# gist-ailab/QuBER

Measured on AMD Instinct MI355X. Metric: refined masks/sec on 640x480 RGB-D (N=20 inst), higher is better.
Workload: dtype f32; 1 GPU; batch=16 640x480 RGB-D, 20 initial instances/frame, ResNet-50 RGB-D refiner (boundary-error -> fg/centre/offset), encode+network+grouping+mask extraction; parallelism=dp1, hipgraph=False, foreground_filter=False

## Files before the change

include/quber_hip.h:

```cpp
#ifndef QUBER_HIP_H
#define QUBER_HIP_H

#include <stddef.h>
#include <stdint.h>

#ifdef __cplusplus
extern "C" {
#endif

typedef struct quber_ctx quber_ctx;

typedef struct quber_config {
    int32_t height, width;
    int32_t max_batch;
    int32_t max_instances;
    int32_t resnet_depth;
    int32_t res5_dilation;
    int32_t backbone_fusion_layers;
    int32_t head_fusion_layers;
    int32_t error_classes;
    int32_t gaussian_sigma;
    int32_t nms_kernel;
    int32_t top_k;
    int32_t stuff_area;
    int32_t min_instance_area;
    int32_t label_divisor;
    int32_t with_network;
    float center_threshold;
    float boundary_ratio;
    float pixel_mean[6];
    float pixel_std[6];
    int32_t eee_mask_on;
    int32_t eee_boundary_on;
    int32_t hierarchical;
    int32_t fusion_feat;
    int32_t fusion_pred;
    int32_t n_levels;
    int32_t level_heads[5][5];
    int32_t fusion_add;
    int32_t streams;
    int32_t compute_dtype;
    int32_t encode_legacy_f32;
    int32_t convs_dim;
    int32_t head_channels;
} quber_config;

#define QUBER_LOGIT_BASE 4

void quber_default_config(quber_config* cfg);
const char* quber_last_error(void);
const char* quber_version(void);

int quber_create(const quber_config* cfg, quber_ctx** out);
void quber_destroy(quber_ctx* ctx);

int quber_set_weight(quber_ctx* ctx, const char* name, const float* host, int64_t numel);
int quber_finalize_weights(quber_ctx* ctx);
int quber_num_weights(quber_ctx* ctx);
int quber_weight_spec(quber_ctx* ctx, int index, const char** name, int64_t* numel);

int quber_encode_initial_masks(quber_ctx* ctx, const uint8_t* dev_masks, int32_t batch, int32_t n_masks,
                               float* dev_out, void* stream);

int quber_encode_label_map(quber_ctx* ctx, const int32_t* dev_labels, int32_t batch, int32_t n_instances, float* dev_out,
                           void* stream);

int64_t quber_workspace_bytes(quber_ctx* ctx);

int quber_explicit_error_maps(quber_ctx* ctx, const uint8_t* dev_init, int32_t n_init, const uint8_t* dev_gt,
                              int32_t n_gt, int32_t batch, uint8_t* dev_out, void* stream);

int quber_forward(quber_ctx* ctx, const uint8_t* dev_bgr, const uint8_t* dev_depth, const float* dev_offsets,
                  int32_t batch, float* dev_logits, void* stream);

int quber_forward_profiled(quber_ctx* ctx, const uint8_t* dev_bgr, const uint8_t* dev_depth,
                           const float* dev_offsets, int32_t batch, float* dev_logits, void* stream,
                           double* kind_ms, int32_t* kind_launches);

int quber_profile_begin(quber_ctx* ctx);
int quber_profile_end(quber_ctx* ctx, void* stream);
int quber_profile_num_stages(quber_ctx* ctx);
int quber_profile_stage(quber_ctx* ctx, int index, const char** name, double* ms, double* bytes, double* flops,
                        int32_t* launches);

int quber_postprocess(quber_ctx* ctx, const float* dev_logits, int32_t n_planes, int32_t batch,
                      float* dev_panoptic, int32_t* dev_count, float* dev_labels, float* dev_scores,
                      float* dev_boxes, int32_t* dev_centers, int32_t* dev_ncenters, void* stream);

int quber_extract_masks(quber_ctx* ctx, const float* dev_panoptic, const float* dev_labels, int32_t batch,
                        int32_t max_inst, uint8_t* dev_masks, void* stream);

int quber_tta_flip_inputs(quber_ctx* ctx, uint8_t* dev_bgr, uint8_t* dev_depth, uint8_t* dev_masks, int32_t batch,
                          int32_t n_masks, void* stream);
int quber_tta_merge(quber_ctx* ctx, const float* dev_logits2, int32_t n_planes, int32_t batch, float* dev_out,
                    void* stream);

int quber_error_decode(quber_ctx* ctx, const float* dev_logits, int32_t n_planes, int32_t first_plane, int32_t classes,
                       int32_t batch, uint8_t* dev_classes, uint32_t* dev_hist, void* stream);
int quber_error_mask_hist(quber_ctx* ctx, const uint8_t* dev_classes, const uint8_t* dev_masks, int32_t batch, int32_t n_masks,
                          int32_t classes, uint32_t* dev_out, void* stream);
int quber_error_score(quber_ctx* ctx, const uint8_t* dev_classes, const uint8_t* dev_explicit, int32_t kind, int32_t error_type,
                      int32_t classes, int32_t batch, uint64_t* dev_table, void* stream);
int quber_error_overlay(quber_ctx* ctx, const uint8_t* dev_bgr, const uint8_t* dev_classes, int32_t batch, uint32_t color0,
                        uint32_t color1, uint32_t color2, uint32_t color3, uint8_t* dev_out, void* stream);

int quber_relabel_panoptic(quber_ctx* ctx, const float* dev_panoptic, const float* dev_labels, const int32_t* dev_count,
                           int32_t batch, int32_t mirror, int32_t* dev_ids, void* stream);
int quber_overlap_masks(quber_ctx* ctx, const uint8_t* dev_masks, const int32_t* dev_ids, int32_t batch, int32_t n_masks,
                        int32_t n_ids, uint32_t* dev_table, uint32_t* dev_area, void* stream);
int quber_overlap_ids(quber_ctx* ctx, const int32_t* dev_a, const int32_t* dev_b, int32_t batch, int32_t n_a, int32_t n_b,
                      uint32_t* dev_table, void* stream);

int quber_cleanup_ids(quber_ctx* ctx, int32_t* dev_ids, int32_t batch, int32_t n_ids, int32_t connectivity, int32_t keep_largest,
                      int32_t min_island_area, int32_t max_hole_area, uint32_t* dev_report, void* stream);
int quber_cleanup_postprocess(quber_ctx* ctx, const float* dev_logits, int32_t n_planes, int32_t batch, float* dev_panoptic,
                              const float* dev_labels, const int32_t* dev_count, float* dev_scores, float* dev_boxes,
                              int32_t connectivity, int32_t keep_largest, int32_t min_island_area, int32_t max_hole_area,
                              uint32_t* dev_report, void* stream);

int quber_perturb_masks(quber_ctx* ctx, const uint8_t* dev_masks, int32_t batch, int32_t n_masks, const int32_t* dev_programs,
                        int32_t n_ops, int32_t ops_per_round, const double* dev_iou_targets, uint8_t* dev_out, uint32_t* dev_report,
                        int32_t placement, void* stream);

int quber_mask_nms(quber_ctx* ctx, const uint8_t* dev_masks, const float* dev_scores, int32_t batch, int32_t n_masks, float thresh,
                   int32_t on_top, uint8_t* dev_out_masks, int32_t* dev_ids, int32_t* dev_source, float* dev_out_scores,
                   int32_t* dev_report, void* stream);

int quber_scene_perturb(quber_ctx* ctx, const uint8_t* dev_gt, const uint8_t* dev_props, const int32_t* dev_n_gt, const int32_t* dev_n_prop,
                        int32_t batch, int32_t n_gt_rows, int32_t n_prop_rows, int32_t max_masks, double min_mask_ratio,
                        const uint8_t* dev_fp_act, const uint8_t* dev_gs_act, const uint8_t* dev_merge_act, const uint8_t* dev_split_act,
                        const int32_t* dev_split_try, const uint8_t* dev_delete_act, uint8_t* dev_out_masks, int32_t* dev_info,
                        int32_t* dev_report, void* stream);

int quber_coco_match(quber_ctx* ctx, const uint8_t* dev_dt, const float* dev_scores, const double* dev_dt_boxes, int32_t n_dt,
                     const uint8_t* dev_gt, const uint8_t* dev_gt_flags, const double* dev_gt_area, const double* dev_gt_boxes, int32_t n_gt,
                     int32_t batch, int32_t iou_type, const double* dev_iou_thrs, int32_t n_thrs, const double* dev_area_rng, int32_t n_rng,
                     int32_t* dev_counts, int32_t* dev_order, float* dev_out_scores, double* dev_dt_area, double* dev_gt_area_used,
                     double* dev_iou, uint8_t* dev_dtm, uint8_t* dev_dtig, uint8_t* dev_gi, int32_t* dev_gorder, void* stream);

int quber_meanshift_seeds(quber_ctx* ctx, const float* dev_emb, int32_t batch, int32_t channels, const int32_t* dev_first, int32_t num_seeds,
                          int32_t* dev_indices, void* stream);
int quber_meanshift_climb(quber_ctx* ctx, const float* dev_emb, int32_t batch, int32_t channels, const int32_t* dev_indices, int32_t num_seeds,
                          float kappa, int32_t iters, float* dev_seeds, void* stream);
int quber_meanshift_link(quber_ctx* ctx, const float* dev_seeds, int32_t batch, int32_t num_seeds, float epsilon, int32_t* dev_seed_labels,
                         void* stream);
int quber_meanshift_assign(quber_ctx* ctx, const float* dev_emb, int32_t batch, int32_t channels, const float* dev_seeds,
                           const int32_t* dev_seed_labels, int32_t num_seeds, const float* dev_depth_z, float depth_threshold, int32_t n_masks,
                           int32_t* dev_ids, uint8_t* dev_masks, int32_t* dev_report, void* stream);
int quber_meanshift_cluster(quber_ctx* ctx, const float* dev_emb, int32_t batch, int32_t channels, const int32_t* dev_first, int32_t num_seeds,
                            float kappa, int32_t iters, float epsilon, const float* dev_depth_z, float depth_threshold, int32_t n_masks,
                            int32_t* dev_indices, float* dev_seeds, int32_t* dev_seed_labels, int32_t* dev_ids, uint8_t* dev_masks,
                            int32_t* dev_report, void* stream);

int quber_gms_seeds(quber_ctx* ctx, const float* dev_votes, const uint8_t* dev_fg, int32_t batch, int32_t subsample, const int32_t* dev_first,
                    const uint32_t* dev_draws, int32_t num_seeds, int32_t* dev_indices, int32_t* dev_info, void* stream);
int quber_gms_climb(quber_ctx* ctx, const float* dev_votes, const uint8_t* dev_fg, int32_t batch, int32_t subsample, const int32_t* dev_indices,
                    const int32_t* dev_info, int32_t num_seeds, float sigma, int32_t iters, float* dev_seeds, void* stream);
int quber_gms_link(quber_ctx* ctx, const float* dev_seeds, int32_t batch, int32_t num_seeds, const int32_t* dev_info, float epsilon,
                   int32_t* dev_seed_labels, void* stream);
int quber_gms_assign(quber_ctx* ctx, const float* dev_votes, const uint8_t* dev_fg, int32_t batch, const float* dev_seeds,
                     const int32_t* dev_seed_labels, const int32_t* dev_info, int32_t num_seeds, int32_t min_pixels, int32_t n_masks,
                     int32_t* dev_ids, uint8_t* dev_masks, float* dev_centers, int32_t* dev_report, void* stream);
int quber_gms_imp(quber_ctx* ctx, int32_t* dev_ids, int32_t batch, int32_t n_ids, int32_t ksize, int32_t largest, int32_t n_masks,
                  uint8_t* dev_masks, float* dev_centers, int32_t* dev_report, void* stream);
int quber_gms_cluster(quber_ctx* ctx, const float* dev_votes, const uint8_t* dev_fg, int32_t batch, const int32_t* dev_first,
                      const uint32_t* dev_draws, int32_t num_seeds, float sigma, int32_t iters, float epsilon, int32_t subsample,
                      int32_t min_pixels, int32_t imp_ksize, int32_t imp_largest, int32_t n_masks, int32_t* dev_indices, float* dev_seeds,
                      int32_t* dev_seed_labels, int32_t* dev_info, int32_t* dev_raw_ids, int32_t* dev_ids, uint8_t* dev_masks,
                      float* dev_centers, int32_t* dev_report, void* stream);

int quber_zoom_rois(quber_ctx* ctx, const int32_t* dev_ids, int32_t batch, int32_t n_ids, float padding, int32_t* dev_rois, void* stream);
int quber_zoom_crop(quber_ctx* ctx, const uint8_t* dev_bgr, const uint8_t* dev_depth, const int32_t* dev_ids, const int32_t* dev_slots,
                    const int32_t* dev_rois, int32_t batch, int32_t n_ids, int32_t n_slots, int32_t crop, uint8_t* dev_bgr_crop,
                    uint8_t* dev_depth_crop, uint8_t* dev_mask_crop, void* stream);
int quber_zoom_paste(quber_ctx* ctx, const int32_t* dev_crop_ids, const float* dev_crop_scores, const uint32_t* dev_table,
                     const uint32_t* dev_area, const uint8_t* dev_depth_crop, const int32_t* dev_slots, const int32_t* dev_rois,
                     int32_t batch, int32_t n_ids, int32_t n_slots, int32_t crop, int32_t n_crop_ids, float min_overlap, int32_t max_inst,
                     int32_t* dev_out_ids, uint8_t* dev_out_masks, int32_t* dev_source, float* dev_out_scores, float* dev_boxes,
                     int32_t* dev_report, void* stream);

#define QUBER_LOSS_WORDS 40
typedef struct quber_loss_spec {
    double top_k;
    double foreground_weight;
    double center_weight;
    double offset_weight;
    int32_t error_type;
    int32_t eee_mask_plane;
    int32_t eee_boundary_plane;
    int32_t eee_mask_loss;
    int32_t eee_boundary_loss;
    int32_t reserved;
} quber_loss_spec;
int quber_loss_targets(quber_ctx* ctx, const int32_t* dev_gt, int32_t batch, int32_t n_gt, int32_t sigma, int32_t small_area,
                       float small_weight, const float* dev_gauss, float* dev_targets, double* dev_points, int32_t* dev_area, void* stream);
int quber_losses(quber_ctx* ctx, const float* dev_logits, int32_t n_planes, const float* dev_targets, const uint8_t* dev_explicit,
                 const quber_loss_spec* spec, int32_t batch, double* dev_out, void* stream);

int64_t quber_contingency_workspace_bytes(int32_t cap);
int quber_label_contingency(const int32_t* dev_pred, const int32_t* dev_gt, int64_t n_pixels, int32_t cap,
                            void* dev_workspace, void* stream);

int64_t quber_boundary_workspace_bytes(int32_t h, int32_t w, int32_t n_masks);
int quber_boundary_overlap(const int32_t* dev_pred, const int32_t* dev_gt, int32_t h, int32_t w, const int32_t* dev_labels,
                           int32_t n_pred, int32_t n_gt, int32_t bound_pix, void* dev_workspace, uint32_t* dev_out,
                           void* stream);

int64_t quber_eval_batch_workspace_bytes(int32_t batch, int32_t h, int32_t w, int32_t cap, int32_t with_boundary);
int quber_eval_batch(const int32_t* dev_pred, const int32_t* dev_gt, int32_t batch, int32_t h, int32_t w, int32_t cap, int32_t bound_pix,
                     int32_t with_boundary, int32_t placement, void* dev_workspace, void* dev_out, void* stream);
int quber_munkres_batch(const double* dev_score, const int32_t* dev_rows, const int32_t* dev_cols, int32_t batch, int32_t cap,
                        int32_t placement, void* dev_workspace, int32_t* dev_assign, int32_t* dev_status, void* stream);

int quber_foreground_filter(const float* dev_fg_logits, int32_t n_classes, int32_t fg_class, const uint8_t* dev_masks,
                            int32_t batch, int32_t n_masks, int64_t hw, uint8_t* dev_fg_mask, uint64_t* dev_counts,
                            void* stream);

int quber_foreground_overlap(const uint8_t* dev_fg, int32_t fg_h, int32_t fg_w, const uint8_t* dev_masks, int32_t batch, int32_t n_masks,
                             int32_t h, int32_t w, uint64_t* dev_counts, void* stream);

int quber_normalize_depth(const void* dev_depth, int32_t is_float32, int64_t n_pixels, double min_val, double max_val,
                          uint8_t* dev_out3, uint8_t* dev_zero, void* stream);

int quber_resize_u8(const uint8_t* dev_src, int32_t src_h, int32_t src_w, int32_t channels, uint8_t* dev_dst,
                    int32_t dst_h, int32_t dst_w, int32_t linear, void* stream);

int quber_inpaint_telea_u8(const uint8_t* host_img, const uint8_t* host_mask, int32_t h, int32_t w, int32_t radius,
                           uint8_t* host_out);
int quber_inpaint_depth_u8(const uint8_t* host_depth3, int32_t h, int32_t w, int32_t kernel, uint8_t* host_out3);
int64_t quber_inpaint_depth_workspace_bytes(int32_t batch, int32_t h, int32_t w);
int quber_inpaint_depth_device(const uint8_t* dev_depth3, int32_t batch, int32_t h, int32_t w, int32_t kernel, void* dev_workspace,
                               int64_t workspace_bytes, uint8_t* dev_out3, void* stream);

int quber_debug_tensor(quber_ctx* ctx, const char* name, float** dev_ptr, int32_t* dims4, int32_t* channel_stride);
int32_t quber_debug_tensor_elem_size(quber_ctx* ctx, const char* name);
double quber_forward_flops(quber_ctx* ctx);
double quber_forward_flops_executed(quber_ctx* ctx);
double quber_forward_flops_padding(quber_ctx* ctx);
int quber_set_option(quber_ctx* ctx, int32_t key, int32_t value);
int quber_get_option(quber_ctx* ctx, int32_t key, int32_t* value);
void quber_set_tuning(int32_t key, int32_t value);
int32_t quber_debug_persistent_segments(int32_t tiles, int32_t blocks, int32_t k_slices, int32_t min_share, int32_t block,
                                        int32_t* out4, int32_t cap);
int32_t quber_debug_persistent_fixup(int32_t tiles, int32_t blocks, int32_t k_slices, int32_t min_share, int32_t xcd, int32_t j,
                                     int32_t* tile, int32_t* slots, int32_t cap);
int64_t quber_debug_ws_bytes(int32_t which, int32_t b, int32_t n, int32_t m, int32_t h, int32_t w, int32_t flag);
int quber_num_ops(quber_ctx* ctx);
int quber_op_info(quber_ctx* ctx, int index, const char** name, int32_t* kind, double* flops, int32_t* launches);
int quber_op_conv2d(const float* dev_x, int32_t batch, int32_t h, int32_t w, int32_t cin, const float* dev_w_oihw,
                    int32_t cout, int32_t ksize, int32_t stride, int32_t pad, int32_t dil, const float* dev_scale,
                    const float* dev_shift, const float* dev_residual, int32_t relu, float* dev_packed_scratch,
                    float* dev_y, void* stream);
int quber_op_conv1x1_f16(const void* dev_x, int32_t batch, int32_t h, int32_t w, int32_t cin, const void* dev_w_oi,
                         int32_t cout, const float* dev_scale, const float* dev_shift, const void* dev_residual,
                         int32_t relu, void* dev_y, void* stream);
int quber_op_conv2d_f16(const void* dev_x, int32_t batch, int32_t h, int32_t w, int32_t cin, const void* dev_w_packed,
                        int32_t cout, int32_t ksize, int32_t stride, int32_t pad, int32_t dil, int32_t kmode,
                        const float* dev_scale, const float* dev_shift, const void* dev_residual, int32_t relu,
                        double* dev_gn_sums, int32_t gn_groups, void* dev_y, void* stream);
int quber_op_conv1x1_dual(const float* dev_y, const float* dev_x, int32_t batch, int32_t oh, int32_t ow, int32_t mid,
                          int32_t h2, int32_t w2, int32_t cin, int32_t stride, const float* dev_w, const float* dev_shift,
                          const float* dev_ones, int32_t cout, int32_t relu, float* dev_out, void* stream);
int quber_op_conv3x3_winograd(const float* dev_x, int32_t batch, int32_t h, int32_t w, int32_t cin,
                              const float* dev_w_oihw, int32_t cout, int32_t dil, int32_t m, const float* dev_scale,
                              const float* dev_shift,
                              int32_t relu, float* dev_u_scratch, float* dev_ws, int64_t ws_floats, float* dev_y,
                              void* stream);
int quber_op_conv2d_view(const float* dev_x, int32_t x_cs, int64_t x_gs, const float* dev_w_oihw, const float* dev_scale, const float* dev_shift,
                         const float* dev_residual, int32_t res_cs, int64_t res_gs, float* dev_y, int32_t y_cs, int64_t y_gs, int32_t groups_of_launch,
                         int32_t batch, int32_t h, int32_t w, int32_t cin, int32_t cout, int32_t ksize, int32_t stride, int32_t pad, int32_t dil,
                         int32_t relu, double* dev_gn_sums, int32_t gn_groups, float* dev_packed_scratch, void* stream);
int quber_debug_conv_route(int32_t x_off, int32_t x_cs, int64_t x_gs, int32_t affine, int32_t res_off, int32_t res_cs, int64_t res_gs, int32_t y_off,
                           int32_t y_cs, int64_t y_gs, int32_t groups_of_launch, int32_t batch, int32_t h, int32_t w, int32_t cin, int32_t cout,
                           int32_t ksize, int32_t stride, int32_t pad, int32_t dil, int32_t gn_groups, int32_t workspace, int32_t cus, int32_t* out12);
int quber_op_conv3x3_winograd_view(const float* dev_x, int32_t x_cs, int64_t x_gs, const float* dev_w_oihw, const float* dev_scale,
                                   const float* dev_shift, float* dev_y, int32_t y_cs, int64_t y_gs, int32_t groups_of_launch, int32_t batch, int32_t h,
                                   int32_t w, int32_t cin, int32_t cout, int32_t dil, int32_t m, int32_t relu, double* dev_gn_sums, int32_t gn_groups,
                                   const double* dev_n_stats, const float* dev_n_gamma, const float* dev_n_beta, int32_t n_param_gs, int32_t n_groups,
                                   int32_t n_relu, float n_eps, float* dev_u_scratch, float* dev_ws, int64_t ws_floats, void* stream);
int quber_debug_winograd_route(int32_t x_cs, int64_t x_gs, int32_t y_cs, int64_t y_gs, int32_t in_place, int32_t groups_of_launch, int32_t batch,
                               int32_t h, int32_t w, int32_t cin, int32_t cout, int32_t dil, int32_t m, int32_t gn_groups, int32_t norm_groups,
                               int64_t ws_floats, int32_t* out12);
int quber_op_conv1x1_dual_view(const float* dev_y, int64_t y_gs, const float* dev_x, int64_t x_gs, const float* dev_w, int64_t w_gs,
                               const float* dev_shift, const float* dev_ones, int32_t ss_gs, float* dev_out, int64_t out_gs, int32_t groups_of_launch,
                               int32_t batch, int32_t oh, int32_t ow, int32_t mid, int32_t h2, int32_t w2, int32_t cin, int32_t stride, int32_t cout,
                               int32_t relu, void* stream);
int quber_debug_dual_route(int64_t y_gs, int64_t x_gs, int64_t w_gs, int32_t ss_gs, int64_t out_gs, int32_t groups_of_launch, int32_t batch, int32_t oh,
                           int32_t ow, int32_t mid, int32_t h2, int32_t w2, int32_t cin, int32_t stride, int32_t cout, int32_t workspace, int32_t cus,
                           int32_t* out12);
int quber_op_groupnorm(const float* dev_x, int32_t batch, int32_t h, int32_t w, int32_t c, int32_t groups,
                       const float* dev_gamma, const float* dev_beta, float eps, int32_t relu,
                       double* dev_stats_scratch, float* dev_y, void* stream);
int quber_op_bilinear(const float* dev_x, int32_t batch, int32_t h, int32_t w, int32_t c, int32_t oh, int32_t ow,
                      float* dev_y, void* stream);
int quber_op_maxpool3x3s2(const float* dev_x, int32_t batch, int32_t h, int32_t w, int32_t c, float* dev_y,
                          void* stream);
int32_t quber_debug_gn_pixels_per_block(int32_t hw, int32_t c, int32_t batch, int32_t groups_of_launch, int32_t stats_pass);
int quber_op_gn_stats(const void* dev_x, int32_t x_cs, int64_t x_gs, int32_t es, int32_t batch, int32_t h, int32_t w, int32_t c,
                      int32_t groups_of_launch, int32_t groups, double* dev_stats, int32_t zero, void* stream);
int quber_op_gn_apply(const void* dev_x, int32_t x_cs, int64_t x_gs, int32_t x_es, void* dev_y, int32_t y_cs, int64_t y_gs, int32_t y_es,
                      int32_t batch, int32_t h, int32_t w, int32_t c, int32_t groups_of_launch, int32_t groups, const double* dev_stats,
                      const float* dev_gamma, const float* dev_beta, int32_t param_gs, float eps, int32_t relu, void* stream);
int quber_op_maxpool_view(const void* dev_x, int32_t x_cs, int64_t x_gs, int32_t x_es, void* dev_y, int32_t y_cs, int64_t y_gs, int32_t y_es,
                          int32_t batch, int32_t h, int32_t w, int32_t c, int32_t groups_of_launch, void* stream);
int quber_op_bilinear_view(const void* dev_x, int32_t x_cs, int32_t x_es, void* dev_y, int32_t y_cs, int32_t y_es, int32_t batch, int32_t h,
                           int32_t w, int32_t c, int32_t oh, int32_t ow, void* stream);
int quber_op_avgpool(const void* dev_x, int32_t x_cs, int32_t x_es, void* dev_y, int32_t y_cs, int32_t y_es, int32_t batch, int32_t h, int32_t w,
                     int32_t c, void* stream);
int quber_op_add_channels(const void* dev_a, int32_t a_cs, int32_t a_es, const void* dev_b, int32_t b_cs, int32_t b_es, void* dev_y, int32_t y_cs,
                          int32_t y_es, int32_t batch, int32_t h, int32_t w, int32_t c, void* stream);
int quber_op_copy_channels(const void* dev_x, int32_t x_cs, int32_t x_es, void* dev_y, int32_t y_cs, int32_t y_es, int32_t batch, int32_t h,
                           int32_t w, int32_t c, void* stream);
int quber_op_predictors(int32_t n, const void* const* dev_feat, const float* const* dev_w, const float* const* dev_bias, void* const* dev_act_dst,
                        const int32_t* cout, const int32_t* q_ch0, const int32_t* act, int32_t c, int32_t feat_cs, int32_t es, int32_t batch,
                        int32_t h, int32_t w, float* dev_q, int32_t q_nch, int32_t act_cs, void* stream);
int quber_op_upsample_logits(const float* dev_q, float* dev_out, int32_t batch, int32_t nch, int32_t h, int32_t w, int32_t scale, int32_t oh,
                             int32_t ow, uint32_t mul_mask, void* stream);
int quber_op_preprocess(const uint8_t* dev_bgr, const uint8_t* dev_depth, const float* dev_offsets, void* dev_x, int32_t x_c, int32_t es,
                        int32_t batch, int32_t batch_cap, int32_t h, int32_t w, const float* mean6, const float* std6, int32_t streams,
                        void* stream);
int quber_dsn_forward(quber_ctx* ctx, const float* dev_xyz, int32_t batch, int32_t flags, float* dev_fg_logits, float* dev_offsets, float* dev_votes,
                      uint8_t* dev_fg_classes, uint8_t* dev_fg, void* stream);
int quber_dsn_forward_profiled(quber_ctx* ctx, const float* dev_xyz, int32_t batch, int32_t flags, float* dev_fg_logits, float* dev_offsets,
                               float* dev_votes, uint8_t* dev_fg_classes, uint8_t* dev_fg, void* stream, double* op_ms);

int32_t quber_op_esp_tiles(int32_t h, int32_t w);
int64_t quber_op_esp_packed_floats(int32_t n1);
int quber_op_dsn_pack(const float* dev_xyz, int32_t batch, int32_t h, int32_t w, int32_t flags, float* dev_x8, float* dev_clean, void* stream);
int quber_op_esp_pack(const float* dev_w1, const float* dev_w2, const float* dev_w4, const float* dev_w8, const float* dev_w16, int32_t n, int32_t n1,
                      float* dev_packed, void* stream);
int quber_op_esp_branches(const float* dev_t, int32_t t_cs, const float* dev_x, int32_t x_cs, float* dev_out, int32_t out_cs, int32_t batch, int32_t h,
                          int32_t w, int32_t c, int32_t groups, const float* dev_packed, double* dev_partials, int32_t tiles, void* stream);
int quber_op_esp_merge(const float* dev_d1, int32_t d1_cs, const float* dev_d2, const float* dev_d4, const float* dev_d8, const float* dev_d16,
                       int32_t d_cs, const float* dev_x, int32_t x_cs, float* dev_out, int32_t out_cs, int32_t batch, int32_t h, int32_t w, int32_t c,
                       int32_t groups, double* dev_partials, int32_t tiles, void* stream);
int quber_op_esp_stats(const double* dev_partials, int32_t batch, int32_t tiles, int32_t groups, double* dev_stats, void* stream);
int quber_op_dsn_head(const float* dev_f, int32_t f_cs, int32_t batch, int32_t h, int32_t w, int32_t c, const float* dev_clean, const float* dev_wfg,
                      const float* dev_wcd, float* dev_logits, float* dev_offsets, float* dev_votes, uint8_t* dev_classes, uint8_t* dev_fg, void* stream);

int quber_rrn_forward(quber_ctx* ctx, const float* dev_rgb_crop, const uint8_t* dev_mask_crop, int32_t n, float logit_threshold, float* dev_logits,
                      uint8_t* dev_refined, void* stream);
int quber_rrn_forward_profiled(quber_ctx* ctx, const float* dev_rgb_crop, const uint8_t* dev_mask_crop, int32_t n, float logit_threshold, float* dev_logits,
                               uint8_t* dev_refined, void* stream, double* op_ms);
int quber_rrn_crop(quber_ctx* ctx, const uint8_t* dev_bytes, const int32_t* dev_ids, const int32_t* dev_slots, const int32_t* dev_rois, const float* dev_table,
                   int32_t batch, int32_t n_ids, int32_t n_slots, int32_t crop, float* dev_rgb_crop, uint8_t* dev_mask_crop, void* stream);
int quber_rrn_paste(quber_ctx* ctx, const uint8_t* dev_refined, const int32_t* dev_slots, const int32_t* dev_rois, const float* dev_z, int32_t batch,
                    int32_t n_ids, int32_t n_slots, int32_t crop, int32_t n_masks, int32_t* dev_out_ids, uint8_t* dev_out_masks, int32_t* dev_source,
                    float* dev_keys, int32_t* dev_report, void* stream);
int quber_op_rrn_pack(const float* dev_rgb, const uint8_t* dev_mask, int32_t batch, int32_t h, int32_t w, float* dev_x8, void* stream);
int quber_op_rrn_head(const float* dev_f, int32_t f_cs, int32_t batch, int32_t h, int32_t w, int32_t c, const float* dev_wfg, float thr, float* dev_logits,
                      uint8_t* dev_refined, void* stream);
int quber_op_rrn_head3(const float* dev_f, int32_t f_cs, int32_t batch, int32_t h, int32_t w, int32_t c, const float* dev_w9, float bias, float thr,
                       float* dev_logits, uint8_t* dev_refined, void* stream);

int32_t quber_op_cgnet_tiles(int32_t h, int32_t w, int32_t joint);
int quber_op_cgnet_joint(const float* dev_x, int32_t x_cs, float* dev_joi, int32_t joi_cs, int32_t batch, int32_t h, int32_t w, int32_t c, int32_t dil,
                         const float* dev_w1, const float* dev_scale1, const float* dev_shift1, const float* dev_slope1, const float* dev_wloc,
                         const float* dev_wsur, const float* dev_scale2, const float* dev_shift2, const float* dev_slope2, double* dev_partials,
                         int32_t tiles, void* stream);
int quber_op_cgnet_sums(const float* dev_x, int32_t x_cs, int32_t batch, int32_t h, int32_t w, int32_t c, double* dev_partials, int32_t tiles,
                        void* stream);
int quber_op_cgnet_apply(const float* dev_joi, int32_t joi_cs, const float* dev_x, int32_t x_cs, float* dev_out, int32_t out_cs, int32_t batch,
                         int32_t h, int32_t w, int32_t c, int32_t hidden, const double* dev_partials, int32_t tiles, const float* dev_fc0,
                         const float* dev_b0, const float* dev_fc2, const float* dev_b2, float* dev_mean, float* dev_y, void* stream);

int quber_op_lmff_preprocess(const uint8_t* dev_bgr, const uint8_t* dev_depth, int64_t pixels, float* dev_x, void* stream);
int quber_op_lmff_dwconv(const float* dev_x, int32_t x_cs, float* dev_y, int32_t y_cs, int32_t batch, int32_t h, int32_t w, int32_t c, int32_t dil,
                         const float* dev_w9, const float* dev_scale, const float* dev_shift, const float* dev_slope, void* stream);
int quber_op_lmff_pool(const float* dev_x, int32_t x_cs, float* dev_y, int32_t y_cs, int32_t batch, int32_t h, int32_t w, int32_t c, int32_t oh,
                       int32_t ow, int32_t mode, void* stream);
int quber_op_lmff_affine(const float* dev_a, int32_t a_cs, const float* dev_b, int32_t b_cs, float* dev_y, int32_t y_cs, int32_t batch, int32_t h,
                         int32_t w, int32_t c, const float* dev_scale, const float* dev_shift, const float* dev_slope, void* stream);
int quber_op_lmff_pmca(const float* dev_x, int32_t x_cs, int32_t batch, int32_t h, int32_t w, int32_t c, const float* dev_w2x2, const float* dev_fc0,
                       const float* dev_alpha, const float* dev_fc2, float* dev_wts, double* dev_sums, void* stream);
int quber_op_lmff_scale(const float* dev_x, int32_t x_cs, const float* dev_wts, float* dev_y, int32_t y_cs, int32_t batch, int32_t h, int32_t w,
                        int32_t c, void* stream);
int quber_op_lmff_gate(const float* dev_o, int32_t o_cs, const float* dev_att, int32_t att_cs, float* dev_q, int32_t batch, int32_t h, int32_t w,
                       int32_t c, void* stream);
int quber_op_group_pixels(const float* dev_logits, int32_t n_planes, int32_t batch, int32_t h, int32_t w, int32_t cap,
                          const int32_t* dev_centers, const int32_t* dev_ncenters, uint8_t* dev_ids, uint32_t* dev_area,
                          void* stream);

#ifdef __cplusplus
}
#endif
#endif
```

quber_amd/_lib.py:

```python
import ctypes as C
import os

_HERE = os.path.dirname(os.path.abspath(__file__))
LIB_PATH = os.environ.get("QUBER_LIB") or os.path.join(_HERE, "libquber_hip.so")


class QuberConfig(C.Structure):
    _fields_ = [
        ("height", C.c_int32), ("width", C.c_int32), ("max_batch", C.c_int32), ("max_instances", C.c_int32),
        ("resnet_depth", C.c_int32), ("res5_dilation", C.c_int32), ("backbone_fusion_layers", C.c_int32),
        ("head_fusion_layers", C.c_int32), ("error_classes", C.c_int32), ("gaussian_sigma", C.c_int32),
        ("nms_kernel", C.c_int32), ("top_k", C.c_int32), ("stuff_area", C.c_int32),
        ("min_instance_area", C.c_int32), ("label_divisor", C.c_int32), ("with_network", C.c_int32),
        ("center_threshold", C.c_float), ("boundary_ratio", C.c_float),
        ("pixel_mean", C.c_float * 6), ("pixel_std", C.c_float * 6),
        ("eee_mask_on", C.c_int32), ("eee_boundary_on", C.c_int32), ("hierarchical", C.c_int32),
        ("fusion_feat", C.c_int32), ("fusion_pred", C.c_int32), ("n_levels", C.c_int32),
        ("level_heads", (C.c_int32 * 5) * 5), ("fusion_add", C.c_int32), ("streams", C.c_int32),
        ("compute_dtype", C.c_int32), ("encode_legacy_f32", C.c_int32),
        ("convs_dim", C.c_int32), ("head_channels", C.c_int32),
    ]


class QuberError(RuntimeError):
    pass


_P = C.c_void_p
_I = C.c_int32
SIGNATURES = {
    "quber_default_config": (None, [C.POINTER(QuberConfig)]),
    "quber_last_error": (C.c_char_p, []),
    "quber_version": (C.c_char_p, []),
    "quber_create": (C.c_int, [C.POINTER(QuberConfig), C.POINTER(_P)]),
    "quber_destroy": (None, [_P]),
    "quber_set_weight": (C.c_int, [_P, C.c_char_p, _P, C.c_int64]),
    "quber_finalize_weights": (C.c_int, [_P]),
    "quber_num_weights": (C.c_int, [_P]),
    "quber_weight_spec": (C.c_int, [_P, C.c_int, C.POINTER(C.c_char_p), C.POINTER(C.c_int64)]),
    "quber_encode_initial_masks": (C.c_int, [_P, _P, _I, _I, _P, _P]),
    "quber_encode_label_map": (C.c_int, [_P, _P, _I, _I, _P, _P]),
    "quber_workspace_bytes": (C.c_int64, [_P]),
    "quber_explicit_error_maps": (C.c_int, [_P, _P, _I, _P, _I, _I, _P, _P]),
    "quber_forward": (C.c_int, [_P, _P, _P, _P, _I, _P, _P]),
    "quber_forward_profiled": (C.c_int, [_P, _P, _P, _P, _I, _P, _P, C.POINTER(C.c_double * 3), C.POINTER(_I * 3)]),
    "quber_profile_begin": (C.c_int, [_P]),
    "quber_profile_end": (C.c_int, [_P, _P]),
    "quber_profile_num_stages": (C.c_int, [_P]),
    "quber_profile_stage": (C.c_int, [_P, C.c_int, C.POINTER(C.c_char_p), C.POINTER(C.c_double), C.POINTER(C.c_double),
                                      C.POINTER(C.c_double), C.POINTER(_I)]),
    "quber_postprocess": (C.c_int, [_P, _P, _I, _I, _P, _P, _P, _P, _P, _P, _P, _P]),
    "quber_extract_masks": (C.c_int, [_P, _P, _P, _I, _I, _P, _P]),
    "quber_tta_flip_inputs": (C.c_int, [_P, _P, _P, _P, _I, _I, _P]),
    "quber_tta_merge": (C.c_int, [_P, _P, _I, _I, _P, _P]),
    "quber_error_decode": (C.c_int, [_P, _P, _I, _I, _I, _I, _P, _P, _P]),
    "quber_error_mask_hist": (C.c_int, [_P, _P, _P, _I, _I, _I, _P, _P]),
    "quber_error_score": (C.c_int, [_P, _P, _P, _I, _I, _I, _I, _P, _P]),
    "quber_error_overlay": (C.c_int, [_P, _P, _P, _I, C.c_uint32, C.c_uint32, C.c_uint32, C.c_uint32, _P, _P]),
    "quber_relabel_panoptic": (C.c_int, [_P, _P, _P, _P, _I, _I, _P, _P]),
    "quber_overlap_masks": (C.c_int, [_P, _P, _P, _I, _I, _I, _P, _P, _P]),
    "quber_overlap_ids": (C.c_int, [_P, _P, _P, _I, _I, _I, _P, _P]),
    "quber_cleanup_ids": (C.c_int, [_P, _P, _I, _I, _I, _I, _I, _I, _P, _P]),
    "quber_cleanup_postprocess": (C.c_int, [_P, _P, _I, _I, _P, _P, _P, _P, _P, _I, _I, _I, _I, _P, _P]),
    "quber_perturb_masks": (C.c_int, [_P, _P, _I, _I, _P, _I, _I, _P, _P, _P, _I, _P]),
    "quber_mask_nms": (C.c_int, [_P, _P, _P, _I, _I, C.c_float, _I, _P, _P, _P, _P, _P, _P]),
    "quber_scene_perturb": (C.c_int, [_P, _P, _P, _P, _P, _I, _I, _I, _I, C.c_double] + [_P] * 10),
    "quber_coco_match": (C.c_int, [_P, _P, _P, _P, _I, _P, _P, _P, _P, _I, _I, _I, _P, _I, _P, _I] + [_P] * 11),
    "quber_meanshift_seeds": (C.c_int, [_P, _P, _I, _I, _P, _I, _P, _P]),
    "quber_meanshift_climb": (C.c_int, [_P, _P, _I, _I, _P, _I, C.c_float, _I, _P, _P]),
    "quber_meanshift_link": (C.c_int, [_P, _P, _I, _I, C.c_float, _P, _P]),
    "quber_meanshift_assign": (C.c_int, [_P, _P, _I, _I, _P, _P, _I, _P, C.c_float, _I, _P, _P, _P, _P]),
    "quber_meanshift_cluster": (C.c_int, [_P, _P, _I, _I, _P, _I, C.c_float, _I, C.c_float, _P, C.c_float, _I, _P, _P, _P, _P, _P, _P, _P]),
    "quber_gms_seeds": (C.c_int, [_P, _P, _P, _I, _I, _P, _P, _I, _P, _P, _P]),
    "quber_gms_climb": (C.c_int, [_P, _P, _P, _I, _I, _P, _P, _I, C.c_float, _I, _P, _P]),
    "quber_gms_link": (C.c_int, [_P, _P, _I, _I, _P, C.c_float, _P, _P]),
    "quber_gms_assign": (C.c_int, [_P, _P, _P, _I, _P, _P, _P, _I, _I, _I, _P, _P, _P, _P, _P]),
    "quber_gms_imp": (C.c_int, [_P, _P, _I, _I, _I, _I, _I, _P, _P, _P, _P]),
    "quber_gms_cluster": (C.c_int, [_P, _P, _P, _I, _P, _P, _I, C.c_float, _I, C.c_float, _I, _I, _I, _I, _I, _P, _P, _P, _P, _P, _P, _P, _P, _P, _P]),
    "quber_zoom_rois": (C.c_int, [_P, _P, _I, _I, C.c_float, _P, _P]),
    "quber_zoom_crop": (C.c_int, [_P, _P, _P, _P, _P, _P, _I, _I, _I, _I, _P, _P, _P, _P]),
    "quber_zoom_paste": (C.c_int, [_P, _P, _P, _P, _P, _P, _P, _P, _I, _I, _I, _I, _I, C.c_float, _I, _P, _P, _P, _P, _P, _P, _P]),
    "quber_loss_targets": (C.c_int, [_P, _P, _I, _I, _I, _I, C.c_float, _P, _P, _P, _P, _P]),
    "quber_losses": (C.c_int, [_P, _P, _I, _P, _P, _P, _I, _P, _P]),
    "quber_contingency_workspace_bytes": (C.c_int64, [_I]),
    "quber_label_contingency": (C.c_int, [_P, _P, C.c_int64, _I, _P, _P]),
    "quber_boundary_workspace_bytes": (C.c_int64, [_I, _I, _I]),
    "quber_boundary_overlap": (C.c_int, [_P, _P, _I, _I, _P, _I, _I, _I, _P, _P, _P]),
    "quber_eval_batch_workspace_bytes": (C.c_int64, [_I, _I, _I, _I, _I]),
    "quber_eval_batch": (C.c_int, [_P, _P, _I, _I, _I, _I, _I, _I, _I, _P, _P, _P]),
    "quber_munkres_batch": (C.c_int, [_P, _P, _P, _I, _I, _I, _P, _P, _P, _P]),
    "quber_foreground_filter": (C.c_int, [_P, _I, _I, _P, _I, _I, C.c_int64, _P, _P, _P]),
    "quber_normalize_depth": (C.c_int, [_P, _I, C.c_int64, C.c_double, C.c_double, _P, _P, _P]),
    "quber_inpaint_telea_u8": (C.c_int, [_P, _P, _I, _I, _I, _P]),
    "quber_inpaint_depth_u8": (C.c_int, [_P, _I, _I, _I, _P]),
    "quber_inpaint_depth_workspace_bytes": (C.c_int64, [_I, _I, _I]),
    "quber_inpaint_depth_device": (C.c_int, [_P, _I, _I, _I, _I, _P, C.c_int64, _P, _P]),
    "quber_resize_u8": (C.c_int, [_P, _I, _I, _I, _P, _I, _I, _I, _P]),
    "quber_debug_tensor": (C.c_int, [_P, C.c_char_p, C.POINTER(_P), C.POINTER(_I * 4), C.POINTER(_I)]),
    "quber_debug_tensor_elem_size": (C.c_int32, [_P, C.c_char_p]),
    "quber_forward_flops": (C.c_double, [_P]),
    "quber_forward_flops_executed": (C.c_double, [_P]),
    "quber_forward_flops_padding": (C.c_double, [_P]),
    "quber_set_tuning": (None, [_I, _I]),
    "quber_set_option": (C.c_int, [_P, _I, _I]),
    "quber_get_option": (C.c_int, [_P, _I, C.POINTER(_I)]),
    "quber_num_ops": (C.c_int, [_P]),
    "quber_op_info": (C.c_int, [_P, C.c_int, C.POINTER(C.c_char_p), C.POINTER(_I), C.POINTER(C.c_double), C.POINTER(_I)]),
    "quber_debug_persistent_segments": (C.c_int32, [_I, _I, _I, _I, _I, _P, _I]),
    "quber_debug_persistent_fixup": (C.c_int32, [_I, _I, _I, _I, _I, _I, _P, _P, _I]),
    "quber_debug_ws_bytes": (C.c_int64, [_I, _I, _I, _I, _I, _I, _I]),
    "quber_op_conv1x1_f16": (C.c_int, [_P, _I, _I, _I, _I, _P, _I, _P, _P, _P, _I, _P, _P]),
    "quber_op_conv2d_f16": (C.c_int, [_P, _I, _I, _I, _I, _P, _I, _I, _I, _I, _I, _I, _P, _P, _P, _I, _P, _I, _P, _P]),
    "quber_op_conv1x1_dual": (C.c_int, [_P, _P, _I, _I, _I, _I, _I, _I, _I, _I, _P, _P, _P, _I, _I, _P, _P]),
    "quber_op_conv2d": (C.c_int, [_P, _I, _I, _I, _I, _P, _I, _I, _I, _I, _I, _P, _P, _P, _I, _P, _P, _P]),
    "quber_op_conv3x3_winograd": (C.c_int, [_P, _I, _I, _I, _I, _P, _I, _I, _I, _P, _P, _I, _P, _P, C.c_int64, _P, _P]),
    "quber_op_conv2d_view": (C.c_int, [_P, _I, C.c_int64, _P, _P, _P, _P, _I, C.c_int64, _P, _I, C.c_int64] + [_I] * 11 + [_P, _I, _P, _P]),
    "quber_debug_conv_route": (C.c_int, [_I, _I, C.c_int64, _I, _I, _I, C.c_int64, _I, _I, C.c_int64] + [_I] * 13 + [_P]),
    "quber_op_conv3x3_winograd_view": (C.c_int, [_P, _I, C.c_int64, _P, _P, _P, _P, _I, C.c_int64] + [_I] * 9 + [_P, _I, _P, _P, _P, _I, _I, _I, C.c_float,
                                                 _P, _P, C.c_int64, _P]),
    "quber_debug_winograd_route": (C.c_int, [_I, C.c_int64, _I, C.c_int64] + [_I] * 11 + [C.c_int64, _P]),
    "quber_op_conv1x1_dual_view": (C.c_int, [_P, C.c_int64, _P, C.c_int64, _P, C.c_int64, _P, _P, _I, _P, C.c_int64] + [_I] * 11 + [_P]),
    "quber_debug_dual_route": (C.c_int, [C.c_int64, C.c_int64, C.c_int64, _I, C.c_int64] + [_I] * 12 + [_P]),
    "quber_op_groupnorm": (C.c_int, [_P, _I, _I, _I, _I, _I, _P, _P, C.c_float, _I, _P, _P, _P]),
    "quber_op_bilinear": (C.c_int, [_P, _I, _I, _I, _I, _I, _I, _P, _P]),
    "quber_op_maxpool3x3s2": (C.c_int, [_P, _I, _I, _I, _I, _P, _P]),
    "quber_debug_gn_pixels_per_block": (C.c_int32, [_I, _I, _I, _I, _I]),
    "quber_op_gn_stats": (C.c_int, [_P, _I, C.c_int64, _I, _I, _I, _I, _I, _I, _I, _P, _I, _P]),
    "quber_op_gn_apply": (C.c_int, [_P, _I, C.c_int64, _I, _P, _I, C.c_int64, _I, _I, _I, _I, _I, _I, _I, _P, _P, _P, _I, C.c_float, _I, _P]),
    "quber_op_maxpool_view": (C.c_int, [_P, _I, C.c_int64, _I, _P, _I, C.c_int64, _I, _I, _I, _I, _I, _I, _P]),
    "quber_op_bilinear_view": (C.c_int, [_P, _I, _I, _P, _I, _I, _I, _I, _I, _I, _I, _I, _P]),
    "quber_op_avgpool": (C.c_int, [_P, _I, _I, _P, _I, _I, _I, _I, _I, _I, _P]),
    "quber_op_add_channels": (C.c_int, [_P, _I, _I, _P, _I, _I, _P, _I, _I, _I, _I, _I, _I, _P]),
    "quber_op_copy_channels": (C.c_int, [_P, _I, _I, _P, _I, _I, _I, _I, _I, _I, _P]),
    "quber_op_predictors": (C.c_int, [_I, _P, _P, _P, _P, _P, _P, _P, _I, _I, _I, _I, _I, _I, _P, _I, _I, _P]),
    "quber_op_upsample_logits": (C.c_int, [_P, _P, _I, _I, _I, _I, _I, _I, _I, C.c_uint32, _P]),
    "quber_op_preprocess": (C.c_int, [_P, _P, _P, _P, _I, _I, _I, _I, _I, _I, _P, _P, _I, _P]),
    "quber_op_group_pixels": (C.c_int, [_P, _I, _I, _I, _I, _I, _P, _P, _P, _P, _P]),
    "quber_foreground_overlap": (C.c_int, [_P, _I, _I, _P, _I, _I, _I, _I, _P, _P]),
    "quber_dsn_forward": (C.c_int, [_P, _P, _I, _I, _P, _P, _P, _P, _P, _P]),
    "quber_dsn_forward_profiled": (C.c_int, [_P, _P, _I, _I, _P, _P, _P, _P, _P, _P, _P]),
    "quber_op_esp_tiles": (C.c_int32, [_I, _I]),
    "quber_op_esp_packed_floats": (C.c_int64, [_I]),
    "quber_op_dsn_pack": (C.c_int, [_P, _I, _I, _I, _I, _P, _P, _P]),
    "quber_op_esp_pack": (C.c_int, [_P, _P, _P, _P, _P, _I, _I, _P, _P]),
    "quber_op_esp_branches": (C.c_int, [_P, _I, _P, _I, _P, _I, _I, _I, _I, _I, _I, _P, _P, _I, _P]),
    "quber_op_esp_merge": (C.c_int, [_P, _I, _P, _P, _P, _P, _I, _P, _I, _P, _I, _I, _I, _I, _I, _I, _P, _I, _P]),
    "quber_op_esp_stats": (C.c_int, [_P, _I, _I, _I, _P, _P]),
    "quber_op_dsn_head": (C.c_int, [_P, _I, _I, _I, _I, _I, _P, _P, _P, _P, _P, _P, _P, _P, _P]),
    "quber_rrn_forward": (C.c_int, [_P, _P, _P, _I, C.c_float, _P, _P, _P]),
    "quber_rrn_forward_profiled": (C.c_int, [_P, _P, _P, _I, C.c_float, _P, _P, _P, _P]),
    "quber_rrn_crop": (C.c_int, [_P, _P, _P, _P, _P, _P, _I, _I, _I, _I, _P, _P, _P]),
    "quber_rrn_paste": (C.c_int, [_P, _P, _P, _P, _P, _I, _I, _I, _I, _I, _P, _P, _P, _P, _P, _P]),
    "quber_op_rrn_pack": (C.c_int, [_P, _P, _I, _I, _I, _P, _P]),
    "quber_op_rrn_head": (C.c_int, [_P, _I, _I, _I, _I, _I, _P, C.c_float, _P, _P, _P]),
    "quber_op_rrn_head3": (C.c_int, [_P, _I, _I, _I, _I, _I, _P, C.c_float, C.c_float, _P, _P, _P]),
    "quber_op_cgnet_tiles": (C.c_int32, [_I, _I, _I]),
    "quber_op_cgnet_joint": (C.c_int, [_P, _I, _P, _I, _I, _I, _I, _I, _I] + [_P] * 10 + [_I, _P]),
    "quber_op_cgnet_sums": (C.c_int, [_P, _I, _I, _I, _I, _I, _P, _I, _P]),
    "quber_op_cgnet_apply": (C.c_int, [_P, _I, _P, _I, _P, _I, _I, _I, _I, _I, _I, _P, _I, _P, _P, _P, _P, _P, _P, _P]),
    "quber_op_lmff_preprocess": (C.c_int, [_P, _P, C.c_int64, _P, _P]),
    "quber_op_lmff_dwconv": (C.c_int, [_P, _I, _P, _I, _I, _I, _I, _I, _I, _P, _P, _P, _P, _P]),
    "quber_op_lmff_pool": (C.c_int, [_P, _I, _P, _I, _I, _I, _I, _I, _I, _I, _I, _P]),
    "quber_op_lmff_affine": (C.c_int, [_P, _I, _P, _I, _P, _I, _I, _I, _I, _I, _P, _P, _P, _P]),
    "quber_op_lmff_pmca": (C.c_int, [_P, _I, _I, _I, _I, _I, _P, _P, _P, _P, _P, _P, _P]),
    "quber_op_lmff_scale": (C.c_int, [_P, _I, _P, _P, _I, _I, _I, _I, _I, _P]),
    "quber_op_lmff_gate": (C.c_int, [_P, _I, _P, _I, _P, _I, _I, _I, _I, _P]),
}

_lib = None


def load():
    global _lib
    if _lib is not None:
        return _lib
    if not os.path.exists(LIB_PATH):
        raise QuberError(
            f"{LIB_PATH} not found: build it with `make -C quber_amd/csrc` (or __graft_entry__.build()); "
            "quber_amd has no CPU fallback")
    import torch
    lib = C.CDLL(LIB_PATH)
    for name, (res, args) in SIGNATURES.items():
        fn = getattr(lib, name)
        fn.restype = res
        fn.argtypes = args
    mode = os.environ.get("QUBER_WINOGRAD", "auto").lower()
    if mode not in ("auto", "f6", "f4", "f2", "off"):
        raise QuberError(f"QUBER_WINOGRAD={mode!r}: expected auto, f6, f4, f2 or off")
    lib.quber_set_tuning(6, 1 if mode == "off" else 0)
    lib.quber_set_tuning(9, {"f2": 2, "f4": 4, "f6": 6}.get(mode, 0))
    if "QUBER_PERSIST" in os.environ:
        lib.quber_set_tuning(13, int(os.environ["QUBER_PERSIST"]))
    _lib = lib
    return lib


def check(rc):
    if rc != 0:
        raise QuberError(load().quber_last_error().decode())
```

quber_amd/csrc/api.hip:

```cpp
#include "plan.h"

#include <optional>

using namespace quber;

namespace quber { int wf_read_stamps(unsigned long long* dst, int n), h8_read_stamps(unsigned long long* dst, int n), x8_read_stamps(unsigned long long* dst, int n); }

int quber::check_cfg(const quber_config& c) {
    if (c.height <= 0 || c.width <= 0) return fail("height and width must be positive");
    if (c.with_network && (c.height < 16 || c.width < 16)) return fail("frames smaller than 16 x 16 are not supported");
    if (c.with_network == 2) {
        if (c.height % 8 || c.width % 8) return fail("LMFFNet needs height and width to be multiples of 8");
        return c.max_batch >= 1 ? 0 : fail("max_batch must be >= 1");
    }
    if (c.with_network == 3) {
        if (c.height % 8 || c.width % 8) return fail("CGNet needs height and width to be multiples of 8");
        return c.max_batch >= 1 ? 0 : fail("max_batch must be >= 1");
    }
    if (c.with_network == 4) {
        if (c.height < 16 || c.width < 16 || c.height % 16 || c.width % 16) return fail("the Depth Seeding Network needs height and width to be multiples of 16");
        return c.max_batch >= 1 ? 0 : fail("max_batch must be >= 1");
    }
    if (c.with_network == 5) {
        if (c.height != c.width || c.height < 16 || c.height % 16) return fail("the Region Refinement Network needs square crops whose side is a multiple of 16");
        return c.max_batch >= 1 ? 0 : fail("max_batch must be >= 1");
    }
    if (c.max_batch < 1) return fail("max_batch must be >= 1");
    if (c.max_instances < 1) return fail("max_instances must be >= 1");
    if (c.resnet_depth != 50 && c.resnet_depth != 101 && c.resnet_depth != 152) return fail("resnet_depth must be 50, 101 or 152");
    if (c.res5_dilation != 1 && c.res5_dilation != 2 && c.res5_dilation != 4) return fail("res5_dilation must be 1, 2 or 4");
    if (c.res5_dilation == 1) return fail("res5_dilation 1 (output stride 32) is not supported by this build");
    if (c.error_classes < 2 || c.error_classes > 4) return fail("error_classes must be 2..4");
    if (c.streams != 1 && c.streams != 2) return fail("streams must be 1 or 2");
    if (c.with_network == 1 && c.convs_dim != 128 && c.convs_dim != 256) return fail("convs_dim must be 128 or 256");
    if (c.with_network == 1 && c.head_channels != 32 && c.head_channels != 64) return fail("head_channels must be 32 or 64");
    if (c.compute_dtype < 0 || c.compute_dtype > 3)
        return fail("compute_dtype must be 0 (fp32 MFMA), 1 (bf16 operands), 2 (fp16 operands) or 3 (fp32 operands as 3 bf16 terms)");
    if (c.with_network && c.hierarchical) {
        if (c.n_levels < 1 || c.n_levels > 5) return fail("n_levels must be 1..5");
        int seen[5] = {0, 0, 0, 0, 0};
        for (int i = 0; i < c.n_levels; ++i) {
            if (c.level_heads[i][0] < 0) return fail("empty hierarchy level");
            for (int j = 0; j < 5 && c.level_heads[i][j] >= 0; ++j) {
                const int k = c.level_heads[i][j];
                if (k > 4) return fail("hierarchy head id out of range");
                seen[k]++;
            }
        }
        const int want[5] = {1, 1, 1, c.eee_mask_on ? 1 : 0, c.eee_boundary_on ? 1 : 0};
        for (int k = 0; k < 5; ++k)
            if (seen[k] != want[k]) return fail("the hierarchy must list every enabled head exactly once");
    }
    if (c.top_k < 1 || c.top_k > 254) return fail("top_k must be in 1..254");
    if (c.gaussian_sigma < 1 || c.gaussian_sigma > 40) return fail("gaussian_sigma out of range");
    return 0;
}

static int ws_reserve(quber_ctx* c, LazyWs& w, size_t need) {
    if (need <= w.bytes) return 0;
    if (w.p) {
        QB_CHECK(hipFree(w.p));
        c->alloc_bytes -= w.bytes;
        w = LazyWs();
    }
    QB_CHECK(hipMalloc(&w.p, need));
    w.bytes = need;
    c->alloc_bytes += need;
    return 0;
}

extern "C" {

const char* quber_version(void) { return "quber-hip 0.1 (gfx950, fp32 MFMA)"; }

void quber_default_config(quber_config* c) {
    memset(c, 0, sizeof(*c));
    c->height = 480; c->width = 640; c->max_batch = 1; c->max_instances = 64;
    c->resnet_depth = 50; c->res5_dilation = 2; c->backbone_fusion_layers = 2; c->head_fusion_layers = 3;
    c->error_classes = 4; c->gaussian_sigma = 10; c->nms_kernel = 7; c->top_k = 200; c->stuff_area = 2048;
    c->min_instance_area = 512; c->label_divisor = 1000; c->with_network = 1;
    c->eee_mask_on = 0; c->eee_boundary_on = 1; c->hierarchical = 1; c->fusion_feat = 1; c->fusion_pred = 1;
    c->n_levels = 2;
    c->streams = 2;
    c->fusion_add = 0;
    c->convs_dim = 128; c->head_channels = 32;
    for (int i = 0; i < 5; ++i)
        for (int j = 0; j < 5; ++j) c->level_heads[i][j] = -1;
    c->level_heads[0][0] = 4;
    c->level_heads[1][0] = 0; c->level_heads[1][1] = 1; c->level_heads[1][2] = 2;
    c->center_threshold = 0.3f; c->boundary_ratio = 0.01f;
    const float mean[6] = {103.53f, 116.28f, 123.675f, 127.5f, 127.5f, 127.5f};
    for (int i = 0; i < 6; ++i) { c->pixel_mean[i] = mean[i]; c->pixel_std[i] = 1.f; }
}

int quber_create(const quber_config* cfg, quber_ctx** out) {
    if (!cfg || !out) return fail("null argument");
    if (check_cfg(*cfg)) return -1;
    int ndev = 0;
    if (hipGetDeviceCount(&ndev) != hipSuccess || ndev == 0) return fail("no HIP device available");
    int device = 0;
    if (hipGetDevice(&device) != hipSuccess) return fail("hipGetDevice failed");
    quber_ctx* c = new quber_ctx();
    c->cfg = *cfg;
    c->tune = quber::g_tune;
    c->device = device;
    const int B = cfg->max_batch, H = cfg->height, W = cfg->width;
    const int sg = cfg->gaussian_sigma, side = 6 * sg + 3, c0 = 3 * sg + 1;
    std::vector<float> g((size_t)side * side);
    for (int y = 0; y < side; ++y)
        for (int x = 0; x < side; ++x)
            g[(size_t)y * side + x] = (float)exp(-((double)((x - c0) * (x - c0)) + (double)((y - c0) * (y - c0))) / (2.0 * sg * sg));
    Builder b(c, false);
    c->gauss = b.upload(g);
    c->enc_ws = b.dalloc_bytes(encode_ws_bytes(B, cfg->max_instances, H, W));
    c->enc_bad = (int*)b.dalloc_bytes(16);
    c->err_ws = (uint8_t*)b.dalloc_bytes(errmaps_ws_bytes(B, cfg->max_instances > 0 ? cfg->max_instances : 1, H, W));
    c->post_ws = b.dalloc_bytes(postprocess_ws_bytes(B, H, W, cfg->top_k));
    c->cleanup_ws = b.dalloc_bytes(cleanup_ws_bytes(B, H, W, cfg->top_k));
    if (!b.err.empty()) {
        std::string e = b.err;
        quber_destroy(c);
        return fail(e);
    }
    if (cfg->with_network) {
        Builder dry(c, true);
        if (cfg->with_network == 2) build_lmff(dry);
        else if (cfg->with_network == 3) build_cgnet(dry);
        else if (cfg->with_network == 4) build_dsn(dry);
        else if (cfg->with_network == 5) build_rrn(dry);
        else dry.build();
    }
    *out = c;
    return 0;
}

void quber_destroy(quber_ctx* c) {
    if (!c) return;
    if (c->prof && quber::g_prof == c->prof.get()) quber::g_prof = nullptr;
    for (hipEvent_t e : c->prof_events) (void)hipEventDestroy(e);
    for (int l = 1; l < LANES; ++l) {
        if (c->lane_fork[l]) (void)hipEventDestroy(c->lane_fork[l]);
        if (c->lane_join[l]) (void)hipEventDestroy(c->lane_join[l]);
        if (c->lane_stream[l]) (void)hipStreamDestroy(c->lane_stream[l]);
    }
    for (void* p : c->allocs) (void)hipFree(p);
    for (LazyWs& w : c->lazy)
        if (w.p) (void)hipFree(w.p);
    delete c;
}

int quber_num_weights(quber_ctx* c) { return c ? (int)c->specs.size() : 0; }
int quber_weight_spec(quber_ctx* c, int i, const char** name, int64_t* numel) {
    if (!c || i < 0 || i >= (int)c->specs.size()) return fail("weight index out of range");
    *name = c->specs[i].first.c_str();
    *numel = c->specs[i].second;
    return 0;
}

int quber_set_weight(quber_ctx* c, const char* name, const float* host, int64_t numel) {
    if (!c || !name || !host || numel <= 0) return fail("bad argument to quber_set_weight");
    if (c->finalized) return fail("weights already finalized");
    c->hostw[name].assign(host, host + numel);
    return 0;
}

int quber_finalize_weights(quber_ctx* c) {
    if (!c) return fail("null context");
    if (!c->cfg.with_network) return fail("context was created with with_network = 0");
    if (c->finalized) return fail("weights already finalized");
    quber::TuneScope tscope(&c->tune);
    Builder b(c, false);
    c->flops = c->wino_flops = c->wino_saved = c->wino_pad = 0.0;
    if (c->cfg.with_network >= 2 && c->cfg.with_network <= 5) {
        c->splitk_floats = (size_t)4 << 20;
        c->splitk_ws = (float*)b.dalloc_bytes(sizeof(float) * c->splitk_floats);
        if (c->cfg.with_network == 2) build_lmff(b);
        else if (c->cfg.with_network == 3) build_cgnet(b);
        else if (c->cfg.with_network == 4) build_dsn(b);
        else build_rrn(b);
    } else {
        b.build();
    }
    if (c->wino_floats) c->wino_ws = (float*)b.dalloc_bytes(sizeof(float) * c->wino_floats);
    if (c->lanes_built) {
        c->lane_splitk_floats = c->splitk_floats;
        for (int l = 1; l < LANES; ++l) {
            QB_CHECK(hipStreamCreateWithFlags(&c->lane_stream[l], hipStreamNonBlocking));
            QB_CHECK(hipEventCreateWithFlags(&c->lane_fork[l], hipEventDisableTiming));
            QB_CHECK(hipEventCreateWithFlags(&c->lane_join[l], hipEventDisableTiming));
            c->lane_splitk_ws[l] = (float*)b.dalloc_bytes(sizeof(float) * c->lane_splitk_floats);
            if (c->lane_wino_floats[l]) c->lane_wino_ws[l] = (float*)b.dalloc_bytes(sizeof(float) * c->lane_wino_floats[l]);
        }
    }
    if (!b.err.empty()) {
        c->ops.clear();
        return fail(b.err);
    }
    QB_CHECK(hipDeviceSynchronize());
    c->hostw.clear();
    c->finalized = true;
    return 0;
}

double quber_forward_flops(quber_ctx* c) { return c ? c->flops : 0.0; }
double quber_forward_flops_executed(quber_ctx* c) {
    if (!c) return 0.0;
    return c->flops - c->wino_saved;
}
double quber_forward_flops_padding(quber_ctx* c) { return c ? c->wino_pad : 0.0; }
void quber_set_tuning(int32_t key, int32_t value) {
    if (op_set_tuning(key, value)) return;
    (void)quber::tuning_set(quber::g_tune, key, value);
}

int quber_set_option(quber_ctx* c, int32_t key, int32_t value) {
    if (!c) return fail("null context");
    if (quber::tuning_plan_time(key) && c->finalized) return fail("option " + std::to_string(key) + " shapes the plan: set it before quber_finalize_weights");
    if (!quber::tuning_set(c->tune, key, value)) return fail("unknown option key " + std::to_string(key));
    return 0;
}

int quber_get_option(quber_ctx* c, int32_t key, int32_t* value) {
    if (!c || !value) return fail("null argument");
    int* f = quber::tuning_field(c->tune, key);
    if (!f) return fail("unknown option key " + std::to_string(key));
    *value = *f;
    return 0;
}

#ifdef WF_STAMPS
int quber_wf_read_stamps(unsigned long long* dst, int n) { return quber::wf_read_stamps(dst, n); }
#endif
#ifdef H8_STAMPS
int quber_h8_read_stamps(unsigned long long* dst, int n) { return quber::h8_read_stamps(dst, n); }
#endif
#ifdef X8_STAMPS
int quber_x8_read_stamps(unsigned long long* dst, int n) { return quber::x8_read_stamps(dst, n); }
#endif
#ifdef PK_STAMPS
int quber_pk_read_stamps(unsigned long long* dst, int n) { return quber::pk_read_stamps(dst, n); }
int quber_pk_read_span(unsigned long long* dst, int n) { return quber::pk_read_span(dst, n); }
#endif

int32_t quber_debug_persistent_segments(int32_t tiles, int32_t blocks, int32_t k_slices, int32_t min_share, int32_t block, int32_t* out4, int32_t cap) {
    return quber::conv_persistent_segments(tiles, blocks, k_slices, min_share, block, out4, cap);
}
int32_t quber_debug_persistent_fixup(int32_t tiles, int32_t blocks, int32_t k_slices, int32_t min_share, int32_t xcd, int32_t j, int32_t* tile, int32_t* slots, int32_t cap) {
    return quber::conv_persistent_fixup(tiles, blocks, k_slices, min_share, xcd, j, tile, slots, cap);
}

int64_t quber_debug_ws_bytes(int32_t which, int32_t b, int32_t n, int32_t m, int32_t h, int32_t w, int32_t flag) {
    switch (which) {
    case 0: return (int64_t)mask_nms_ws_bytes(b, n, h, w);
    case 1: return (int64_t)coco_match_ws_bytes(b, n, h, w, flag);
    case 2: return (int64_t)scene_ws_bytes(b, n, m, h, w);
    case 3: return (int64_t)meanshift_ws_bytes(b, h, w);
    case 4: return (int64_t)gms_ws_bytes(b, h, w);
    case 5: return (int64_t)zoom_ws_bytes(b, h, w);
    case 6: return (int64_t)losses_ws_bytes(b, h, w);
    case 7: return (int64_t)cleanup_ws_bytes(b, h, w, n);
    case 8: return (int64_t)postprocess_ws_bytes(b, h, w, n);
    default: return -1;
    }
}

int quber_profile_begin(quber_ctx* c) {
    if (!c) return fail("null context");
    if (!c->prof) c->prof.reset(new quber::Profiler());
    c->prof->recs.clear(); c->prof->sums.clear(); c->prof->used = 0;
    quber::g_prof = c->prof.get();
    return 0;
}

int quber_profile_end(quber_ctx* c, void* stream) {
    if (!c || !c->prof || quber::g_prof != c->prof.get()) return fail("quber_profile_end without quber_profile_begin");
    quber::g_prof = nullptr;
    QB_CHECK(hipStreamSynchronize((hipStream_t)stream));
    quber::Profiler& p = *c->prof;
    p.sums.assign(p.tags.size(), quber::StageSum());
    for (size_t i = 0; i < p.tags.size(); ++i) p.sums[i].name = p.tags[i];
    for (const quber::ProfRec& r : p.recs) {
        float ms = 0.f;
        QB_CHECK(hipEventElapsedTime(&ms, r.e0, r.e1));
        quber::StageSum& s = p.sums[r.tag];
        s.ms += ms; s.bytes += r.bytes; s.flops += r.flops; s.launches += 1;
    }
    return 0;
}

int quber_profile_num_stages(quber_ctx* c) { return (c && c->prof) ? (int)c->prof->sums.size() : 0; }

int quber_profile_stage(quber_ctx* c, int i, const char** name, double* ms, double* bytes, double* flops, int32_t* launches) {
    if (!c || !c->prof || i < 0 || i >= (int)c->prof->sums.size()) return fail("stage index out of range");
    const quber::StageSum& s = c->prof->sums[i];
    *name = s.name.c_str(); *ms = s.ms; *bytes = s.bytes; *flops = s.flops; *launches = s.launches;
    return 0;
}

int quber_num_ops(quber_ctx* c) { return c ? (int)c->ops.size() : 0; }
int quber_op_info(quber_ctx* c, int i, const char** name, int32_t* kind, double* flops, int32_t* launches) {
    if (!c || i < 0 || i >= (int)c->ops.size()) return fail("op index out of range");
    const Op& o = c->ops[i];
    *name = o.name.c_str(); *kind = o.kind; *flops = o.flops; *launches = o.launches;
    return 0;
}

int quber_encode_initial_masks(quber_ctx* c, const uint8_t* masks, int32_t batch, int32_t n, float* out, void* stream) {
    if (check_batch(c, batch)) return -1;
    if (n > c->cfg.max_instances) return fail("more initial masks than max_instances");
    if (!masks && n > 0) return fail("null masks");
    return launch_encode(masks, batch, n, c->cfg.height, c->cfg.width, c->gauss, c->cfg.gaussian_sigma, c->cfg.encode_legacy_f32, c->enc_ws, out, (hipStream_t)stream);
}

int quber_encode_label_map(quber_ctx* c, const int32_t* labels, int32_t batch, int32_t n, float* out, void* stream) {
    if (check_batch(c, batch)) return -1;
    if (n > c->cfg.max_instances) return fail("more instances than max_instances");
    if (!labels && n > 0) return fail("null label map");
    return launch_encode_labels(labels, batch, n, c->cfg.height, c->cfg.width, c->gauss, c->cfg.gaussian_sigma, c->cfg.encode_legacy_f32, c->enc_ws, out, c->enc_bad, (hipStream_t)stream);
}

int64_t quber_workspace_bytes(quber_ctx* c) { return c ? (int64_t)c->alloc_bytes : 0; }

int quber_explicit_error_maps(quber_ctx* c, const uint8_t* init, int32_t n_init, const uint8_t* gt, int32_t n_gt, int32_t batch, uint8_t* out, void* stream) {
    if (check_batch(c, batch)) return -1;
    const int H = c->cfg.height, W = c->cfg.width;
    int d = (int)rint((double)c->cfg.boundary_ratio * sqrt((double)H * H + (double)W * W));
    if (d < 1) d = 1;
    return launch_errmaps(init, n_init, gt, n_gt, batch, c->cfg.max_instances > 0 ? c->cfg.max_instances : 1, H, W, d, c->err_ws, out, (hipStream_t)stream);
}

static int forward_begin(quber_ctx* c, const char* who, std::optional<quber::TuneScope>& scope, const uint8_t* bgr, const uint8_t* depth,
                         const float* offs, int batch, float* logits, bool lmff_own, bool rest_ok, const char* null_msg, hipStream_t st) {
    if (check_batch(c, batch)) return -1;
    if (!c->finalized) return fail(std::string(who) + " before quber_finalize_weights");
    scope.emplace(&c->tune);
    if (c->cfg.with_network == 4) return fail(std::string(who) + ": a Depth Seeding Network context runs through quber_dsn_forward");
    if (c->cfg.with_network == 5) return fail(std::string(who) + ": a Region Refinement Network context runs through quber_rrn_forward");
    if (lmff_own && c->cfg.with_network >= 2) return 1;
    if (!bgr || (!depth && c->cfg.streams == 2) || !offs || !logits || !rest_ok) return fail(null_msg);
    c->cur_out = logits;
    c->cur_bgr = bgr; c->cur_depth = depth; c->cur_off = offs;
    return c->stem_fused ? 0 : launch_preprocess(bgr, depth, offs, c->X, batch, c->cfg.max_batch, c->cfg.height, c->cfg.width,
                                                 c->cfg.pixel_mean, c->cfg.pixel_std, c->cfg.streams, st);
}

int quber_forward(quber_ctx* c, const uint8_t* bgr, const uint8_t* depth, const float* offs, int32_t batch, float* logits, void* stream) {
    hipStream_t st = (hipStream_t)stream;
    std::optional<quber::TuneScope> tscope;
    int rc = forward_begin(c, "quber_forward", tscope, bgr, depth, offs, batch, logits, true, true, "null tensor", st);
    if (rc == 1) {
        if (!bgr || !depth || !logits) return fail("null tensor");
        c->cur_out = logits;
        const long pixels = (long)batch * c->cfg.height * c->cfg.width;
        int r2 = c->cfg.with_network == 3 ? launch_cg_preprocess(bgr, depth, pixels, c->X.p, st) : launch_lmff_preprocess(bgr, depth, pixels, c->X.p, st);
        for (size_t i = 0; !r2 && i < c->ops.size(); ++i)
            if (!c->ops[i].ctl) r2 = c->ops[i].run(batch, st);
        return r2;
    }
    if (rc) return rc;
    c->lanes_on = c->lanes_built && tune().lanes && batch <= (c->cfg.compute_dtype == 0 || c->cfg.compute_dtype == 3 ? LANE_BATCH_F32 : LANE_BATCH) && c->lane_stream[1] != nullptr &&
                  quber::g_prof == nullptr;
    auto lane_used = [&](int l) { return c->lanes_on && l > 0; };
    for (auto& op : c->ops) {
        if (op.ctl == 1) {
            if (lane_used(op.lane)) {
                QB_CHECK(hipEventRecord(c->lane_fork[op.lane], st));
                QB_CHECK(hipStreamWaitEvent(c->lane_stream[op.lane], c->lane_fork[op.lane], 0));
            }
            continue;
        }
        if (op.ctl == 2) {
            if (lane_used(op.lane)) {
                QB_CHECK(hipEventRecord(c->lane_join[op.lane], c->lane_stream[op.lane]));
                QB_CHECK(hipStreamWaitEvent(st, c->lane_join[op.lane], 0));
            }
            continue;
        }
        c->lane_now = lane_used(op.lane) ? op.lane : 0;
        rc = op.run(batch, c->lane_now ? c->lane_stream[op.lane] : st);
        if (rc) return rc;
    }
    c->lane_now = 0;
    c->lanes_on = false;
    return 0;
}

static int run_ops(quber_ctx* c, int batch, hipStream_t st, double* op_ms) {
    const size_t n = c->ops.size();
    if (op_ms && c->prof_events.size() < 2 * n) {
        const size_t old = c->prof_events.size();
        c->prof_events.resize(2 * n);
        for (size_t i = old; i < 2 * n; ++i) QB_CHECK(hipEventCreate(&c->prof_events[i]));
    }
    for (size_t i = 0; i < n; ++i) {
        if (op_ms) QB_CHECK(hipEventRecord(c->prof_events[2 * i], st));
        if (!c->ops[i].ctl) {
            const int rc = c->ops[i].run(batch, st);
            if (rc) return rc;
        }
        if (op_ms) QB_CHECK(hipEventRecord(c->prof_events[2 * i + 1], st));
    }
    if (!op_ms) return 0;
    QB_CHECK(hipStreamSynchronize(st));
    for (size_t i = 0; i < n; ++i) {
        float ms = 0.f;
        QB_CHECK(hipEventElapsedTime(&ms, c->prof_events[2 * i], c->prof_events[2 * i + 1]));
        op_ms[i] = ms;
    }
    return 0;
}

static int dsn_run(quber_ctx* c, const char* who, const float* xyz, int batch, int flags, float* fg_logits, float* offsets, float* votes, uint8_t* fg_classes, uint8_t* fg,
                   hipStream_t st, double* op_ms) {
    if (check_batch(c, batch)) return -1;
    if (c->cfg.with_network != 4) return fail(std::string(who) + ": the context was not created with with_network = 4");
    if (!c->finalized) return fail(std::string(who) + " before quber_finalize_weights");
    if (!xyz) return fail(std::string(who) + ": null xyz");
    if (flags & ~1) return fail(std::string(who) + ": unknown flag bits");
    quber::TuneScope tscope(&c->tune);
    c->dsn_xyz = xyz; c->dsn_flags = flags;
    c->dsn_logits = fg_logits; c->dsn_offsets = offsets; c->dsn_votes = votes; c->dsn_classes = fg_classes; c->dsn_fg = fg;
    return run_ops(c, batch, st, op_ms);
}

int quber_dsn_forward(quber_ctx* c, const float* xyz, int32_t batch, int32_t flags, float* fg_logits, float* offsets, float* votes, uint8_t* fg_classes, uint8_t* fg,
                      void* stream) {
    return dsn_run(c, "quber_dsn_forward", xyz, batch, flags, fg_logits, offsets, votes, fg_classes, fg, (hipStream_t)stream, nullptr);
}

int quber_dsn_forward_profiled(quber_ctx* c, const float* xyz, int32_t batch, int32_t flags, float* fg_logits, float* offsets, float* votes, uint8_t* fg_classes,
                               uint8_t* fg, void* stream, double* op_ms) {
    if (!op_ms) return fail("quber_dsn_forward_profiled: null op_ms");
    return dsn_run(c, "quber_dsn_forward_profiled", xyz, batch, flags, fg_logits, offsets, votes, fg_classes, fg, (hipStream_t)stream, op_ms);
}

static int rrn_run(quber_ctx* c, const char* who, const float* rgb_crop, const uint8_t* mask_crop, int n, float thr, float* logits, uint8_t* refined, hipStream_t st,
                   double* op_ms) {
    if (check_batch(c, n)) return -1;
    if (c->cfg.with_network != 5) return fail(std::string(who) + ": the context was not created with with_network = 5");
    if (!c->finalized) return fail(std::string(who) + " before quber_finalize_weights");
    if (!rgb_crop || !mask_crop) return fail(std::string(who) + ": null crops");
    if (!logits && !refined) return fail(std::string(who) + ": neither logits nor refined masks requested");
    if (!(thr == thr)) return fail(std::string(who) + ": logit_threshold is not a number");
    quber::TuneScope tscope(&c->tune);
    c->rrn_rgb = rgb_crop; c->rrn_mask = mask_crop; c->rrn_thr = thr; c->rrn_logits = logits; c->rrn_refined = refined;
    return run_ops(c, n, st, op_ms);
}

int quber_rrn_forward(quber_ctx* c, const float* rgb_crop, const uint8_t* mask_crop, int32_t n, float logit_threshold, float* logits, uint8_t* refined, void* stream) {
    return rrn_run(c, "quber_rrn_forward", rgb_crop, mask_crop, n, logit_threshold, logits, refined, (hipStream_t)stream, nullptr);
}

int quber_rrn_forward_profiled(quber_ctx* c, const float* rgb_crop, const uint8_t* mask_crop, int32_t n, float logit_threshold, float* logits, uint8_t* refined,
                               void* stream, double* op_ms) {
    if (!op_ms) return fail("quber_rrn_forward_profiled: null op_ms");
    return rrn_run(c, "quber_rrn_forward_profiled", rgb_crop, mask_crop, n, logit_threshold, logits, refined, (hipStream_t)stream, op_ms);
}

int quber_forward_profiled(quber_ctx* c, const uint8_t* bgr, const uint8_t* depth, const float* offs, int32_t batch,
                           float* logits, void* stream, double* kind_ms, int32_t* kind_launches) {
    hipStream_t st = (hipStream_t)stream;
    std::optional<quber::TuneScope> tscope;
    int rc = forward_begin(c, "quber_forward_profiled", tscope, bgr, depth, offs, batch, logits, false, kind_ms && kind_launches, "null argument", st);
    if (rc) return rc;
    const size_t n = c->ops.size();
    if (c->prof_events.size() < 2 * n) {
        const size_t old = c->prof_events.size();
        c->prof_events.resize(2 * n);
        for (size_t i = old; i < 2 * n; ++i) QB_CHECK(hipEventCreate(&c->prof_events[i]));
    }
    c->lanes_on = false;
    for (size_t i = 0; i < n; ++i) {
        QB_CHECK(hipEventRecord(c->prof_events[2 * i], st));
        if (!c->ops[i].ctl) {
            rc = c->ops[i].run(batch, st);
            if (rc) return rc;
        }
        QB_CHECK(hipEventRecord(c->prof_events[2 * i + 1], st));
    }
    QB_CHECK(hipStreamSynchronize(st));
    for (int k = 0; k < OP_KINDS; ++k) { kind_ms[k] = 0.0; kind_launches[k] = 0; }
    for (size_t i = 0; i < n; ++i) {
        float ms = 0.f;
        QB_CHECK(hipEventElapsedTime(&ms, c->prof_events[2 * i], c->prof_events[2 * i + 1]));
        kind_ms[c->ops[i].kind] += ms;
        kind_launches[c->ops[i].kind] += 1;
    }
    return 0;
}

int quber_postprocess(quber_ctx* c, const float* logits, int32_t n_planes, int32_t batch, float* pan, int32_t* count,
                      float* labels, float* scores, float* boxes, int32_t* centers, int32_t* ncenters, void* stream) {
    if (check_batch(c, batch)) return -1;
    PostCfg pc;
    pc.threshold = c->cfg.center_threshold; pc.nms_kernel = c->cfg.nms_kernel; pc.top_k = c->cfg.top_k;
    pc.stuff_area = c->cfg.stuff_area; pc.min_area = c->cfg.min_instance_area; pc.label_divisor = c->cfg.label_divisor;
    pc.cap = c->cfg.top_k;
    return launch_postprocess(logits, n_planes, batch, c->cfg.height, c->cfg.width, pc, c->post_ws, pan, count, labels,
                              scores, boxes, centers, ncenters, (hipStream_t)stream);
}

int quber_extract_masks(quber_ctx* c, const float* pan, const float* labels, int32_t batch, int32_t max_inst,
                        uint8_t* masks, void* stream) {
    if (check_batch(c, batch)) return -1;
    return launch_extract_masks(pan, labels, batch, c->cfg.height, c->cfg.width, c->cfg.top_k, max_inst, masks,
                                (hipStream_t)stream);
}

int quber_tta_flip_inputs(quber_ctx* c, uint8_t* bgr, uint8_t* depth, uint8_t* masks, int32_t batch, int32_t n, void* stream) {
    if (check_tta_batch(c, batch)) return -1;
    if (n < 0 || n > c->cfg.max_instances) return fail("initial masks outside 0..max_instances");
    if (!bgr || (!masks && n > 0)) return fail("null tensor");
    const int H = c->cfg.height, W = c->cfg.width;
    const long hw = (long)H * W;
    hipStream_t st = (hipStream_t)stream;
    if (launch_tta_flip_u8(bgr, bgr + batch * hw * 3, batch, H, W, 3, st)) return -1;
    if (depth && launch_tta_flip_u8(depth, depth + batch * hw * 3, batch, H, W, 3, st)) return -1;
    if (n > 0 && launch_tta_flip_u8(masks, masks + (long)batch * n * hw, (long)batch * n, H, W, 1, st)) return -1;
    return 0;
}

int quber_tta_merge(quber_ctx* c, const float* logits2, int32_t n_planes, int32_t batch, float* out, void* stream) {
    if (check_tta_batch(c, batch)) return -1;
    if (n_planes < 4) return fail("test-time augmentation: fewer than 4 logit planes");
    if (!logits2 || !out) return fail("null tensor");
    return launch_tta_merge(logits2, n_planes, batch, c->cfg.height, c->cfg.width, out, (hipStream_t)stream);
}

int quber_error_decode(quber_ctx* c, const float* logits, int32_t n_planes, int32_t first_plane, int32_t classes, int32_t batch,
                       uint8_t* classes_out, uint32_t* hist, void* stream) {
    if (check_batch(c, batch)) return -1;
    if (!logits || !classes_out) return fail("null tensor");
    return launch_error_decode(logits, n_planes, first_plane, classes, batch, c->cfg.height, c->cfg.width, classes_out, hist,
                               (hipStream_t)stream);
}

int quber_error_mask_hist(quber_ctx* c, const uint8_t* classes_map, const uint8_t* masks, int32_t batch, int32_t n, int32_t classes,
                          uint32_t* out, void* stream) {
    if (check_batch(c, batch)) return -1;
    if (n < 0 || n > c->cfg.max_instances) return fail("initial masks outside 0..max_instances");
    if (n == 0) return 0;
    if (!classes_map || !masks || !out) return fail("null tensor");
    return launch_error_mask_hist(classes_map, masks, batch, n, classes, c->cfg.height, c->cfg.width, out, (hipStream_t)stream);
}

int quber_error_score(quber_ctx* c, const uint8_t* classes_map, const uint8_t* explicit_maps, int32_t kind, int32_t error_type,
                      int32_t classes, int32_t batch, uint64_t* table, void* stream) {
    if (check_batch(c, batch)) return -1;
    if (!classes_map || !explicit_maps || !table) return fail("null tensor");
    return launch_error_score(classes_map, explicit_maps, kind, error_type, classes, batch, c->cfg.height, c->cfg.width,
                              (unsigned long long*)table, (hipStream_t)stream);
}

// ... 513 lines not shown
```

quber_amd/csrc/common.h:

```cpp
#pragma once
#include <hip/hip_runtime.h>
#include <stdint.h>
#include <string>

struct quber_loss_spec;

namespace quber {

struct View {
    float* p = nullptr;
    int B = 0, H = 0, W = 0, C = 0;
    int cs = 0;
    long gs = 0;
    int es = 4;
    float* at(long elems) const { return p ? reinterpret_cast<float*>(reinterpret_cast<char*>(p) + elems * es) : nullptr; }
};

struct ConvP {
    const float* in;
    const float* w;
    const float* scale;
    const float* shift;
    const float* res;
    const float* prelu;
    float* out;
    int B, H, W, Cin, in_cs;
    int OH, OW, Cout, out_cs;
    int res_cs;
    int K, Kpad;
    int kh, kw, stride, pad, dil;
    int relu;
    int M;
    int mtiles, ntiles;
    int vec_out;
    float* ws;
    size_t ws_floats;
    int ksplit;
    int kchunk;
    int nfull, tail_shift;
    int ws_rows, ws_row0;
    double* gn_sum;
    int gn_groups, gn_cpg;
    int ohw;
    int kmode;
    int skip_rows;
    long in_gs, out_gs, res_gs, w_gs;
    int ss_gs;
    const char* tag;
    int pk_T, pk_tpg, pk_min, pk_in_bytes, pk_debug;
    const float* in2;
    int in2_cs, H2, W2, stride2, K1, pk_in2_bytes;
    long in2_gs;
    int es;
    int acc_chunk;
    int lean_in_bytes;
    unsigned dv_m[5], dv_s[5];
    const void* w3;
    long w3_plane;
    int dil_g[4];
    int h8_ss_bytes;
    const double* n_stats; const float* n_gamma; const float* n_beta; float* n_coef;
    int n_groups, n_param_gs, n_relu, n_coef_bytes; float n_eps;
    int bf16;
    int zones, zx1, zx2;
};

int device_cus();
void set_error(const std::string& msg);
int fail(const std::string& msg);

inline size_t ws_align(size_t v) { return (v + 255) / 256 * 256; }
struct WsWalk {
    char* base;
    size_t off = 0;
    template <class T> T* take(size_t count, bool pad = true) {
        T* p = base ? reinterpret_cast<T*>(base + off) : nullptr;
        off += pad ? ws_align(count * sizeof(T)) : count * sizeof(T);
        return p;
    }
};

struct ProfScope {
    int rec;
    hipStream_t st;
    ProfScope(const char* tag, double bytes, double flops, hipStream_t s);
    ~ProfScope();
    ProfScope(const ProfScope&) = delete;
    ProfScope& operator=(const ProfScope&) = delete;
};

struct WinoNorm {
    const double* stats;
    const float* gamma;
    const float* beta;
    int groups, cpg, param_gs, relu;
    double n;
    float eps;
};

struct WinoP {
    View in, out;
    const float* u;
    const void* u3;
    long u3_plane;
    const float* uf;
    int algo;
    const float* scale;
    const float* shift;
    int ss_gs, relu;
    int dil;
    int m;
    int pack;
    int dtype;
    double* gn_sum;
    int gn_groups;
    WinoNorm norm;
    float* ws;
    size_t ws_floats;
    float* splitk_ws;
    size_t splitk_floats;
};

enum { ROUTE_TILE = 1, ROUTE_SPLITK = 2, ROUTE_PERSISTENT = 3, ROUTE_WINO = 4, ROUTE_WINO_FUSED = 5, ROUTE_X8 = 6, ROUTE_SEPARATE = 7 };
struct ConvRoute {
    int kernel;
    int sums;
    int BM, BN;
    int S;
    int tail_shift;
    int tiles, blocks, nk, min_share;
    int packed, shared_v;
    int cus;
};

int launch_conv(const ConvP& p, int G, hipStream_t st, ConvRoute* dry = nullptr);
int launch_conv_winograd(const WinoP& q, int B, int G, hipStream_t st, ConvRoute* dry = nullptr);
int launch_winograd_weights(const float* w_oihw, int Cout, int Cin, int m, float* u, hipStream_t st);
void winograd_weights_host(const float* w_oihw, int Cout, int Cin, int m, float* u);
bool winograd_eligible(int k, int stride, int pad, int dil, int Cin, int Cout);
bool winograd_m6_channels_ok(int Cin, int Cout);
size_t winograd_ws_floats(int B, int H, int W, int Cin, int Cout, int G, int dil, int m);
double winograd_mac_ratio(int H, int W, int dil, int m);
double winograd_mac_ratio_run(int H, int W, int dil, int m, bool pack);
bool winograd_fused_ok(const WinoP& q, int B, int G);
int launch_conv_winograd_fused(const WinoP& q, int B, int G, hipStream_t st, ConvRoute* dry = nullptr);
void winograd_fused_pack_host(const float* u, int Cout, int Cin, float* uf);
int launch_winograd_fused_pack(const float* u, int Cout, int Cin, float* uf, hipStream_t st);
size_t winograd_fused_ws_floats(int B, int Cin, int G);
int winograd_fused_prepare();

struct Tuning {
    int winograd = 0;
    int wino_min_cin = 32;
    int wino_max_ratio = 67;
    int wino_variant = 0;
    int wino_min_cout = 32;
    int wino_pairs = 0;
    int wino_chunk_mb = 0;
    int wino_pack = 1;
    int wino_fused = 1;
    int wino_fused_max_cin = 160;
    int acc_chunk = 2;
    int tile_128x64 = 1;
    int force_tile = 0;
    int force_split = 0;
    int tail_split = 1;
    int persist = 1;
    int persist_min_nk = 32;
    int persist_min_tiles = 256;
    int persist_debug = 0;
    int stem_fused = 1;
    int lean_loader = 1;
    int fuse_shortcut = 1;
    int lanes = 1;
    int h8 = 1;
    int x8 = 1;
    int x8_min_nk = 8;
    int x8_min_rounds = 2;
    int zone_cols = 1;
    int small_n_64 = 1;
    int aspp_lanes = 1;
    int h8_narrow = 1;
    int h8_norm = 1;
    int cgnet_fused = 1;
    int dsn_fused = 0;
    int rrn_head = 1;
    int h8_min_tiles = 224;
};
extern Tuning g_tune;
extern thread_local const Tuning* t_tune;
inline const Tuning& tune() { return t_tune ? *t_tune : g_tune; }
struct TuneScope {
    const Tuning* prev;
    explicit TuneScope(const Tuning* t) : prev(t_tune) { t_tune = t; }
    ~TuneScope() { t_tune = prev; }
    TuneScope(const TuneScope&) = delete;
    TuneScope& operator=(const TuneScope&) = delete;
};
bool tuning_set(Tuning& t, int key, int value);
template <int BM, int BN, int WM, int WN> int launch_conv_persistent(ConvP p, int G, int bpc, hipStream_t st);
struct PkGrid {
    int tiles, blocks, nk, min_share;
    void report(ConvRoute* r) const { r->tiles = tiles; r->blocks = blocks; r->nk = nk; r->min_share = min_share; }
};
PkGrid conv_persistent_grid(const ConvP& p, int G, int bpc);
size_t conv_persistent_ws_floats(int BM, int BN, int bpc);
bool conv_persistent_ok(const ConvP& p);
int conv_persistent_segments(int T, int P, int nk, int min_slices, int bid, int* out4, int cap);
int conv_persistent_fixup(int T, int P, int nk, int min_slices, int xcd, int j, int* tile, int* slots, int cap);
int launch_conv_dual(ConvP p, int G, hipStream_t st, ConvRoute* dry = nullptr);
bool conv_h8_patch_takes(const ConvP& p, int G, bool norm);
int launch_conv_x8(ConvP p, int G, hipStream_t st, ConvRoute* dry = nullptr);
int launch_split_bf16x3(const float* w, long n, void* planes, hipStream_t st);
int launch_conv_h8(ConvP p, int G, hipStream_t st);
#ifdef PK_STAMPS
int pk_read_stamps(unsigned long long* dst, int n);
int pk_read_span(unsigned long long* dst, int n);
#endif
int launch_preprocess(const uint8_t* rgb, const uint8_t* depth, const float* offs, const View& x, int B, int Bcap,
                      int H, int W, const float* mean6, const float* std6, int streams, hipStream_t st);
int launch_maxpool3x3s2(const View& in, const View& out, int B, int G, hipStream_t st);
int launch_stem_conv1(const uint8_t* bgr, const uint8_t* depth, const float* offs, int B, int H, int W, int streams, const float* mean6,
                      const float* std6, const float* w, const float* scale, const float* shift, float* out, long out_gs, int es, hipStream_t st,
                      const void* wf16 = nullptr);
int launch_zero(void* p, size_t bytes, hipStream_t st);
int launch_gn_stats(const View& in, int B, int G, int groups, double* stats, hipStream_t st, bool zero = true);
int gn_pixels_per_block(int HW, int C, int B, int G, bool stats = false);
int launch_gn_apply(const View& in, const View& out, int B, int G, int groups, const double* stats,
                    const float* gamma, const float* beta, int param_gs, float eps, int relu, hipStream_t st);
int launch_bilinear(const View& in, const View& out, int B, hipStream_t st);
int launch_avgpool(const View& in, const View& out, int B, hipStream_t st);
struct PredHeads { int n; const void* in[5]; const float* w[5]; const float* bias[5]; void* sm[5]; int cout[5], q_ch0[5], act[5] ; };
int launch_predictors(const PredHeads& hs, int C, int in_cs, int es, int H, int W, float* q, int q_nch, int sm_cs, int B, hipStream_t st);
int launch_copy_channels(const View& in, const View& out, int B, hipStream_t st);
int launch_add_channels(const View& a, const View& b, const View& out, int B, hipStream_t st);
int launch_upsample_logits(const float* q, float* out, int B, int nch, int h, int w, int scale, int OH, int OW,
                           unsigned mul_mask, hipStream_t st);

int launch_normalize_depth(const void* depth, int is_float, long n, double lo, double hi, uint8_t* out3, uint8_t* zero,
                           hipStream_t st);

int inpaint_telea_u8_host(const uint8_t* img, const uint8_t* mask, int H, int W, int radius, uint8_t* out);
int inpaint_depth_u8_host(const uint8_t* depth3, int H, int W, int kernel, uint8_t* out3);
size_t inpaint_depth_ws_bytes(int B, int H, int W);
int launch_inpaint_depth(const uint8_t* depth3, int B, int H, int W, int kernel, void* ws, size_t ws_bytes, uint8_t* out3, hipStream_t st);
int launch_resize_u8(const uint8_t* src, int sh, int sw, int ch, uint8_t* dst, int dh, int dw, int linear, hipStream_t st);

int launch_lmff_preprocess(const uint8_t* bgr, const uint8_t* depth, long pixels, float* x, hipStream_t st);
int launch_dwconv3x3(const View& in, const View& out, int B, int dil, const float* w9, const float* scale,
                     const float* shift, const float* slope, hipStream_t st);
int launch_pool_s2(const View& in, const View& out, int B, int mode , hipStream_t st);
int launch_affine_prelu(const View& a, const View* b, const View& out, int B, const float* scale, const float* shift,
                        const float* slope, hipStream_t st);
int launch_pmca(const View& x, int B, const float* w2x2, const float* fc0, const float* alpha, const float* fc2, float* wts,
                double* sums , hipStream_t st);
int launch_scale_channels(const View& in, const float* wts, const View& out, int B, hipStream_t st);
int launch_mad_gate(const View& o, const View& att, float* q, int B, int C, hipStream_t st);
int launch_argmax_fg(const float* logits, int B, long HW, int nc, int cls, uint8_t* fg, hipStream_t st);
int launch_mask_overlap(const uint8_t* masks, const uint8_t* fg, int B, int K, long HW, unsigned long long* counts,
                        hipStream_t st);

int cg_joint_tiles(int H, int W);
int cg_sums_tiles(int H, int W);
int launch_cg_preprocess(const uint8_t* bgr, const uint8_t* depth, long pixels, float* x, hipStream_t st);
int launch_cg_joint(const View& x, const View& joi, int B, int dil, const float* w1, const float* s1, const float* h1, const float* a1, const float* wloc,
                    const float* wsur, const float* s2, const float* h2, const float* a2, double* partials, int tiles, hipStream_t st);
int launch_cg_sums(const View& in, int B, double* partials, int tiles, hipStream_t st);
int launch_cg_apply(const View& joi, const View* x, const View& out, int B, int hidden, const double* partials, int tiles, const float* fc0, const float* b0,
                    const float* fc2, const float* b2, float* mean, float* y, hipStream_t st);
int launch_cg_planes(const View& in, int nc, int B, float* q, hipStream_t st);
int launch_fg_overlap(const uint8_t* fg, int fh, int fw, const uint8_t* masks, int B, int K, int H, int W, unsigned long long* counts, hipStream_t st);

int esp_tiles(int H, int W);
int esp_nt(int n1);
size_t esp_packed_floats(int n1);
int launch_dsn_pack(const float* xyz, int B, int H, int W, int flags, float* x8, float* clean, hipStream_t st);
int launch_esp_pack(const float* const w[5], int n, int n1, float* packed, hipStream_t st);
int launch_esp_branches(const View& t, const View* x, const View& out, int B, int n, int n1, int groups, const float* packed, double* partials, int tiles, hipStream_t st);
int launch_esp_merge(const View d[5], const View* x, const View& out, int B, int n, int n1, int groups, double* partials, int tiles, hipStream_t st);
int launch_esp_stats(const double* partials, int B, int tiles, int groups, double* stats, hipStream_t st);
int launch_dsn_head(const View& f, int B, const float* clean, const float* wfg, const float* wcd, float* logits, float* offsets, float* votes, uint8_t* classes,
                    uint8_t* fg, hipStream_t st);

int launch_rrn_crop(const uint8_t* img, const int* ids, const int* slots, const int* rois, const float* table, int B, int n_ids, int T, int S, int H, int W,
                    float* rgb_crop, uint8_t* mask_crop, hipStream_t st);
int launch_rrn_pack(const float* rgb, const uint8_t* mask, int B, int H, int W, float* x8, hipStream_t st);
int launch_rrn_head(const View& f, int B, const float* wfg, float thr, float* logits, uint8_t* refined, hipStream_t st);
int launch_rrn_head3(const View& f, int B, const float* w9, float bias, float thr, float* logits, uint8_t* refined, hipStream_t st);
int launch_rrn_paste(const uint8_t* refined, const int* slots, const int* rois, const float* z, int B, int n_ids, int T, int S, int N, int H, int W,
                     int* out_ids, uint8_t* out_masks, int* source, float* keys, int* report, void* ws, int cap_b, hipStream_t st);
size_t rrn_paste_ws_bytes(int cap_b, int H, int W);

int launch_boundary_overlap(const int* pred, const int* gt, int H, int W, const int* labels, int n_pred, int n_gt, int radius,
                            void* ws, unsigned* out, hipStream_t st);
size_t boundary_ws_bytes(int H, int W, int n_masks);
int launch_contingency(const int* pred, const int* gt, long n, int cap, void* ws, hipStream_t st);
size_t contingency_ws_bytes(int cap);
int launch_eval_batch(const int* pred, const int* gt, int batch, int H, int W, int cap, int radius, int with_boundary, int placement, void* ws,
                      void* out, hipStream_t st);
size_t eval_batch_ws_bytes(int batch, int H, int W, int cap, int with_boundary);
size_t eval_batch_out_bytes(int batch, int cap);
int launch_munkres_batch(const double* score, const int* rows, const int* cols, int batch, int cap, int placement, double* mat, int* assign,
                         long assign_stride, int* status, long status_stride, hipStream_t st);

int launch_encode(const uint8_t* masks, int B, int N, int H, int W, const float* gauss, int sigma, int legacy_f32,
                  void* ws, float* out, hipStream_t st);
int launch_encode_labels(const int* labels, int B, int N, int H, int W, const float* gauss, int sigma, int legacy_f32, void* ws,
                         float* out, int* bad, hipStream_t st);
size_t encode_ws_bytes(int B, int N, int H, int W);

int launch_errmaps(const uint8_t* init, int N, const uint8_t* gt, int Ng, int B, int Nmax, int H, int W, int d,
                   uint8_t* ws, uint8_t* out, hipStream_t st);
size_t errmaps_ws_bytes(int B, int Nmax, int H, int W);

struct InstStat {
    double prob;
    unsigned long long sy, sx;
    unsigned cnt;
    int xmin, ymin, xmax, ymax;
    int pad;
};
int launch_post_finalize(const float* logits, int nch, int B, int H, int W, int cap, const int* count, const InstStat* stats, float* scores,
                         float* boxes, hipStream_t st);
int launch_post_paint_finalize(const float* logits, int nch, int B, int H, int W, int cap, int label_divisor, const int* ids, const float* lut,
                               const int* count, float* pan, InstStat* stats, float* scores, float* boxes, hipStream_t st);
struct PostCfg {
    float threshold;
    int nms_kernel, top_k, stuff_area, min_area, label_divisor, cap;
};
int launch_postprocess(const float* logits, int nch, int B, int H, int W, const PostCfg& c, void* ws,
                       float* pan, int* count, float* labels, float* scores, float* boxes, int* centers,
                       int* ncenters, hipStream_t st);
size_t postprocess_ws_bytes(int B, int H, int W, int cap);
int launch_extract_masks(const float* pan, const float* labels, int B, int H, int W, int cap, int max_inst,
                         uint8_t* out, hipStream_t st);
int launch_tta_flip_u8(const uint8_t* src, uint8_t* dst, long planes, int H, int W, int C, hipStream_t st);
int launch_tta_merge(const float* logits2, int planes, int B, int H, int W, float* out, hipStream_t st);
int launch_error_decode(const float* logits, int n_planes, int first_plane, int classes, int B, int H, int W, uint8_t* cls,
                        unsigned* hist, hipStream_t st);
int launch_error_mask_hist(const uint8_t* cls, const uint8_t* masks, int B, int N, int classes, int H, int W, unsigned* out,
                           hipStream_t st);
int launch_error_score(const uint8_t* cls, const uint8_t* expl, int kind, int error_type, int classes, int B, int H, int W,
                       unsigned long long* table, hipStream_t st);
int launch_error_overlay(const uint8_t* bgr, const uint8_t* cls, int B, int H, int W, const unsigned* colors, uint8_t* out,
                         hipStream_t st);
int launch_relabel_panoptic(const float* pan, const float* labels, const int* count, int B, int top_k, int mirror, int H, int W,
                            int* ids, hipStream_t st);
int launch_overlap_masks(const uint8_t* masks, const int* ids, int B, int N, int n_ids, int H, int W, unsigned* table, unsigned* area,
                         hipStream_t st);
int launch_overlap_ids(const int* a, const int* b, int B, int n_a, int n_b, int H, int W, unsigned* table, hipStream_t st);
int launch_cleanup_ids(int* ids, int B, int H, int W, int n_ids, int conn, int keep_largest, int min_island, int max_hole, void* ws,
                       unsigned* report, hipStream_t st);
int launch_cleanup_postprocess(const float* logits, int nch, int B, int H, int W, int cap, int label_divisor, float* pan, const float* labels, const int* count,
                               float* scores, float* boxes, int conn, int keep_largest, int min_island, int max_hole, void* ws,
                               unsigned* report, hipStream_t st);
size_t cleanup_ws_bytes(int B, int H, int W, int cap);
int launch_perturb(const uint8_t* masks, long n_masks, int H, int W, const int* programs, int n_ops, int ops_per_round, const double* targets,
                   uint8_t* out, unsigned* report, int lds, void* ws, hipStream_t st);
bool perturb_fits_lds(int H, int W);
size_t perturb_ws_bytes(long n_masks, int H, int W);
int launch_mask_nms(const uint8_t* masks, const float* scores, int B, int N, int H, int W, float thresh, int small_on_top, uint8_t* out_masks,
                    int* ids, int* source, float* out_scores, int* report, void* ws, hipStream_t st);
size_t mask_nms_ws_bytes(int B, int N, int H, int W);
int mask_nms_max();
struct ScenePerturbArgs {
    const uint8_t* gt; const uint8_t* props; const int* n_gt; const int* n_prop; int N; int P; int M; double min_mask_ratio;
    const uint8_t* fp_act; const uint8_t* gs_act; const uint8_t* merge_act; const uint8_t* split_act; const int* split_try;
    const uint8_t* delete_act; uint8_t* out_masks; int* info; int* report;
};
int launch_scene_perturb(const ScenePerturbArgs& q, int B, int H, int W, void* ws, hipStream_t st);
size_t scene_ws_bytes(int B, int S, int M, int H, int W);
int scene_max();
struct CocoMatchArgs {
    const uint8_t* dt; const float* scores; const double* dt_boxes; int n_dt;
    const uint8_t* gt; const uint8_t* gt_flags; const double* gt_area; const double* gt_boxes; int n_gt;
    int iou_type; const double* iou_thrs; int n_thrs; const double* area_rng; int n_rng;
    int* counts; int* order; float* out_scores; double* dt_area; double* gt_area_used; double* iou;
    uint8_t* dtm; uint8_t* dtig; uint8_t* gi; int* gorder;
};
int launch_coco_match(const CocoMatchArgs& q, int B, int H, int W, void* ws, hipStream_t st);
size_t coco_match_ws_bytes(int B, int n_gt, int H, int W, int bbox);
int coco_match_top();
int launch_meanshift_seeds(const float* X, const int* first, int B, int S, int H, int W, int* idx, void* ws, int cap_b, hipStream_t st);
int launch_meanshift_climb(const float* X, const int* idx, float* Z, int B, int S, int H, int W, float kappa, int iters, void* ws, int cap_b,
                           hipStream_t st);
int launch_meanshift_link(const float* Z, int B, int S, float eps, int* labels, hipStream_t st);
int launch_meanshift_assign(const float* X, const float* Z, const int* seed_labels, const float* depth_z, float thresh, int B, int S, int N, int H,
                            int W, int* ids, uint8_t* planes, int* report, void* ws, int cap_b, hipStream_t st);
size_t meanshift_ws_bytes(int cap_b, int H, int W);
int launch_gms_seeds(const float* votes, const uint8_t* fg, const int* first, const unsigned* draws, int B, int S, int sub, int H, int W, int* idx,
                     int* info, void* ws, int cap_b, hipStream_t st);
int launch_gms_climb(const float* votes, const uint8_t* fg, const int* idx, const int* counts, float* Z, int B, int S, int sub, int H, int W,
                     float sigma, int iters, bool compact, void* ws, int cap_b, hipStream_t st);
int launch_gms_link(const float* Z, const int* counts, int B, int S, float eps, int* labels, hipStream_t st);
int launch_gms_assign(const float* votes, const uint8_t* fg, const float* Z, const int* seed_labels, const int* counts, int B, int S, int N,
                      int min_pixels, int H, int W, int* ids, uint8_t* planes, float* centers, int* report, void* ws, int cap_b, hipStream_t st);
int launch_gms_imp(int* ids, int B, int n_ids, int ksize, int largest, int N, int H, int W, uint8_t* planes, float* centers, int* report, void* ws,
                   int cap_b, void* cleanup_ws, hipStream_t st);
int launch_gms_copy_ids(const int* src, int* dst, size_t n, hipStream_t st);
size_t gms_ws_bytes(int cap_b, int H, int W);
size_t gms_imp_lds_bytes(int H, int W);
int gms_prepare();
int launch_zoom_rois(const int* ids, int B, int n_ids, int H, int W, float padding, int* rois, void* ws, int cap_b, hipStream_t st);
int launch_zoom_crop(const uint8_t* bgr, const uint8_t* depth, const int* ids, const int* slots, const int* rois, int B, int n_ids, int T, int S,
                     int H, int W, uint8_t* bgr_crop, uint8_t* depth_crop, uint8_t* mask_crop, hipStream_t st);
int launch_zoom_paste(const int* crop_ids, const float* crop_scores, const unsigned* table, const unsigned* area, const uint8_t* depth_crop,
                      const int* slots, const int* rois, int B, int n_ids, int T, int S, int C, float min_overlap, int max_inst, int H, int W,
                      int* out_ids, uint8_t* out_masks, int* source, float* out_scores, float* boxes, int* report, void* ws, int cap_b,
                      hipStream_t st);
size_t zoom_ws_bytes(int cap_b, int H, int W);
int launch_loss_targets(const int* labels, int B, int n, int H, int W, int sigma, int small_area, float small_weight, int legacy_f32,
                        const float* gauss, float* targets, double* points, int* area, void* ws, int cap_b, hipStream_t st);
int launch_losses(const float* logits, int P, const float* targets, const uint8_t* expl, const ::quber_loss_spec& sp, int ncls, long k,
                  int B, int H, int W, double* out, void* ws, int cap_b, hipStream_t st);
size_t losses_ws_bytes(int cap_b, int H, int W);
int launch_group_pixels(const float* logits, int nch, int B, int H, int W, int cap, const int* centers, const int* ncenters,
                        uint8_t* idmap, unsigned* area, hipStream_t st);

}

#define QB_CHECK(expr)                                                                         \
    do {                                                                                       \
        hipError_t e__ = (expr);                                                               \
        if (e__ != hipSuccess)                                                                 \
            return quber::fail(std::string(#expr) + ": " + hipGetErrorString(e__));            \
    } while (0)
```

quber_amd/csrc/runtime.hip:

```cpp
#include <atomic>

#include "plan.h"

namespace quber {

Tuning g_tune;
thread_local const Tuning* t_tune = nullptr;

struct TuneKey { int key; int Tuning::*field; bool plan; };
constexpr TuneKey TUNE_KEYS[] = {
    {3, &Tuning::force_split, false},           {4, &Tuning::force_tile, false},
    {5, &Tuning::tail_split, false},            {6, &Tuning::winograd, true},
    {7, &Tuning::wino_min_cin, true},           {8, &Tuning::wino_max_ratio, true},
    {9, &Tuning::wino_variant, true},           {10, &Tuning::wino_min_cout, true},
    {13, &Tuning::persist, false},              {14, &Tuning::persist_min_nk, false},
    {15, &Tuning::persist_min_tiles, false},    {16, &Tuning::persist_debug, false},
    {17, &Tuning::wino_pairs, false},           {18, &Tuning::fuse_shortcut, true},
    {19, &Tuning::tile_128x64, false},          {20, &Tuning::wino_chunk_mb, false},
    {21, &Tuning::acc_chunk, false},            {24, &Tuning::lanes, false},
    {25, &Tuning::wino_fused, true},            {27, &Tuning::wino_fused_max_cin, true},
    {29, &Tuning::stem_fused, true},            {30, &Tuning::lean_loader, false},
    {31, &Tuning::h8, false},                   {32, &Tuning::h8_min_tiles, false},
    {35, &Tuning::x8, false},                   {36, &Tuning::x8_min_rounds, false},
    {37, &Tuning::x8_min_nk, false},            {38, &Tuning::h8_narrow, false},
    {39, &Tuning::h8_norm, true},               {41, &Tuning::aspp_lanes, true},
    {42, &Tuning::small_n_64, false},           {43, &Tuning::zone_cols, false},
    {51, &Tuning::wino_pack, true},              {52, &Tuning::cgnet_fused, true},
    {53, &Tuning::dsn_fused, true},              {54, &Tuning::rrn_head, true},
};
int* tuning_field(Tuning& t, int key) {
    for (const TuneKey& k : TUNE_KEYS)
        if (k.key == key) return &(t.*k.field);
    return nullptr;
}
bool tuning_set(Tuning& t, int key, int value) {
    int* f = tuning_field(t, key);
    if (f) *f = value;
    return f != nullptr;
}
bool tuning_plan_time(int key) {
    for (const TuneKey& k : TUNE_KEYS)
        if (k.key == key) return k.plan;
    return false;
}

int device_cus() {
    static std::atomic<int> cache[64];
    int dev = 0;
    if (hipGetDevice(&dev) != hipSuccess) return -1;
    const bool cached = dev >= 0 && dev < 64;
    if (cached) {
        const int v = cache[dev].load(std::memory_order_relaxed);
        if (v > 0) return v;
    }
    hipDeviceProp_t prop;
    if (hipGetDeviceProperties(&prop, dev) != hipSuccess) return -1;
    const int cus = prop.multiProcessorCount > 0 ? prop.multiProcessorCount : 256;
    if (cached) cache[dev].store(cus, std::memory_order_relaxed);
    return cus;
}

static thread_local std::string g_err;
extern "C" const char* quber_last_error(void) { return g_err.c_str(); }
void set_error(const std::string& m) { g_err = m; }
int fail(const std::string& m) { g_err = m; return -1; }

thread_local Profiler* g_prof = nullptr;

ProfScope::ProfScope(const char* tag, double bytes, double flops, hipStream_t s) : rec(-1), st(s) {
    Profiler* p = g_prof;
    if (!p) return;
    int ti = -1;
    for (size_t i = 0; i < p->tags.size(); ++i)
        if (p->tags[i] == tag) { ti = (int)i; break; }
    if (ti < 0) { ti = (int)p->tags.size(); p->tags.emplace_back(tag); }
    ProfRec r{ti, p->get(), p->get(), bytes, flops};
    if (!r.e0 || !r.e1 || hipEventRecord(r.e0, s) != hipSuccess) return;
    rec = (int)p->recs.size();
    p->recs.push_back(r);
}
ProfScope::~ProfScope() {
    if (rec >= 0 && g_prof) (void)hipEventRecord(g_prof->recs[rec].e1, st);
}

}
```

quber_amd/csrc/wino_fused.hip:

```cpp
#include <algorithm>

#include "common.h"
#include "winograd_xf.h"

namespace quber {


using namespace wxf;

__host__ __device__ inline long fused_src(long i, int Cout, int Cin) {
    const int e = (int)(i & 3), l = (int)((i >> 2) & 63);
    long r = i >> 8;
    const int p = (int)(r % 36);
    r /= 36;
    const int ks = (int)(r % (Cin / 8)), cc = (int)(r / (Cin / 8));
    return ((long)p * Cout + cc * 32 + (l & 31)) * Cin + ks * 8 + 4 * (l >> 5) + e;
}

namespace {

using f32x16 = __attribute__((ext_vector_type(16))) float;
using f32x4 = __attribute__((ext_vector_type(4))) float;
using f32x2 = __attribute__((ext_vector_type(2))) float;

#ifndef WF_SPLIT
#define WF_SPLIT 7
#endif
#ifndef WF_SKIP
#define WF_SKIP 0
#endif
#ifndef WF_OPT
#define WF_OPT 3
#endif
#ifdef WF_STAMPS
constexpr int WF_STAMP_BLOCKS = 512, WF_STAMP_N = 16;
__device__ unsigned long long g_wf_stamps[WF_STAMP_BLOCKS * 4 * WF_STAMP_N];
#define WF_STAMP(i) do { if (lane == 0 && blockIdx.x < WF_STAMP_BLOCKS && blockIdx.z == 0) g_wf_stamps[((int)blockIdx.x * 4 + wave) * WF_STAMP_N + (i)] = (i) == 15 ? __builtin_amdgcn_s_memrealtime() : __builtin_amdgcn_s_memtime(); } while (0)
#else
#define WF_STAMP(i) do {} while (0)
#endif
constexpr int FT = 32;
constexpr int FC = 32;
constexpr int FK = 16;
constexpr int FP = 36;
constexpr int SLICE = FP * FT * 8;
constexpr int STAGE = 2 * SLICE;
constexpr int M_FLOATS = FP * FT * FC;
constexpr int SMEM_BYTES = 2 * STAGE * 4 + 2 * 32 * 2 * 8;
static_assert(M_FLOATS == 2 * STAGE, "the epilogue image overlays the two round images");
constexpr unsigned OOBH = 0x40000000u;
constexpr int RSRC_FLAGS = 0x00020000;

__device__ __forceinline__ __amdgpu_buffer_rsrc_t make_rsrc(const void* ptr, unsigned bytes) {
    const unsigned long a = (unsigned long)ptr;
    const unsigned lo = __builtin_amdgcn_readfirstlane((unsigned)a), hi = __builtin_amdgcn_readfirstlane((unsigned)(a >> 32));
    return __builtin_amdgcn_make_buffer_rsrc(reinterpret_cast<void*>(((unsigned long)hi << 32) | lo), 0,
                                             (int)__builtin_amdgcn_readfirstlane(bytes), RSRC_FLAGS);
}
__device__ __forceinline__ f32x2 buf_load2(__amdgpu_buffer_rsrc_t r, unsigned voff, unsigned soff) {
    return __builtin_bit_cast(f32x2, __builtin_amdgcn_raw_buffer_load_b64(r, voff, soff, 0));
}
__device__ __forceinline__ void buf_store4(f32x4 v, __amdgpu_buffer_rsrc_t r, unsigned voff) {
    using u32x4 = __attribute__((ext_vector_type(4))) unsigned;
    __builtin_amdgcn_raw_buffer_store_b128(__builtin_bit_cast(u32x4, v), r, voff, 0, 0);
}
__device__ __forceinline__ f32x4 buf_load4(__amdgpu_buffer_rsrc_t r, unsigned voff, unsigned soff) {
    return __builtin_bit_cast(f32x4, __builtin_amdgcn_raw_buffer_load_b128(r, voff, soff, 0));
}

__device__ __forceinline__ f32x2 pk_fma(f32x2 a, f32x2 c, f32x2 b) {
    f32x2 d;
    asm("v_pk_fma_f32 %0, %1, %2, %3" : "=v"(d) : "v"(a), "s"(c), "v"(b));
    return d;
}
__device__ __forceinline__ f32x2 pk_fnma(f32x2 a, f32x2 c, f32x2 b) {
    f32x2 d;
    asm("v_pk_fma_f32 %0, %1, %2, %3 neg_lo:[0,1,0] neg_hi:[0,1,0]" : "=v"(d) : "v"(a), "s"(c), "v"(b));
    return d;
}
__device__ __forceinline__ f32x2 pk_fma_v(f32x2 a, f32x2 c, f32x2 b) {
    f32x2 d;
    asm("v_pk_fma_f32 %0, %1, %2, %3" : "=v"(d) : "v"(a), "v"(c), "v"(b));
    return d;
}
__device__ __forceinline__ void bt4(const f32x2* x, f32x2* y) {
    const f32x2 k225 = {2.25f, 2.25f}, k05625 = {0.5625f, 0.5625f}, k075 = {0.75f, 0.75f}, k15 = {1.5f, 1.5f};
    const f32x2 k1265625 = {1.265625f, 1.265625f}, k28125 = {2.8125f, 2.8125f};
    const f32x2 t1 = pk_fnma(x[1], k225, x[3]), e1 = pk_fnma(x[2], k225, x[4]);
    const f32x2 t2 = pk_fnma(x[1], k05625, x[3]), e2 = pk_fnma(x[2], k05625, x[4]);
    y[0] = pk_fma(x[0], k1265625, pk_fnma(x[2], k28125, x[4]));
    y[1] = pk_fma(t1, k075, e1);
    y[2] = pk_fnma(t1, k075, e1);
    y[3] = pk_fma(t2, k15, e2);
    y[4] = pk_fnma(t2, k15, e2);
    y[5] = pk_fma(x[1], k1265625, pk_fnma(x[3], k28125, x[5]));
}

struct PV { f32x2 lo, hi; };
__device__ __forceinline__ f32x2 pk_add(f32x2 a, f32x2 b) {
    f32x2 d;
    asm("v_pk_add_f32 %0, %1, %2" : "=v"(d) : "v"(a), "v"(b));
    return d;
}
__device__ __forceinline__ f32x2 pk_sub(f32x2 a, f32x2 b) {
    f32x2 d;
    asm("v_pk_add_f32 %0, %1, %2 neg_lo:[0,1] neg_hi:[0,1]" : "=v"(d) : "v"(a), "v"(b));
    return d;
}
__device__ __forceinline__ f32x2 pk_mul(f32x2 a, f32x2 c) {
    f32x2 d;
    asm("v_pk_mul_f32 %0, %1, %2" : "=v"(d) : "v"(a), "s"(c));
    return d;
}
__device__ __forceinline__ f32x2 at4_y(int o, f32x2 x0, f32x2 a, f32x2 b, f32x2 c, f32x2 d, f32x2 x5) {
    const f32x2 k075 = {0.75f, 0.75f}, k15 = {1.5f, 1.5f}, k05625 = {0.5625f, 0.5625f}, k225 = {2.25f, 2.25f};
    const f32x2 k0421875 = {0.421875f, 0.421875f}, k3375 = {3.375f, 3.375f};
    if (o == 0) return pk_add(pk_add(x0, a), c);
    if (o == 1) return pk_fma(d, k15, pk_mul(b, k075));
    if (o == 2) return pk_fma(c, k225, pk_mul(a, k05625));
    return pk_fma(b, k0421875, pk_fma(d, k3375, x5));
}
__device__ __forceinline__ void at4(const PV* x, PV* y) {
    const f32x2 al = pk_add(x[1].lo, x[2].lo), bl = pk_sub(x[1].lo, x[2].lo), cl = pk_add(x[3].lo, x[4].lo), dl = pk_sub(x[3].lo, x[4].lo);
    const f32x2 ah = pk_add(x[1].hi, x[2].hi), bh = pk_sub(x[1].hi, x[2].hi), ch = pk_add(x[3].hi, x[4].hi), dh = pk_sub(x[3].hi, x[4].hi);
#pragma unroll
    for (int o = 0; o < 4; ++o) {
        y[o].lo = at4_y(o, x[0].lo, al, bl, cl, dl, x[5].lo);
        y[o].hi = at4_y(o, x[0].hi, ah, bh, ch, dh, x[5].hi);
    }
}
__device__ __forceinline__ PV ldpv(const float* p) {
    const f32x4 t = *reinterpret_cast<const f32x4*>(p);
    return PV{f32x2{t.x, t.y}, f32x2{t.z, t.w}};
}

struct FusedArgs {
    const float* in; long in_gs; int in_cs, H, W, Cin; unsigned in_bytes;
    const float* uf; long uf_gs;
    const float* coef; long coef_gs;
    int relu_in;
    int Ball, boff, B;
    const float* scale; const float* shift; int ss_gs, relu;
    float* out; int out_cs; long out_gs; int Cout; unsigned out_bytes;
    int TH, TW, d; long tiles, per_img; int NC, NB;
    double* gn_sum; int gn_groups, gn_cpg;
};

template <bool NORM>
__global__ __launch_bounds__(256) __attribute__((amdgpu_waves_per_eu(1, 1))) void wino_fused_kernel(const FusedArgs a) {
    extern __shared__ __attribute__((aligned(16))) float smem[];
    double* const gacc = reinterpret_cast<double*>(smem + 2 * STAGE);
    const int t = threadIdx.x, lane = t & 63;
    const int wave = __builtin_amdgcn_readfirstlane(t >> 6);
    const int g = blockIdx.z;
    const int xcd = blockIdx.x & 7, bq_ = a.NB >> 3, br = a.NB & 7;
    const int vb = (xcd < br ? xcd * (bq_ + 1) : br * (bq_ + 1) + (xcd - br) * bq_) + (blockIdx.x >> 3);
    const int tb = vb / a.NC, cc = vb - tb * a.NC;
    if (t < 128) gacc[t] = 0.0;
    WF_STAMP(0);
    WF_STAMP(15);

    const int lt = t >> 3, q = t & 7;
    const long tile = (long)tb * FT + lt;
    const bool tvalid = tile < a.tiles;
    const TileAt ta = locate32(tvalid ? (unsigned)tile : 0u, (unsigned)a.TH, (unsigned)a.TW, (unsigned)a.d);
    const int y0 = a.d * (4 * ta.ty - 1) + ta.py, x0 = a.d * (4 * ta.tx - 1) + ta.px;
    const unsigned pix = (unsigned)a.in_cs * 4u;
    const unsigned base = (unsigned)((ta.b * a.H + y0) * a.W + x0) * pix + (unsigned)q * 8u;
    unsigned rowbase[6], colterm[6];
    bool edge = false;
#pragma unroll
    for (int i = 0; i < 6; ++i) {
        const bool ok = tvalid && (unsigned)(y0 + i * a.d) < (unsigned)a.H;
        rowbase[i] = ok ? base + (unsigned)(i * a.d * a.W) * pix : OOBH;
        edge |= !ok;
    }
#pragma unroll
    for (int j = 0; j < 6; ++j) {
        const bool ok = (unsigned)(x0 + j * a.d) < (unsigned)a.W;
        colterm[j] = ok ? (unsigned)(j * a.d) * pix : OOBH;
        edge |= !ok;
    }
    const bool border = NORM && __any(edge);
    const float relu_lo = a.relu_in ? 0.f : -__builtin_inff();
    const __amdgpu_buffer_rsrc_t rs_in = make_rsrc(a.in + (long)g * a.in_gs, a.in_bytes);
    const int nslice = a.Cin / 8;
    const __amdgpu_buffer_rsrc_t rs_u = make_rsrc(a.uf + (long)g * a.uf_gs + (long)cc * nslice * (FP * 256), (unsigned)nslice * (FP * 1024u));
    const float* coef = NORM ? a.coef + (long)g * a.coef_gs + ((long)(a.boff + ta.b) * a.Cin + 2 * q) * 2 : nullptr;

    f32x2 dd[6][6];
    f32x4 cf = {1.f, 0.f, 1.f, 0.f};
    const int R = a.Cin / FK;
    auto gload_row = [&](int i, int r) __attribute__((always_inline)) {
        const unsigned so = (unsigned)r * (FK * 4u);
#pragma unroll
        for (int j = 0; j < 6; ++j) {
#if (WF_SKIP & 1)
            asm volatile("" : "+v"(dd[i][j]) : "s"(so));
#else
            dd[i][j] = buf_load2(rs_in, rowbase[i] + colterm[j], so);
#endif
        }
    };
    auto gload_coef = [&](int r) __attribute__((always_inline)) {
        if constexpr (NORM) cf = *reinterpret_cast<const f32x4*>(coef + (long)r * (FK * 2));
    };
    auto col_pass = [&](int j) __attribute__((always_inline)) {
        f32x2 col[6], tc[6];
#pragma unroll
        for (int i = 0; i < 6; ++i) {
            f32x2 v = dd[i][j];
            if constexpr (NORM) {
                v = pk_fma_v(v, f32x2{cf.x, cf.z}, f32x2{cf.y, cf.w});
                v.x = fmaxf(v.x, relu_lo); v.y = fmaxf(v.y, relu_lo);
            }
            col[i] = v;
        }
        if constexpr (NORM) {
            if (border) {
                asm volatile("");
#pragma unroll
                for (int i = 0; i < 6; ++i)
                    if (rowbase[i] == OOBH || colterm[j] == OOBH) col[i] = f32x2{0.f, 0.f};
            }
        }
        bt4(col, tc);
#pragma unroll
        for (int i = 0; i < 6; ++i) dd[i][j] = tc[i];
    };
    auto row_pass = [&](int i, float* vs) __attribute__((always_inline)) {
        float* dst = vs + (q >> 2) * SLICE + lt * 8 + 2 * (q & 3);
        f32x2 row[6];
        bt4(dd[i], row);
#pragma unroll
        for (int j = 0; j < 6; ++j) *reinterpret_cast<f32x2*>(dst + (i * 6 + j) * (FT * 8)) = row[j];
    };

    constexpr int SPLIT = WF_SPLIT;
    f32x16 acc[2][9];
    const f32x16 zero = {0.f, 0.f, 0.f, 0.f, 0.f, 0.f, 0.f, 0.f, 0.f, 0.f, 0.f, 0.f, 0.f, 0.f, 0.f, 0.f};
    const int a_off = (wave * 9) * (FT * 8) + (lane & 31) * 8 + (lane >> 5) * 4;
    const unsigned b_voff = (unsigned)lane * 16u;
    const unsigned b_pos = (unsigned)(wave * 9) * 1024u;
    constexpr int BR = 6;
    f32x4 bq[BR];
    auto bload = [&](int slot, int r, int kk) __attribute__((always_inline)) {
        const int sl = 2 * r + kk / 9, pi = kk % 9;
#if (WF_SKIP & 2)
        asm volatile("" : "+v"(bq[slot]) : "s"(sl));
#else
        bq[slot] = buf_load4(rs_u, sl < nslice ? b_voff : 0x80000000u, (unsigned)sl * (FP * 1024u) + b_pos + (unsigned)pi * 1024u);
#endif
    };
    auto round = [&](const float* vs, float* vn, const int r, const int kbase, const bool first) __attribute__((always_inline)) {
        const int r2 = r + 2 < R ? r + 2 : R - 1;
        f32x4 av_next = *reinterpret_cast<const f32x4*>(vs + a_off);
#pragma unroll
        for (int k = 0; k < 18; ++k) {
            const int s = k / 9, pi = k % 9;
            const f32x4 av = av_next;
            if (k + 1 < 18) av_next = *reinterpret_cast<const f32x4*>(vs + ((k + 1) / 9) * SLICE + a_off + ((k + 1) % 9) * (FT * 8));
            const f32x4 bv = bq[(kbase + k) % BR];
#if (WF_SKIP & 16)
            acc[pi < SPLIT ? s : 0][pi][0] += av.x * bv.x + av.y * bv.y + av.z * bv.z + av.w * bv.w;
#else
            f32x16& ac = acc[pi < SPLIT ? s : 0][pi];
#if (WF_OPT & 2)
            ac = __builtin_amdgcn_mfma_f32_32x32x2f32(bv.x, av.x, (first && (s == 0 || pi < SPLIT)) ? zero : ac, 0, 0, 0);
            ac = __builtin_amdgcn_mfma_f32_32x32x2f32(bv.y, av.y, ac, 0, 0, 0);
            ac = __builtin_amdgcn_mfma_f32_32x32x2f32(bv.z, av.z, ac, 0, 0, 0);
            ac = __builtin_amdgcn_mfma_f32_32x32x2f32(bv.w, av.w, ac, 0, 0, 0);
#else
            ac = __builtin_amdgcn_mfma_f32_32x32x2f32(av.x, bv.x, (first && (s == 0 || pi < SPLIT)) ? zero : ac, 0, 0, 0);
            ac = __builtin_amdgcn_mfma_f32_32x32x2f32(av.y, bv.y, ac, 0, 0, 0);
            ac = __builtin_amdgcn_mfma_f32_32x32x2f32(av.z, bv.z, ac, 0, 0, 0);
            ac = __builtin_amdgcn_mfma_f32_32x32x2f32(av.w, bv.w, ac, 0, 0, 0);
#endif
#endif
            bload((kbase + k) % BR, r, k + BR);
#if !(WF_SKIP & 4)
            if (k < 6) { row_pass(k, vn); gload_row(k, r2); }
            if (k == 6) gload_coef(r2);
            if (k >= 12) col_pass(k - 12);
#endif
            __builtin_amdgcn_sched_barrier(0);
        }
    };

    float* const st0 = smem;
    float* const st1 = smem + STAGE;
    {
        f32x2 d1[6][6];
        const unsigned so1 = (unsigned)(R > 1 ? 1 : 0) * (FK * 4u);
#pragma unroll
        for (int i = 0; i < 6; ++i) gload_row(i, 0);
#pragma unroll
        for (int i = 0; i < 6; ++i)
#pragma unroll
            for (int j = 0; j < 6; ++j) d1[i][j] = buf_load2(rs_in, rowbase[i] + colterm[j], so1);
        gload_coef(0);
#pragma unroll
        for (int g0 = 0; g0 < BR; ++g0) bload(g0, 0, g0);
#pragma unroll
        for (int j = 0; j < 6; ++j) col_pass(j);
#pragma unroll
        for (int i = 0; i < 6; ++i) row_pass(i, st0);
#pragma unroll
        for (int i = 0; i < 6; ++i)
#pragma unroll
            for (int j = 0; j < 6; ++j) dd[i][j] = d1[i][j];
    }
    gload_coef(R > 1 ? 1 : 0);
#pragma unroll
    for (int j = 0; j < 6; ++j) col_pass(j);
    __syncthreads();
    static_assert(36 % BR == 0, "the ring index is static over a pair of rounds");
    WF_STAMP(1);
    round(st0, st1, 0, 0, true);
    __syncthreads();
    WF_STAMP(2);
    round(st1, st0, 1, 18, false);
    __syncthreads();
    WF_STAMP(3);
    for (int r = 2; r < ((WF_SKIP & 64) ? 0 : R); r += 2) {
        round(st0, st1, r, 0, false);
        __syncthreads();
        round(st1, st0, r + 1, 18, false);
        __syncthreads();
    }
    WF_STAMP(6);

#if (WF_SKIP & 32)
    if (acc[0][0][0] != 12345.f) return;
#endif
    const int h = lane >> 5, rr = lane & 31;
#if (WF_OPT & 2)
#pragma unroll
    for (int pi = 0; pi < 9; ++pi)
#pragma unroll
        for (int g4 = 0; g4 < 4; ++g4) {
            f32x4 v;
#pragma unroll
            for (int e = 0; e < 4; ++e) v[e] = pi < SPLIT ? acc[0][pi][4 * g4 + e] + acc[1][pi][4 * g4 + e] : acc[0][pi][4 * g4 + e];
            *reinterpret_cast<f32x4*>(smem + ((wave * 9 + pi) * FT + rr) * FC + (((2 * g4 + h) ^ ((rr >> 1) & 7)) << 2)) = v;
        }
#else
#pragma unroll
    for (int pi = 0; pi < 9; ++pi)
#pragma unroll
        for (int e = 0; e < 16; ++e)
            smem[((wave * 9 + pi) * FT + 8 * (e >> 2) + 4 * h + (e & 3)) * FC + rr] = pi < SPLIT ? acc[0][pi][e] + acc[1][pi][e] : acc[0][pi][e];
#endif
    __syncthreads();
    WF_STAMP(7);
    const int c = cc * FC + 4 * q;
#if (WF_OPT & 2)
    const int csw = (q ^ ((lt >> 1) & 7)) << 2;
#else
    const int csw = 4 * q;
#endif
    PV s[4][6];
#pragma unroll
    for (int j = 0; j < 6; ++j) {
        PV col[6], sj[4];
#pragma unroll
        for (int i = 0; i < 6; ++i) col[i] = ldpv(smem + ((i * 6 + j) * FT + lt) * FC + csw);
        at4(col, sj);
#pragma unroll
        for (int i = 0; i < 4; ++i) s[i][j] = sj[i];
    }
    PV sc = {f32x2{1.f, 1.f}, f32x2{1.f, 1.f}}, sh = {f32x2{0.f, 0.f}, f32x2{0.f, 0.f}};
    if (a.scale) {
        sc = ldpv(a.scale + g * a.ss_gs + c);
        sh = ldpv(a.shift + g * a.ss_gs + c);
    }
    const float lo = a.relu ? 0.f : -__builtin_inff();
    const int b0 = (int)(((long)tb * FT) / a.per_img);
    double sa = 0.0, sq = 0.0;
#if (WF_OPT & 4)
    f32x2 psa = {0.f, 0.f}, psq = {0.f, 0.f};
#endif
    const __amdgpu_buffer_rsrc_t rs_out = make_rsrc(a.out + (long)g * a.out_gs, a.out_bytes);
    const unsigned opix = (unsigned)a.out_cs * 4u;
    const int oy0 = a.d * 4 * ta.ty + ta.py, ox0 = a.d * 4 * ta.tx + ta.px;
    const unsigned obase = (unsigned)((ta.b * a.H + oy0) * a.W + ox0) * opix + (unsigned)c * 4u;
    unsigned orow[4], ocol[4];
#pragma unroll
    for (int i = 0; i < 4; ++i) {
        orow[i] = (tvalid && oy0 + i * a.d < a.H) ? obase + (unsigned)(i * a.d * a.W) * opix : OOBH;
        ocol[i] = (ox0 + i * a.d < a.W) ? (unsigned)(i * a.d) * opix : OOBH;
    }
#pragma unroll
    for (int i = 0; i < 4; ++i) {
        PV row[4];
        at4(s[i], row);
#pragma unroll
        for (int j = 0; j < 4; ++j) {
            const f32x2 yl = pk_fma_v(row[j].lo, sc.lo, sh.lo), yh = pk_fma_v(row[j].hi, sc.hi, sh.hi);
            const f32x4 y = {fmaxf(yl.x, lo), fmaxf(yl.y, lo), fmaxf(yh.x, lo), fmaxf(yh.y, lo)};
            const unsigned vo = orow[i] + ocol[j];
            if (a.gn_sum) {
                if (vo < OOBH) {
#if (WF_OPT & 4)
                    const f32x2 y01 = {y.x, y.y}, y23 = {y.z, y.w};
                    psa = pk_add(pk_add(psa, y01), y23);
                    psq = pk_fma_v(y23, y23, pk_fma_v(y01, y01, psq));
#else
#pragma unroll
                    for (int e = 0; e < 4; ++e) { sa += (double)y[e]; sq += (double)y[e] * y[e]; }
#endif
                }
            }
            buf_store4(y, rs_out, vo);
        }
    }
    WF_STAMP(8);
    if (a.gn_sum) {
#if (WF_OPT & 4)
        sa = (double)psa.x + (double)psa.y;
        sq = (double)psq.x + (double)psq.y;
#endif
        if (tvalid && (sa != 0.0 || sq != 0.0)) {
            const int grp = c / a.gn_cpg, o = ta.b == b0 ? 0 : 64;
            atomicAdd(&gacc[o + grp * 2], sa);
            atomicAdd(&gacc[o + grp * 2 + 1], sq);
        }
        __syncthreads();
        if (t < 128) {
            const double v = gacc[t];
            const int b = b0 + (t >> 6);
            if (v != 0.0 && b < a.B) atomicAdd(&a.gn_sum[(((long)g * a.Ball + a.boff + b) * a.gn_groups) * 2 + (t & 63)], v);
        }
    }
    WF_STAMP(9);
#ifdef WF_STAMPS
    if (lane == 0 && blockIdx.x < WF_STAMP_BLOCKS && blockIdx.z == 0) {
        g_wf_stamps[((int)blockIdx.x * 4 + wave) * WF_STAMP_N + 14] = __builtin_amdgcn_s_memrealtime();
        g_wf_stamps[((int)blockIdx.x * 4 + wave) * WF_STAMP_N + 13] = ((unsigned long long)__builtin_amdgcn_s_getreg(63508) << 32) | __builtin_amdgcn_s_getreg(63492);
    }
#endif
}


namespace w64 {
constexpr int FT = 16, FC = 64, FK = 32;
constexpr int SLICE = FP * FT * 16;
constexpr int STAGE = 2 * SLICE;
static_assert(FP * FT * FC == 2 * STAGE, "the epilogue image overlays the two round images");
constexpr int SMEM_BYTES = 2 * STAGE * 4 + 2 * 32 * 2 * 8;
}

__host__ __device__ inline bool fused_wide(int Cout, int Cin) { return Cout % 64 == 0 && ((Cin / 32) % 2 == 0 || (Cin == 32 && (WF_OPT & 1))); }
__host__ __device__ inline long fused64_src(long i, int Cout, int Cin) {
    const int e = (int)(i & 3), l = (int)((i >> 2) & 63), nt = (int)((i >> 8) & 3);
    long r = i >> 10;
    const int p = (int)(r % 36);
    r /= 36;
    const int ks = (int)(r % (Cin / 16)), cc = (int)(r / (Cin / 16));
    return ((long)p * Cout + cc * 64 + nt * 16 + (l & 15)) * Cin + ks * 16 + 4 * (l >> 4) + e;
}

template <bool NORM, bool ONE = false>
__global__ __launch_bounds__(256) __attribute__((amdgpu_waves_per_eu(1, 1))) void wino_fused64_kernel(const FusedArgs a) {
    constexpr int FT = w64::FT, FC = w64::FC, FK = w64::FK, SLICE = w64::SLICE, STAGE = w64::STAGE;
    extern __shared__ __attribute__((aligned(16))) float smem[];
    double* const gacc = reinterpret_cast<double*>(smem + 2 * STAGE);
    const int t = threadIdx.x, lane = t & 63;
    const int wave = __builtin_amdgcn_readfirstlane(t >> 6);
    const int g = blockIdx.z;
    const int xcd = blockIdx.x & 7, bq_ = a.NB >> 3, br = a.NB & 7;
    const int vb = (xcd < br ? xcd * (bq_ + 1) : br * (bq_ + 1) + (xcd - br) * bq_) + (blockIdx.x >> 3);
    const int tb = vb / a.NC, cc = vb - tb * a.NC;
    if (t < 128) gacc[t] = 0.0;
    WF_STAMP(0);
    WF_STAMP(15);

    const int lt = t >> 4, q = t & 15;
    const long tile = (long)tb * FT + lt;
    const bool tvalid = tile < a.tiles;
    const TileAt ta = locate32(tvalid ? (unsigned)tile : 0u, (unsigned)a.TH, (unsigned)a.TW, (unsigned)a.d);
    const int y0 = a.d * (4 * ta.ty - 1) + ta.py, x0 = a.d * (4 * ta.tx - 1) + ta.px;
    const unsigned pix = (unsigned)a.in_cs * 4u;
    const unsigned base = (unsigned)((ta.b * a.H + y0) * a.W + x0) * pix + (unsigned)q * 8u;
    unsigned rowbase[6], colterm[6];
    bool edge = false;
#pragma unroll
    for (int i = 0; i < 6; ++i) {
        const bool ok = tvalid && (unsigned)(y0 + i * a.d) < (unsigned)a.H;
        rowbase[i] = ok ? base + (unsigned)(i * a.d * a.W) * pix : OOBH;
        edge |= !ok;
    }
#pragma unroll
    for (int j = 0; j < 6; ++j) {
        const bool ok = (unsigned)(x0 + j * a.d) < (unsigned)a.W;
        colterm[j] = ok ? (unsigned)(j * a.d) * pix : OOBH;
        edge |= !ok;
    }
    const bool border = NORM && __any(edge);
    const float relu_lo = a.relu_in ? 0.f : -__builtin_inff();
    const __amdgpu_buffer_rsrc_t rs_in = make_rsrc(a.in + (long)g * a.in_gs, a.in_bytes);
    const int nslice = a.Cin / 16;
    const __amdgpu_buffer_rsrc_t rs_u = make_rsrc(a.uf + (long)g * a.uf_gs + (long)cc * nslice * (FP * 1024), (unsigned)nslice * (FP * 4096u));
    const float* coef = NORM ? a.coef + (long)g * a.coef_gs + ((long)(a.boff + ta.b) * a.Cin + 2 * q) * 2 : nullptr;

    f32x2 dd[6][6];
    f32x4 cf = {1.f, 0.f, 1.f, 0.f};
    const int R = a.Cin / FK;
    auto gload_row = [&](int i, int r) __attribute__((always_inline)) {
        const unsigned so = (unsigned)r * (FK * 4u);
#pragma unroll
        for (int j = 0; j < 6; ++j) dd[i][j] = buf_load2(rs_in, rowbase[i] + colterm[j], so);
    };
    auto gload_coef = [&](int r) __attribute__((always_inline)) {
        if constexpr (NORM) cf = *reinterpret_cast<const f32x4*>(coef + (long)r * (FK * 2));
    };
    auto col_pass = [&](int j) __attribute__((always_inline)) {
        f32x2 col[6], tc[6];
#pragma unroll
        for (int i = 0; i < 6; ++i) {
            f32x2 v = dd[i][j];
            if constexpr (NORM) {
                v = pk_fma_v(v, f32x2{cf.x, cf.z}, f32x2{cf.y, cf.w});
                v.x = fmaxf(v.x, relu_lo); v.y = fmaxf(v.y, relu_lo);
            }
            col[i] = v;
        }
        if constexpr (NORM) {
            if (border) {
                asm volatile("");
#pragma unroll
                for (int i = 0; i < 6; ++i)
                    if (rowbase[i] == OOBH || colterm[j] == OOBH) col[i] = f32x2{0.f, 0.f};
            }
        }
        bt4(col, tc);
#pragma unroll
        for (int i = 0; i < 6; ++i) dd[i][j] = tc[i];
    };
    auto row_pass = [&](int i, float* vs) __attribute__((always_inline)) {
        float* dst = vs + (q >> 3) * SLICE + lt * 16 + 2 * (q & 7);
        f32x2 row[6];
        bt4(dd[i], row);
#pragma unroll
        for (int j = 0; j < 6; ++j) *reinterpret_cast<f32x2*>(dst + (i * 6 + j) * (FT * 16)) = row[j];
    };

    constexpr int SPLIT = WF_SPLIT;
    f32x4 acc[2][9][4];
    const f32x4 zero = {0.f, 0.f, 0.f, 0.f};
    const int a_off = (wave * 9) * (FT * 16) + (lane & 15) * 16 + (lane >> 4) * 4;
    const unsigned b_voff = (unsigned)lane * 16u;
    const unsigned b_pos = (unsigned)(wave * 9) * 4096u;
    constexpr int BR = 3;
    f32x4 bq[BR][4];
    auto bload = [&](int slot, int r, int kk) __attribute__((always_inline)) {
        const int sl = 2 * r + kk / 9, pi = kk % 9;
        const unsigned vo = sl < nslice ? b_voff : 0x80000000u;
        const unsigned so = (unsigned)sl * (FP * 4096u) + b_pos + (unsigned)pi * 4096u;
#pragma unroll
        for (int nt = 0; nt < 4; ++nt) bq[slot][nt] = buf_load4(rs_u, vo + nt * 1024u, so);
    };
    auto round = [&](const float* vs, float* vn, const int r, const int kbase, const bool first) __attribute__((always_inline)) {
        const int r2 = r + 2 < R ? r + 2 : R - 1;
        const bool do_rows = !(WF_OPT & 1) || r + 1 < R, do_full = !(WF_OPT & 1) || r + 2 < R;
        f32x4 av_next = *reinterpret_cast<const f32x4*>(vs + a_off);
#pragma unroll
        for (int k = 0; k < 18; ++k) {
            const int s2 = k / 9, pi = k % 9;
            const f32x4 av = av_next;
            if (k + 1 < 18) av_next = *reinterpret_cast<const f32x4*>(vs + ((k + 1) / 9) * SLICE + a_off + ((k + 1) % 9) * (FT * 16));
            f32x4 bv[4];
#pragma unroll
            for (int nt = 0; nt < 4; ++nt) bv[nt] = bq[(kbase + k) % BR][nt];
#pragma unroll
            for (int e = 0; e < 4; ++e)
#pragma unroll
                for (int nt = 0; nt < 4; ++nt) {
                    f32x4& ac = acc[pi < SPLIT ? s2 : 0][pi][nt];
                    const f32x4 c0 = (first && e == 0 && (s2 == 0 || pi < SPLIT)) ? zero : ac;
#if (WF_OPT & 2)
                    ac = __builtin_amdgcn_mfma_f32_16x16x4f32(bv[nt][e], av[e], c0, 0, 0, 0);
#else
                    ac = __builtin_amdgcn_mfma_f32_16x16x4f32(av[e], bv[nt][e], c0, 0, 0, 0);
#endif
                }
            bload((kbase + k) % BR, r, k + BR);
            if (k < 6 && do_rows) row_pass(k, vn);
            if (do_full) {
                if (k < 6) gload_row(k, r2);
                if (k == 6) gload_coef(r2);
                if (k >= 12) col_pass(k - 12);
            }
            __builtin_amdgcn_sched_barrier(0);
        }
    };

    float* const st0 = smem;
    float* const st1 = smem + STAGE;
    const int r1 = R > 1 ? 1 : 0;
    static_assert(36 % BR == 0, "the ring index is static over a pair of rounds");
    if constexpr (ONE) {
#pragma unroll
        for (int i = 0; i < 6; ++i) gload_row(i, 0);
        gload_coef(0);
#pragma unroll
        for (int g0 = 0; g0 < BR; ++g0) bload(g0, 0, g0);
#pragma unroll
        for (int j = 0; j < 6; ++j) col_pass(j);
#pragma unroll
        for (int i = 0; i < 6; ++i) row_pass(i, st0);
        __syncthreads();
        WF_STAMP(1);
        round(st0, st1, 0, 0, true);
        __syncthreads();
    } else {
    {
        f32x2 d1[6][6];
        const unsigned so1 = (unsigned)r1 * (FK * 4u);
#pragma unroll
        for (int i = 0; i < 6; ++i) gload_row(i, 0);
#pragma unroll
        for (int i = 0; i < 6; ++i)
#pragma unroll
            for (int j = 0; j < 6; ++j) d1[i][j] = buf_load2(rs_in, rowbase[i] + colterm[j], so1);
        gload_coef(0);
#pragma unroll
        for (int g0 = 0; g0 < BR; ++g0) bload(g0, 0, g0);
#pragma unroll
        for (int j = 0; j < 6; ++j) col_pass(j);
#pragma unroll
        for (int i = 0; i < 6; ++i) row_pass(i, st0);
#pragma unroll
        for (int i = 0; i < 6; ++i)
#pragma unroll
            for (int j = 0; j < 6; ++j) dd[i][j] = d1[i][j];
    }
    gload_coef(r1);
#pragma unroll
    for (int j = 0; j < 6; ++j) col_pass(j);
    __syncthreads();
    WF_STAMP(1);
    round(st0, st1, 0, 0, true);
    __syncthreads();
    WF_STAMP(2);
    round(st1, st0, 1, 18, false);
    __syncthreads();
    WF_STAMP(3);
    for (int r = 2; r < R; r += 2) {
        round(st0, st1, r, 0, false);
        __syncthreads();
        round(st1, st0, r + 1, 18, false);
        __syncthreads();
    }
    }
    WF_STAMP(6);

    const int hq = lane >> 4, rr = lane & 15;
#if (WF_OPT & 2)
#pragma unroll
    for (int pi = 0; pi < 9; ++pi)
#pragma unroll
        for (int nt = 0; nt < 4; ++nt) {
            const f32x4 v = pi < SPLIT ? acc[0][pi][nt] + acc[1][pi][nt] : acc[0][pi][nt];
            *reinterpret_cast<f32x4*>(smem + ((wave * 9 + pi) * FT + rr) * FC + (((nt * 4 + hq) ^ rr) << 2)) = v;
        }
#else
#pragma unroll
    for (int pi = 0; pi < 9; ++pi)
#pragma unroll
        for (int nt = 0; nt < 4; ++nt)
#pragma unroll
            for (int e = 0; e < 4; ++e)
                smem[((wave * 9 + pi) * FT + 4 * hq + e) * FC + ((nt ^ hq) << 4) + rr] = pi < SPLIT ? acc[0][pi][nt][e] + acc[1][pi][nt][e] : acc[0][pi][nt][e];
#endif
    __syncthreads();
    WF_STAMP(7);
    const int c = cc * FC + 4 * q;
#if (WF_OPT & 2)
    const int csw = ((q ^ lt) & 15) << 2;
#else
    const int csw = (((q >> 2) ^ ((lt >> 2) & 3)) << 4) + (q & 3) * 4;
#endif
    PV s[4][6];
#pragma unroll
    for (int j = 0; j < 6; ++j) {
        PV col[6], sj[4];
#pragma unroll
        for (int i = 0; i < 6; ++i) col[i] = ldpv(smem + ((i * 6 + j) * FT + lt) * FC + csw);
        at4(col, sj);
#pragma unroll
        for (int i = 0; i < 4; ++i) s[i][j] = sj[i];
    }
    PV sc = {f32x2{1.f, 1.f}, f32x2{1.f, 1.f}}, sh = {f32x2{0.f, 0.f}, f32x2{0.f, 0.f}};
    if (a.scale) {
        sc = ldpv(a.scale + g * a.ss_gs + c);
        sh = ldpv(a.shift + g * a.ss_gs + c);
    }
    const float lo = a.relu ? 0.f : -__builtin_inff();
    const int b0 = (int)(((long)tb * FT) / a.per_img);
    double sa = 0.0, sq = 0.0;
#if (WF_OPT & 4)
    f32x2 psa = {0.f, 0.f}, psq = {0.f, 0.f};
#endif
    const __amdgpu_buffer_rsrc_t rs_out = make_rsrc(a.out + (long)g * a.out_gs, a.out_bytes);
    const unsigned opix = (unsigned)a.out_cs * 4u;
    const int oy0 = a.d * 4 * ta.ty + ta.py, ox0 = a.d * 4 * ta.tx + ta.px;
    const unsigned obase = (unsigned)((ta.b * a.H + oy0) * a.W + ox0) * opix + (unsigned)c * 4u;
    unsigned orow[4], ocol[4];
#pragma unroll
    for (int i = 0; i < 4; ++i) {
        orow[i] = (tvalid && oy0 + i * a.d < a.H) ? obase + (unsigned)(i * a.d * a.W) * opix : OOBH;
        ocol[i] = (ox0 + i * a.d < a.W) ? (unsigned)(i * a.d) * opix : OOBH;
    }
#pragma unroll
    for (int i = 0; i < 4; ++i) {
        PV row[4];
        at4(s[i], row);
#pragma unroll
        for (int j = 0; j < 4; ++j) {
            const f32x2 yl = pk_fma_v(row[j].lo, sc.lo, sh.lo), yh = pk_fma_v(row[j].hi, sc.hi, sh.hi);
            const f32x4 y = {fmaxf(yl.x, lo), fmaxf(yl.y, lo), fmaxf(yh.x, lo), fmaxf(yh.y, lo)};
            const unsigned vo = orow[i] + ocol[j];
            if (a.gn_sum) {
                if (vo < OOBH) {
#if (WF_OPT & 4)
                    const f32x2 y01 = {y.x, y.y}, y23 = {y.z, y.w};
                    psa = pk_add(pk_add(psa, y01), y23);
                    psq = pk_fma_v(y23, y23, pk_fma_v(y01, y01, psq));
#else
#pragma unroll
                    for (int e = 0; e < 4; ++e) { sa += (double)y[e]; sq += (double)y[e] * y[e]; }
#endif
                }
            }
            buf_store4(y, rs_out, vo);
        }
    }
    WF_STAMP(8);
    if (a.gn_sum) {
#if (WF_OPT & 4)
        sa = (double)psa.x + (double)psa.y;
        sq = (double)psq.x + (double)psq.y;
#endif
        if (tvalid && (sa != 0.0 || sq != 0.0)) {
            const int grp = c / a.gn_cpg, o = ta.b == b0 ? 0 : 64;
            atomicAdd(&gacc[o + grp * 2], sa);
            atomicAdd(&gacc[o + grp * 2 + 1], sq);
        }
        __syncthreads();
        if (t < 128) {
            const double v = gacc[t];
            const int b = b0 + (t >> 6);
            if (v != 0.0 && b < a.B) atomicAdd(&a.gn_sum[(((long)g * a.Ball + a.boff + b) * a.gn_groups) * 2 + (t & 63)], v);
        }
    }
    WF_STAMP(9);
#ifdef WF_STAMPS
    if (lane == 0 && blockIdx.x < WF_STAMP_BLOCKS && blockIdx.z == 0) {
        g_wf_stamps[((int)blockIdx.x * 4 + wave) * WF_STAMP_N + 14] = __builtin_amdgcn_s_memrealtime();
        g_wf_stamps[((int)blockIdx.x * 4 + wave) * WF_STAMP_N + 13] = ((unsigned long long)__builtin_amdgcn_s_getreg(63508) << 32) | __builtin_amdgcn_s_getreg(63492);
    }
#endif
}

__global__ void wino_norm_coef_kernel(const WinoNorm np, int G, int Ball, int Cin, float* __restrict__ coef) {
    const long n = (long)G * Ball * Cin;
    for (long i = blockIdx.x * (long)blockDim.x + threadIdx.x; i < n; i += (long)gridDim.x * blockDim.x) {
        const int c = (int)(i % Cin);
        const long gb = i / Cin;
        const int g = (int)(gb / Ball);
        const double* sb = np.stats + (gb * np.groups + c / np.cpg) * 2;
        const double mean = sb[0] / np.n;
        double var = sb[1] / np.n - mean * mean;
        if (var < 0.0) var = 0.0;
        const float rstd = (float)(1.0 / sqrt(var + (double)np.eps));
        const float sc = rstd * np.gamma[g * np.param_gs + c];
        coef[i * 2] = sc;
        coef[i * 2 + 1] = np.beta[g * np.param_gs + c] - (float)mean * sc;
    }
}

__global__ void wino_pack_fused_kernel(const float* __restrict__ u, int Cout, int Cin, float* __restrict__ uf) {
    const long n = (long)FP * Cout * Cin;
    for (long i = blockIdx.x * (long)blockDim.x + threadIdx.x; i < n; i += (long)gridDim.x * blockDim.x)
        uf[i] = u[fused_wide(Cout, Cin) ? fused64_src(i, Cout, Cin) : fused_src(i, Cout, Cin)];
}

}

void winograd_fused_pack_host(const float* u, int Cout, int Cin, float* uf) {
    const long n = (long)FP * Cout * Cin;
    for (long i = 0; i < n; ++i) uf[i] = u[fused_wide(Cout, Cin) ? fused64_src(i, Cout, Cin) : fused_src(i, Cout, Cin)];
}

int launch_winograd_fused_pack(const float* u, int Cout, int Cin, float* uf, hipStream_t st) {
    hipLaunchKernelGGL(wino_pack_fused_kernel, dim3(512), dim3(256), 0, st, u, Cout, Cin, uf);
    QB_CHECK(hipGetLastError());
    return 0;
}

bool winograd_fused_ok(const WinoP& q, int Ball, int G) {
    const View& in = q.in;
    const View& out = q.out;
    if (!tune().wino_fused || q.m != 4 || (q.dtype != 0 && q.dtype != 3) || !q.uf || in.es != 4 || out.es != 4) return false;
    if (q.dtype == 3 && G > 1 && in.gs == 0 && out.C >= 64) return false;
    if (in.C % 32 || out.C % FC) return false;
    if (in.p == out.p) return false;
    if (in.C > tune().wino_fused_max_cin) return false;
    const double in_bytes = 4.0 * (((double)Ball * in.H * in.W - 1) * in.cs + in.C);
    const double out_bytes = 4.0 * (((double)Ball * in.H * in.W - 1) * out.cs + out.C);
    if (in_bytes > (double)0x3F000000u || out_bytes > (double)0x3F000000u) return false;
    if ((long)q.dil * in.W * in.cs * 4 * 6 > (1L << 26)) return false;
    return true;
}

size_t winograd_fused_ws_floats(int B, int Cin, int G) { return (size_t)2 * G * B * Cin; }

int winograd_fused_prepare() {
    QB_CHECK(hipFuncSetAttribute((const void*)wino_fused_kernel<true>, hipFuncAttributeMaxDynamicSharedMemorySize, SMEM_BYTES));
    QB_CHECK(hipFuncSetAttribute((const void*)wino_fused_kernel<false>, hipFuncAttributeMaxDynamicSharedMemorySize, SMEM_BYTES));
    QB_CHECK(hipFuncSetAttribute((const void*)wino_fused64_kernel<true>, hipFuncAttributeMaxDynamicSharedMemorySize, w64::SMEM_BYTES));
    QB_CHECK(hipFuncSetAttribute((const void*)wino_fused64_kernel<false>, hipFuncAttributeMaxDynamicSharedMemorySize, w64::SMEM_BYTES));
    QB_CHECK(hipFuncSetAttribute((const void*)wino_fused64_kernel<true, true>, hipFuncAttributeMaxDynamicSharedMemorySize, w64::SMEM_BYTES));
    QB_CHECK(hipFuncSetAttribute((const void*)wino_fused64_kernel<false, true>, hipFuncAttributeMaxDynamicSharedMemorySize, w64::SMEM_BYTES));
    return 0;
}

#ifdef WF_STAMPS
int wf_read_stamps(unsigned long long* dst, int n) {
    if (n > WF_STAMP_BLOCKS * 4 * WF_STAMP_N) n = WF_STAMP_BLOCKS * 4 * WF_STAMP_N;
    QB_CHECK(hipMemcpyFromSymbol(dst, HIP_SYMBOL(g_wf_stamps), sizeof(unsigned long long) * n));
    return 0;
}
#endif

static bool fused_gn_here(const WinoP& q, int Cout, long tiles_per_image, int ft) {
    return q.gn_sum && q.gn_groups > 0 && q.gn_groups <= 32 && (Cout / q.gn_groups) % 4 == 0 && tiles_per_image >= ft;
}

int launch_conv_winograd_fused(const WinoP& q, int Ball, int G, hipStream_t st, ConvRoute* dry) {
    const View& in = q.in;
    const View& out = q.out;
    const int H = in.H, W = in.W, d = q.dil;
    FusedArgs a{};
    a.in = in.p; a.in_gs = in.gs; a.in_cs = in.cs; a.H = H; a.W = W; a.Cin = in.C;
    a.in_bytes = (unsigned)(4 * (((long)Ball * H * W - 1) * in.cs + in.C));
    a.uf = q.uf; a.uf_gs = (long)FP * out.C * in.C;
    a.Ball = Ball; a.boff = 0; a.B = Ball;
    a.scale = q.scale; a.shift = q.shift; a.ss_gs = q.ss_gs; a.relu = q.relu;
    a.out = out.p; a.out_cs = out.cs; a.out_gs = out.gs; a.Cout = out.C;
    a.out_bytes = (unsigned)(4 * (((long)Ball * H * W - 1) * out.cs + out.C));
    a.TH = tiles_1d(H, d, 4); a.TW = tiles_1d(W, d, 4); a.d = d;
    a.per_img = wino_tiles(H, W, d, 4);
    a.tiles = (long)Ball * a.per_img;
    const bool wide = fused_wide(out.C, in.C);
    const int ft = wide ? w64::FT : FT;
    a.NC = out.C / (wide ? w64::FC : FC);
    const long tblocks = (a.tiles + ft - 1) / ft;
    if (tblocks * a.NC >= (1L << 31) || a.tiles + 64 >= (1L << 31)) return fail("winograd (fused): too many blocks");
    a.NB = (int)(tblocks * a.NC);
    const bool gn_here = fused_gn_here(q, out.C, a.per_img, ft);
    if (dry) {
        dry->kernel = ROUTE_WINO_FUSED; dry->sums = !q.gn_sum ? 0 : gn_here ? ROUTE_WINO_FUSED : ROUTE_SEPARATE;
        dry->BM = ft; dry->BN = wide ? w64::FC : FC; dry->S = 1; dry->tail_shift = 0; dry->tiles = (int)a.per_img; dry->blocks = a.NB;
        return 0;
    }
    a.gn_sum = gn_here ? q.gn_sum : nullptr; a.gn_groups = q.gn_groups; a.gn_cpg = q.gn_groups ? out.C / q.gn_groups : 1;
    const bool norm = q.norm.stats != nullptr;
    if (norm) {
        WinoNorm np = q.norm;
        if (np.groups <= 0 || in.C % np.groups) return fail("winograd (fused): GroupNorm groups do not divide the channels");
        np.cpg = in.C / np.groups;
        np.n = (double)H * W * np.cpg;
        if (winograd_fused_ws_floats(Ball, in.C, G) > q.ws_floats) return fail("winograd (fused): workspace too small");
        const long n = (long)G * Ball * in.C;
        hipLaunchKernelGGL(wino_norm_coef_kernel, dim3((unsigned)((n + 255) / 256)), dim3(256), 0, st, np, G, Ball, in.C, q.ws);
        QB_CHECK(hipGetLastError());
        a.coef = q.ws; a.coef_gs = (long)Ball * in.C * 2; a.relu_in = np.relu;
    }
    {
        ProfScope prof(q.dtype == 3 ? "conv_gemm_f32pipe" : "wino_fused", 4.0 * G * ((double)Ball * H * W * (in.C + out.C) + (double)FP * in.C * out.C),
                       2.0 * G * FP * (double)a.tiles * in.C * out.C, st);
        const void* fn32 = norm ? (const void*)wino_fused_kernel<true> : (const void*)wino_fused_kernel<false>;
        const void* fn64 = in.C == 32 ? (norm ? (const void*)wino_fused64_kernel<true, true> : (const void*)wino_fused64_kernel<false, true>)
                                      : (norm ? (const void*)wino_fused64_kernel<true> : (const void*)wino_fused64_kernel<false>);
        const void* fn = wide ? fn64 : fn32;
        const int smem_bytes = wide ? w64::SMEM_BYTES : SMEM_BYTES;
        void* args[] = {(void*)&a};
        QB_CHECK(hipLaunchKernel(fn, dim3(a.NB, 1, G), dim3(256), args, smem_bytes, st));
    }
    QB_CHECK(hipGetLastError());
    if (q.gn_sum && !gn_here) return launch_gn_stats(out, Ball, G, q.gn_groups, q.gn_sum, st, false);
    return 0;
}

}
```

Baseline: 10180 refined masks/s.

## Make fused Winograd kernel persistent with next-tile prefetch during epilogue

Converts the fused Winograd conv kernels into a persistent, XCD-aware walk: the launch is capped at one block per CU (for non-norm, narrow or Cin=32 cases), and each block iterates over several virtual tile blocks. During the output epilogue of one item, the block locates and issues global loads for the next item, so input and filter loading overlaps with output transform and store. The change adds loop-carried state, per-iteration GN accumulator resets and extra register pressure. It also exposes a debug walk function and tuning keys.

```diff
diff --git a/include/quber_hip.h b/include/quber_hip.h
--- a/include/quber_hip.h
+++ b/include/quber_hip.h
@@ -244,6 +244,7 @@
                                         int32_t* out4, int32_t cap);
 int32_t quber_debug_persistent_fixup(int32_t tiles, int32_t blocks, int32_t k_slices, int32_t min_share, int32_t xcd, int32_t j,
                                      int32_t* tile, int32_t* slots, int32_t cap);
+int32_t quber_debug_wino_fused_walk(int32_t NB, int32_t blocks, int32_t block, int32_t* items, int32_t cap);
 int64_t quber_debug_ws_bytes(int32_t which, int32_t b, int32_t n, int32_t m, int32_t h, int32_t w, int32_t flag);
 int quber_num_ops(quber_ctx* ctx);
 int quber_op_info(quber_ctx* ctx, int index, const char** name, int32_t* kind, double* flops, int32_t* launches);
diff --git a/quber_amd/_lib.py b/quber_amd/_lib.py
--- a/quber_amd/_lib.py
+++ b/quber_amd/_lib.py
@@ -108,6 +108,7 @@
     "quber_op_info": (C.c_int, [_P, C.c_int, C.POINTER(C.c_char_p), C.POINTER(_I), C.POINTER(C.c_double), C.POINTER(_I)]),
     "quber_debug_persistent_segments": (C.c_int32, [_I, _I, _I, _I, _I, _P, _I]),
     "quber_debug_persistent_fixup": (C.c_int32, [_I, _I, _I, _I, _I, _I, _P, _P, _I]),
+    "quber_debug_wino_fused_walk": (C.c_int32, [_I, _I, _I, _P, _I]),
     "quber_debug_ws_bytes": (C.c_int64, [_I, _I, _I, _I, _I, _I, _I]),
     "quber_op_conv1x1_f16": (C.c_int, [_P, _I, _I, _I, _I, _P, _I, _P, _P, _P, _I, _P, _P]),
     "quber_op_conv2d_f16": (C.c_int, [_P, _I, _I, _I, _I, _P, _I, _I, _I, _I, _I, _I, _P, _P, _P, _I, _P, _I, _P, _P]),
diff --git a/quber_amd/csrc/api.hip b/quber_amd/csrc/api.hip
--- a/quber_amd/csrc/api.hip
+++ b/quber_amd/csrc/api.hip
@@ -249,6 +249,10 @@
     return quber::conv_persistent_fixup(tiles, blocks, k_slices, min_share, xcd, j, tile, slots, cap);
 }
 
+int32_t quber_debug_wino_fused_walk(int32_t NB, int32_t blocks, int32_t block, int32_t* items, int32_t cap) {
+    return quber::winograd_fused_walk(NB, blocks, block, items, cap);
+}
+
 int64_t quber_debug_ws_bytes(int32_t which, int32_t b, int32_t n, int32_t m, int32_t h, int32_t w, int32_t flag) {
     switch (which) {
     case 0: return (int64_t)mask_nms_ws_bytes(b, n, h, w);
diff --git a/quber_amd/csrc/common.h b/quber_amd/csrc/common.h
--- a/quber_amd/csrc/common.h
+++ b/quber_amd/csrc/common.h
@@ -148,6 +148,7 @@
 int launch_winograd_fused_pack(const float* u, int Cout, int Cin, float* uf, hipStream_t st);
 size_t winograd_fused_ws_floats(int B, int Cin, int G);
 int winograd_fused_prepare();
+int winograd_fused_walk(int NB, int blocks, int block, int* items, int cap);
 
 struct Tuning {
     int winograd = 0;
@@ -160,6 +161,8 @@
     int wino_pack = 1;
     int wino_fused = 1;
     int wino_fused_max_cin = 160;
+    int wino_fused_walk = 1;
+    int wino_fused_blocks = 0;
     int acc_chunk = 2;
     int tile_128x64 = 1;
     int force_tile = 0;
diff --git a/quber_amd/csrc/runtime.hip b/quber_amd/csrc/runtime.hip
--- a/quber_amd/csrc/runtime.hip
+++ b/quber_amd/csrc/runtime.hip
@@ -27,6 +27,7 @@
     {42, &Tuning::small_n_64, false},           {43, &Tuning::zone_cols, false},
     {51, &Tuning::wino_pack, true},              {52, &Tuning::cgnet_fused, true},
     {53, &Tuning::dsn_fused, true},              {54, &Tuning::rrn_head, true},
+    {55, &Tuning::wino_fused_walk, false},       {56, &Tuning::wino_fused_blocks, false},
 };
 int* tuning_field(Tuning& t, int key) {
     for (const TuneKey& k : TUNE_KEYS)
diff --git a/quber_amd/csrc/wino_fused.hip b/quber_amd/csrc/wino_fused.hip
--- a/quber_amd/csrc/wino_fused.hip
+++ b/quber_amd/csrc/wino_fused.hip
@@ -15,6 +15,13 @@
     r /= 36;
     const int ks = (int)(r % (Cin / 8)), cc = (int)(r / (Cin / 8));
     return ((long)p * Cout + cc * 32 + (l & 31)) * Cin + ks * 8 + 4 * (l >> 5) + e;
+}
+
+struct FusedWalk { int first, step, end; };
+__host__ __device__ inline FusedWalk fused_walk(int NB, int blocks, int block) {
+    const int xcd = block & 7, q = NB >> 3, r = NB & 7;
+    const int start = xcd < r ? xcd * (q + 1) : r * (q + 1) + (xcd - r) * q;
+    return FusedWalk{start + (block >> 3), (blocks >> 3) + (xcd < (blocks & 7) ? 1 : 0), start + q + (xcd < r ? 1 : 0)};
 }
 
 namespace {
@@ -146,47 +153,58 @@
     double* gn_sum; int gn_groups, gn_cpg;
 };
 
-template <bool NORM>
+template <bool NORM, bool WALK>
 __global__ __launch_bounds__(256) __attribute__((amdgpu_waves_per_eu(1, 1))) void wino_fused_kernel(const FusedArgs a) {
     extern __shared__ __attribute__((aligned(16))) float smem[];
     double* const gacc = reinterpret_cast<double*>(smem + 2 * STAGE);
     const int t = threadIdx.x, lane = t & 63;
     const int wave = __builtin_amdgcn_readfirstlane(t >> 6);
     const int g = blockIdx.z;
-    const int xcd = blockIdx.x & 7, bq_ = a.NB >> 3, br = a.NB & 7;
-    const int vb = (xcd < br ? xcd * (bq_ + 1) : br * (bq_ + 1) + (xcd - br) * bq_) + (blockIdx.x >> 3);
-    const int tb = vb / a.NC, cc = vb - tb * a.NC;
+    const FusedWalk wk = fused_walk(a.NB, (int)gridDim.x, (int)blockIdx.x);
+    if (WALK && wk.first >= wk.end) return;
     if (t < 128) gacc[t] = 0.0;
     WF_STAMP(0);
     WF_STAMP(15);
 
     const int lt = t >> 3, q = t & 7;
-    const long tile = (long)tb * FT + lt;
-    const bool tvalid = tile < a.tiles;
-    const TileAt ta = locate32(tvalid ? (unsigned)tile : 0u, (unsigned)a.TH, (unsigned)a.TW, (unsigned)a.d);
-    const int y0 = a.d * (4 * ta.ty - 1) + ta.py, x0 = a.d * (4 * ta.tx - 1) + ta.px;
     const unsigned pix = (unsigned)a.in_cs * 4u;
-    const unsigned base = (unsigned)((ta.b * a.H + y0) * a.W + x0) * pix + (unsigned)q * 8u;
-    unsigned rowbase[6], colterm[6];
-    bool edge = false;
-#pragma unroll
-    for (int i = 0; i < 6; ++i) {
-        const bool ok = tvalid && (unsigned)(y0 + i * a.d) < (unsigned)a.H;
-        rowbase[i] = ok ? base + (unsigned)(i * a.d * a.W) * pix : OOBH;
-        edge |= !ok;
-    }
-#pragma unroll
-    for (int j = 0; j < 6; ++j) {
-        const bool ok = (unsigned)(x0 + j * a.d) < (unsigned)a.W;
-        colterm[j] = ok ? (unsigned)(j * a.d) * pix : OOBH;
-        edge |= !ok;
-    }
-    const bool border = NORM && __any(edge);
     const float relu_lo = a.relu_in ? 0.f : -__builtin_inff();
     const __amdgpu_buffer_rsrc_t rs_in = make_rsrc(a.in + (long)g * a.in_gs, a.in_bytes);
     const int nslice = a.Cin / 8;
-    const __amdgpu_buffer_rsrc_t rs_u = make_rsrc(a.uf + (long)g * a.uf_gs + (long)cc * nslice * (FP * 256), (unsigned)nslice * (FP * 1024u));
-    const float* coef = NORM ? a.coef + (long)g * a.coef_gs + ((long)(a.boff + ta.b) * a.Cin + 2 * q) * 2 : nullptr;
+    int tb, cc;
+    bool tvalid, border;
+    TileAt ta;
+    unsigned rowbase[6], colterm[6];
+    __amdgpu_buffer_rsrc_t rs_u;
+    const float* coef = nullptr;
+    auto locate = [&](int vb, bool live) __attribute__((always_inline)) {
+        unsigned TH = (unsigned)a.TH, TW = (unsigned)a.TW, dil = (unsigned)a.d;
+        int NC = a.NC, gl = g;
+        if constexpr (WALK) asm volatile("" : "+s"(TH), "+s"(TW), "+s"(dil), "+s"(NC), "+s"(gl));
+        tb = vb / NC; cc = vb - tb * NC;
+        const long tile = (long)tb * FT + lt;
+        tvalid = live && tile < a.tiles;
+        ta = locate32(tvalid ? (unsigned)tile : 0u, TH, TW, dil);
+        const int y0 = a.d * (4 * ta.ty - 1) + ta.py, x0 = a.d * (4 * ta.tx - 1) + ta.px;
+        const unsigned base = (unsigned)((ta.b * a.H + y0) * a.W + x0) * pix + (unsigned)q * 8u;
+        bool edge = false;
+#pragma unroll
+        for (int i = 0; i < 6; ++i) {
+            const bool ok = tvalid && (unsigned)(y0 + i * a.d) < (unsigned)a.H;
+            rowbase[i] = ok ? base + (unsigned)(i * a.d * a.W) * pix : OOBH;
+            edge |= !ok;
+        }
+#pragma unroll
+        for (int j = 0; j < 6; ++j) {
+            const bool ok = (unsigned)(x0 + j * a.d) < (unsigned)a.W;
+            colterm[j] = ok ? (unsigned)(j * a.d) * pix : OOBH;
+            edge |= !ok;
+        }
+        border = NORM && __any(edge);
+        rs_u = make_rsrc(a.uf + (long)gl * a.uf_gs + (long)cc * nslice * (FP * 256), live ? (unsigned)nslice * (FP * 1024u) : 0u);
+        if constexpr (NORM) coef = a.coef + (long)gl * a.coef_gs + ((long)(a.boff + ta.b) * a.Cin + 2 * q) * 2;
+    };
+    locate(wk.first, true);
 
     f32x2 dd[6][6];
     f32x4 cf = {1.f, 0.f, 1.f, 0.f};
@@ -289,27 +307,36 @@
 
     float* const st0 = smem;
     float* const st1 = smem + STAGE;
+    f32x2 d1[6][6];
+    auto request = [&]() __attribute__((always_inline)) {
+#pragma unroll
+        for (int i = 0; i < 6; ++i) gload_row(i, 0);
+        gload_coef(0);
+    };
+    request();
+    for (int vb = wk.first;;) {
+    WF_STAMP(5);
+#pragma unroll
+    for (int g0 = 0; g0 < BR; ++g0) bload(g0, 0, g0);
     {
-        f32x2 d1[6][6];
         const unsigned so1 = (unsigned)(R > 1 ? 1 : 0) * (FK * 4u);
 #pragma unroll
-        for (int i = 0; i < 6; ++i) gload_row(i, 0);
-#pragma unroll
         for (int i = 0; i < 6; ++i)
 #pragma unroll
             for (int j = 0; j < 6; ++j) d1[i][j] = buf_load2(rs_in, rowbase[i] + colterm[j], so1);
-        gload_coef(0);
-#pragma unroll
-        for (int g0 = 0; g0 < BR; ++g0) bload(g0, 0, g0);
-#pragma unroll
-        for (int j = 0; j < 6; ++j) col_pass(j);
-#pragma unroll
-        for (int i = 0; i < 6; ++i) row_pass(i, st0);
-#pragma unroll
-        for (int i = 0; i < 6; ++i)
-#pragma unroll
-            for (int j = 0; j < 6; ++j) dd[i][j] = d1[i][j];
-    }
+    }
+#ifdef WF_STAMPS
+    asm volatile("s_waitcnt vmcnt(0)" ::: "memory");
+#endif
+    WF_STAMP(4);
+#pragma unroll
+    for (int j = 0; j < 6; ++j) col_pass(j);
+#pragma unroll
+    for (int i = 0; i < 6; ++i) row_pass(i, st0);
+#pragma unroll
+    for (int i = 0; i < 6; ++i)
+#pragma unroll
+        for (int j = 0; j < 6; ++j) dd[i][j] = d1[i][j];
     gload_coef(R > 1 ? 1 : 0);
 #pragma unroll
     for (int j = 0; j < 6; ++j) col_pass(j);
@@ -329,11 +356,15 @@
         __syncthreads();
     }
     WF_STAMP(6);
+    int et = t, ge = g, relu_e = a.relu;
+    unsigned per_img_e = (unsigned)a.per_img, cpg_e = (unsigned)a.gn_cpg;
+    if constexpr (WALK) asm volatile("" : "+v"(et), "+s"(ge), "+s"(relu_e), "+s"(per_img_e), "+s"(cpg_e));
+    const int elane = et & 63, elt = et >> 3, eq = et & 7;
 
 #if (WF_SKIP & 32)
     if (acc[0][0][0] != 12345.f) return;
 #endif
-    const int h = lane >> 5, rr = lane & 31;
+    const int h = elane >> 5, rr = elane & 31;
 #if (WF_OPT & 2)
 #pragma unroll
     for (int pi = 0; pi < 9; ++pi)
@@ -353,34 +384,24 @@
 #endif
     __syncthreads();
     WF_STAMP(7);
-    const int c = cc * FC + 4 * q;
+    const int c = cc * FC + 4 * eq;
 #if (WF_OPT & 2)
-    const int csw = (q ^ ((lt >> 1) & 7)) << 2;
-#else
-    const int csw = 4 * q;
-#endif
-    PV s[4][6];
-#pragma unroll
-    for (int j = 0; j < 6; ++j) {
-        PV col[6], sj[4];
-#pragma unroll
-        for (int i = 0; i < 6; ++i) col[i] = ldpv(smem + ((i * 6 + j) * FT + lt) * FC + csw);
-        at4(col, sj);
-#pragma unroll
-        for (int i = 0; i < 4; ++i) s[i][j] = sj[i];
-    }
+    const int csw = (eq ^ ((elt >> 1) & 7)) << 2;
+#else
+    const int csw = 4 * eq;
+#endif
     PV sc = {f32x2{1.f, 1.f}, f32x2{1.f, 1.f}}, sh = {f32x2{0.f, 0.f}, f32x2{0.f, 0.f}};
     if (a.scale) {
-        sc = ldpv(a.scale + g * a.ss_gs + c);
-        sh = ldpv(a.shift + g * a.ss_gs + c);
-    }
-    const float lo = a.relu ? 0.f : -__builtin_inff();
-    const int b0 = (int)(((long)tb * FT) / a.per_img);
+        sc = ldpv(a.scale + ge * a.ss_gs + c);
+        sh = ldpv(a.shift + ge * a.ss_gs + c);
+    }
+    const float lo = relu_e ? 0.f : -__builtin_inff();
+    const int b0 = (int)((unsigned)(tb * FT) / per_img_e);
     double sa = 0.0, sq = 0.0;
 #if (WF_OPT & 4)
     f32x2 psa = {0.f, 0.f}, psq = {0.f, 0.f};
 #endif
-    const __amdgpu_buffer_rsrc_t rs_out = make_rsrc(a.out + (long)g * a.out_gs, a.out_bytes);
+    const __amdgpu_buffer_rsrc_t rs_out = make_rsrc(a.out + (long)ge * a.out_gs, a.out_bytes);
     const unsigned opix = (unsigned)a.out_cs * 4u;
     const int oy0 = a.d * 4 * ta.ty + ta.py, ox0 = a.d * 4 * ta.tx + ta.px;
     const unsigned obase = (unsigned)((ta.b * a.H + oy0) * a.W + ox0) * opix + (unsigned)c * 4u;
@@ -389,6 +410,23 @@
     for (int i = 0; i < 4; ++i) {
         orow[i] = (tvalid && oy0 + i * a.d < a.H) ? obase + (unsigned)(i * a.d * a.W) * opix : OOBH;
         ocol[i] = (ox0 + i * a.d < a.W) ? (unsigned)(i * a.d) * opix : OOBH;
+    }
+    const int gslot = a.gn_sum && tvalid ? (ta.b == b0 ? 0 : 64) + (int)((unsigned)c / cpg_e) * 2 : -1;
+    const int vnext = vb + wk.step;
+    const bool more = WALK && vnext < wk.end;
+    if constexpr (WALK) {
+        locate(vnext, more);
+        request();
+    }
+    PV s[4][6];
+#pragma unroll
+    for (int j = 0; j < 6; ++j) {
+        PV col[6], sj[4];
+#pragma unroll
+        for (int i = 0; i < 6; ++i) col[i] = ldpv(smem + ((i * 6 + j) * FT + elt) * FC + csw);
+        at4(col, sj);
+#pragma unroll
+        for (int i = 0; i < 4; ++i) s[i][j] = sj[i];
     }
 #pragma unroll
     for (int i = 0; i < 4; ++i) {
@@ -420,19 +458,24 @@
         sa = (double)psa.x + (double)psa.y;
         sq = (double)psq.x + (double)psq.y;
 #endif
-        if (tvalid && (sa != 0.0 || sq != 0.0)) {
-            const int grp = c / a.gn_cpg, o = ta.b == b0 ? 0 : 64;
-            atomicAdd(&gacc[o + grp * 2], sa);
-            atomicAdd(&gacc[o + grp * 2 + 1], sq);
+        if (gslot >= 0 && (sa != 0.0 || sq != 0.0)) {
+            atomicAdd(&gacc[gslot], sa);
+            atomicAdd(&gacc[gslot + 1], sq);
         }
         __syncthreads();
-        if (t < 128) {
-            const double v = gacc[t];
-            const int b = b0 + (t >> 6);
-            if (v != 0.0 && b < a.B) atomicAdd(&a.gn_sum[(((long)g * a.Ball + a.boff + b) * a.gn_groups) * 2 + (t & 63)], v);
-        }
+        if (et < 128) {
+            const double v = gacc[et];
+            const int b = b0 + (et >> 6);
+            if (v != 0.0 && b < a.B) atomicAdd(&a.gn_sum[(((long)ge * a.Ball + a.boff + b) * a.gn_groups) * 2 + (et & 63)], v);
+            if (more) gacc[et] = 0.0;
+        }
+    } else if (more) {
+        __syncthreads();
     }
     WF_STAMP(9);
+    if (!more) break;
+    vb = vnext;
+    }
 #ifdef WF_STAMPS
     if (lane == 0 && blockIdx.x < WF_STAMP_BLOCKS && blockIdx.z == 0) {
         g_wf_stamps[((int)blockIdx.x * 4 + wave) * WF_STAMP_N + 14] = __builtin_amdgcn_s_memrealtime();
@@ -460,7 +503,7 @@
     return ((long)p * Cout + cc * 64 + nt * 16 + (l & 15)) * Cin + ks * 16 + 4 * (l >> 4) + e;
 }
 
-template <bool NORM, bool ONE = false>
+template <bool NORM, bool ONE, bool WALK>
 __global__ __launch_bounds__(256) __attribute__((amdgpu_waves_per_eu(1, 1))) void wino_fused64_kernel(const FusedArgs a) {
     constexpr int FT = w64::FT, FC = w64::FC, FK = w64::FK, SLICE = w64::SLICE, STAGE = w64::STAGE;
     extern __shared__ __attribute__((aligned(16))) float smem[];
@@ -468,40 +511,51 @@
     const int t = threadIdx.x, lane = t & 63;
     const int wave = __builtin_amdgcn_readfirstlane(t >> 6);
     const int g = blockIdx.z;
-    const int xcd = blockIdx.x & 7, bq_ = a.NB >> 3, br = a.NB & 7;
-    const int vb = (xcd < br ? xcd * (bq_ + 1) : br * (bq_ + 1) + (xcd - br) * bq_) + (blockIdx.x >> 3);
-    const int tb = vb / a.NC, cc = vb - tb * a.NC;
+    const FusedWalk wk = fused_walk(a.NB, (int)gridDim.x, (int)blockIdx.x);
+    if (WALK && wk.first >= wk.end) return;
     if (t < 128) gacc[t] = 0.0;
     WF_STAMP(0);
     WF_STAMP(15);
 
     const int lt = t >> 4, q = t & 15;
-    const long tile = (long)tb * FT + lt;
-    const bool tvalid = tile < a.tiles;
-    const TileAt ta = locate32(tvalid ? (unsigned)tile : 0u, (unsigned)a.TH, (unsigned)a.TW, (unsigned)a.d);
-    const int y0 = a.d * (4 * ta.ty - 1) + ta.py, x0 = a.d * (4 * ta.tx - 1) + ta.px;
     const unsigned pix = (unsigned)a.in_cs * 4u;
-    const unsigned base = (unsigned)((ta.b * a.H + y0) * a.W + x0) * pix + (unsigned)q * 8u;
-    unsigned rowbase[6], colterm[6];
-    bool edge = false;
-#pragma unroll
-    for (int i = 0; i < 6; ++i) {
-        const bool ok = tvalid && (unsigned)(y0 + i * a.d) < (unsigned)a.H;
-        rowbase[i] = ok ? base + (unsigned)(i * a.d * a.W) * pix : OOBH;
-        edge |= !ok;
-    }
-#pragma unroll
-    for (int j = 0; j < 6; ++j) {
-        const bool ok = (unsigned)(x0 + j * a.d) < (unsigned)a.W;
-        colterm[j] = ok ? (unsigned)(j * a.d) * pix : OOBH;
-        edge |= !ok;
-    }
-    const bool border = NORM && __any(edge);
     const float relu_lo = a.relu_in ? 0.f : -__builtin_inff();
     const __amdgpu_buffer_rsrc_t rs_in = make_rsrc(a.in + (long)g * a.in_gs, a.in_bytes);
     const int nslice = a.Cin / 16;
-    const __amdgpu_buffer_rsrc_t rs_u = make_rsrc(a.uf + (long)g * a.uf_gs + (long)cc * nslice * (FP * 1024), (unsigned)nslice * (FP * 4096u));
-    const float* coef = NORM ? a.coef + (long)g * a.coef_gs + ((long)(a.boff + ta.b) * a.Cin + 2 * q) * 2 : nullptr;
+    int tb, cc;
+    bool tvalid, border;
+    TileAt ta;
+    unsigned rowbase[6], colterm[6];
+    __amdgpu_buffer_rsrc_t rs_u;
+    const float* coef = nullptr;
+    auto locate = [&](int vb, bool live) __attribute__((always_inline)) {
+        unsigned TH = (unsigned)a.TH, TW = (unsigned)a.TW, dil = (unsigned)a.d;
+        int NC = a.NC, gl = g;
+        if constexpr (WALK) asm volatile("" : "+s"(TH), "+s"(TW), "+s"(dil), "+s"(NC), "+s"(gl));
+        tb = vb / NC; cc = vb - tb * NC;
+        const long tile = (long)tb * FT + lt;
+        tvalid = live && tile < a.tiles;
+        ta = locate32(tvalid ? (unsigned)tile : 0u, TH, TW, dil);
+        const int y0 = a.d * (4 * ta.ty - 1) + ta.py, x0 = a.d * (4 * ta.tx - 1) + ta.px;
+        const unsigned base = (unsigned)((ta.b * a.H + y0) * a.W + x0) * pix + (unsigned)q * 8u;
+        bool edge = false;
+#pragma unroll
+        for (int i = 0; i < 6; ++i) {
+            const bool ok = tvalid && (unsigned)(y0 + i * a.d) < (unsigned)a.H;
+            rowbase[i] = ok ? base + (unsigned)(i * a.d * a.W) * pix : OOBH;
+            edge |= !ok;
+        }
+#pragma unroll
+        for (int j = 0; j < 6; ++j) {
+            const bool ok = (unsigned)(x0 + j * a.d) < (unsigned)a.W;
+            colterm[j] = ok ? (unsigned)(j * a.d) * pix : OOBH;
+            edge |= !ok;
+        }
+        border = NORM && __any(edge);
+        rs_u = make_rsrc(a.uf + (long)gl * a.uf_gs + (long)cc * nslice * (FP * 1024), live ? (unsigned)nslice * (FP * 4096u) : 0u);
+        if constexpr (NORM) coef = a.coef + (long)gl * a.coef_gs + ((long)(a.boff + ta.b) * a.Cin + 2 * q) * 2;
+    };
+    locate(wk.first, true);
 
     f32x2 dd[6][6];
     f32x4 cf = {1.f, 0.f, 1.f, 0.f};
@@ -599,12 +653,29 @@
     float* const st1 = smem + STAGE;
     const int r1 = R > 1 ? 1 : 0;
     static_assert(36 % BR == 0, "the ring index is static over a pair of rounds");
-    if constexpr (ONE) {
+    f32x2 d1[ONE ? 1 : 6][ONE ? 1 : 6];
+    auto request = [&]() __attribute__((always_inline)) {
 #pragma unroll
         for (int i = 0; i < 6; ++i) gload_row(i, 0);
         gload_coef(0);
-#pragma unroll
-        for (int g0 = 0; g0 < BR; ++g0) bload(g0, 0, g0);
+    };
+    request();
+    for (int vb = wk.first;;) {
+    WF_STAMP(5);
+#pragma unroll
+    for (int g0 = 0; g0 < BR; ++g0) bload(g0, 0, g0);
+    if constexpr (!ONE) {
+        const unsigned so1 = (unsigned)r1 * (FK * 4u);
+#pragma unroll
+        for (int i = 0; i < 6; ++i)
+#pragma unroll
+            for (int j = 0; j < 6; ++j) d1[i][j] = buf_load2(rs_in, rowbase[i] + colterm[j], so1);
+    }
+#ifdef WF_STAMPS
+    asm volatile("s_waitcnt vmcnt(0)" ::: "memory");
+#endif
+    WF_STAMP(4);
+    if constexpr (ONE) {
 #pragma unroll
         for (int j = 0; j < 6; ++j) col_pass(j);
 #pragma unroll
@@ -614,27 +685,14 @@
         round(st0, st1, 0, 0, true);
         __syncthreads();
     } else {
-    {
-        f32x2 d1[6][6];
-        const unsigned so1 = (unsigned)r1 * (FK * 4u);
-#pragma unroll
-        for (int i = 0; i < 6; ++i) gload_row(i, 0);
-#pragma unroll
-        for (int i = 0; i < 6; ++i)
-#pragma unroll
-            for (int j = 0; j < 6; ++j) d1[i][j] = buf_load2(rs_in, rowbase[i] + colterm[j], so1);
-        gload_coef(0);
-#pragma unroll
-        for (int g0 = 0; g0 < BR; ++g0) bload(g0, 0, g0);
-#pragma unroll
-        for (int j = 0; j < 6; ++j) col_pass(j);
-#pragma unroll
-        for (int i = 0; i < 6; ++i) row_pass(i, st0);
-#pragma unroll
-        for (int i = 0; i < 6; ++i)
-#pragma unroll
-            for (int j = 0; j < 6; ++j) dd[i][j] = d1[i][j];
-    }
+#pragma unroll
+    for (int j = 0; j < 6; ++j) col_pass(j);
+#pragma unroll
+    for (int i = 0; i < 6; ++i) row_pass(i, st0);
+#pragma unroll
+    for (int i = 0; i < 6; ++i)
+#pragma unroll
+        for (int j = 0; j < 6; ++j) dd[i][j] = d1[i][j];
     gload_coef(r1);
 #pragma unroll
     for (int j = 0; j < 6; ++j) col_pass(j);
@@ -654,8 +712,12 @@
     }
     }
     WF_STAMP(6);
-
-    const int hq = lane >> 4, rr = lane & 15;
+    int et = t, ge = g, relu_e = a.relu;
+    unsigned per_img_e = (unsigned)a.per_img, cpg_e = (unsigned)a.gn_cpg;
+    if constexpr (WALK) asm volatile("" : "+v"(et), "+s"(ge), "+s"(relu_e), "+s"(per_img_e), "+s"(cpg_e));
+    const int elane = et & 63, elt = et >> 4, eq = et & 15;
+
+    const int hq = elane >> 4, rr = elane & 15;
 #if (WF_OPT & 2)
 #pragma unroll
     for (int pi = 0; pi < 9; ++pi)
@@ -675,34 +737,24 @@
 #endif
     __syncthreads();
     WF_STAMP(7);
-    const int c = cc * FC + 4 * q;
+    const int c = cc * FC + 4 * eq;
 #if (WF_OPT & 2)
-    const int csw = ((q ^ lt) & 15) << 2;
-#else
-    const int csw = (((q >> 2) ^ ((lt >> 2) & 3)) << 4) + (q & 3) * 4;
-#endif
-    PV s[4][6];
-#pragma unroll
-    for (int j = 0; j < 6; ++j) {
-        PV col[6], sj[4];
-#pragma unroll
-        for (int i = 0; i < 6; ++i) col[i] = ldpv(smem + ((i * 6 + j) * FT + lt) * FC + csw);
-        at4(col, sj);
-#pragma unroll
-        for (int i = 0; i < 4; ++i) s[i][j] = sj[i];
-    }
+    const int csw = ((eq ^ elt) & 15) << 2;
+#else
+    const int csw = (((eq >> 2) ^ ((elt >> 2) & 3)) << 4) + (eq & 3) * 4;
+#endif
     PV sc = {f32x2{1.f, 1.f}, f32x2{1.f, 1.f}}, sh = {f32x2{0.f, 0.f}, f32x2{0.f, 0.f}};
     if (a.scale) {
-        sc = ldpv(a.scale + g * a.ss_gs + c);
-        sh = ldpv(a.shift + g * a.ss_gs + c);
-    }
-    const float lo = a.relu ? 0.f : -__builtin_inff();
-    const int b0 = (int)(((long)tb * FT) / a.per_img);
+        sc = ldpv(a.scale + ge * a.ss_gs + c);
+        sh = ldpv(a.shift + ge * a.ss_gs + c);
+    }
+    const float lo = relu_e ? 0.f : -__builtin_inff();
+    const int b0 = (int)((unsigned)(tb * FT) / per_img_e);
     double sa = 0.0, sq = 0.0;
 #if (WF_OPT & 4)
     f32x2 psa = {0.f, 0.f}, psq = {0.f, 0.f};
 #endif
-    const __amdgpu_buffer_rsrc_t rs_out = make_rsrc(a.out + (long)g * a.out_gs, a.out_bytes);
+    const __amdgpu_buffer_rsrc_t rs_out = make_rsrc(a.out + (long)ge * a.out_gs, a.out_bytes);
     const unsigned opix = (unsigned)a.out_cs * 4u;
     const int oy0 = a.d * 4 * ta.ty + ta.py, ox0 = a.d * 4 * ta.tx + ta.px;
     const unsigned obase = (unsigned)((ta.b * a.H + oy0) * a.W + ox0) * opix + (unsigned)c * 4u;
@@ -711,6 +763,23 @@
     for (int i = 0; i < 4; ++i) {
         orow[i] = (tvalid && oy0 + i * a.d < a.H) ? obase + (unsigned)(i * a.d * a.W) * opix : OOBH;
         ocol[i] = (ox0 + i * a.d < a.W) ? (unsigned)(i * a.d) * opix : OOBH;
+    }
+    const int gslot = a.gn_sum && tvalid ? (ta.b == b0 ? 0 : 64) + (int)((unsigned)c / cpg_e) * 2 : -1;
+    const int vnext = vb + wk.step;
+    const bool more = WALK && vnext < wk.end;
+    if constexpr (WALK) {
+        locate(vnext, more);
+        request();
+    }
+    PV s[4][6];
+#pragma unroll
+    for (int j = 0; j < 6; ++j) {
+        PV col[6], sj[4];
+#pragma unroll
+        for (int i = 0; i < 6; ++i) col[i] = ldpv(smem + ((i * 6 + j) * FT + elt) * FC + csw);
+        at4(col, sj);
+#pragma unroll
+        for (int i = 0; i < 4; ++i) s[i][j] = sj[i];
     }
 #pragma unroll
     for (int i = 0; i < 4; ++i) {
@@ -742,19 +811,24 @@
         sa = (double)psa.x + (double)psa.y;
         sq = (double)psq.x + (double)psq.y;
 #endif
-        if (tvalid && (sa != 0.0 || sq != 0.0)) {
-            const int grp = c / a.gn_cpg, o = ta.b == b0 ? 0 : 64;
-            atomicAdd(&gacc[o + grp * 2], sa);
-            atomicAdd(&gacc[o + grp * 2 + 1], sq);
+        if (gslot >= 0 && (sa != 0.0 || sq != 0.0)) {
+            atomicAdd(&gacc[gslot], sa);
+            atomicAdd(&gacc[gslot + 1], sq);
         }
         __syncthreads();
-        if (t < 128) {
-            const double v = gacc[t];
-            const int b = b0 + (t >> 6);
-            if (v != 0.0 && b < a.B) atomicAdd(&a.gn_sum[(((long)g * a.Ball + a.boff + b) * a.gn_groups) * 2 + (t & 63)], v);
-        }
+        if (et < 128) {
+            const double v = gacc[et];
+            const int b = b0 + (et >> 6);
+            if (v != 0.0 && b < a.B) atomicAdd(&a.gn_sum[(((long)ge * a.Ball + a.boff + b) * a.gn_groups) * 2 + (et & 63)], v);
+            if (more) gacc[et] = 0.0;
+        }
+    } else if (more) {
+        __syncthreads();
     }
     WF_STAMP(9);
+    if (!more) break;
+    vb = vnext;
+    }
 #ifdef WF_STAMPS
     if (lane == 0 && blockIdx.x < WF_STAMP_BLOCKS && blockIdx.z == 0) {
         g_wf_stamps[((int)blockIdx.x * 4 + wave) * WF_STAMP_N + 14] = __builtin_amdgcn_s_memrealtime();
@@ -816,14 +890,33 @@
 
 size_t winograd_fused_ws_floats(int B, int Cin, int G) { return (size_t)2 * G * B * Cin; }
 
+static const void* fused_kernel(bool wide, bool one, bool norm, bool walk) {
+    static const void* const k32[2][2] = {{(const void*)wino_fused_kernel<false, false>, (const void*)wino_fused_kernel<false, true>},
+                                          {(const void*)wino_fused_kernel<true, false>, (const void*)wino_fused_kernel<true, true>}};
+    static const void* const k64[2][2][2] = {
+        {{(const void*)wino_fused64_kernel<false, false, false>, (const void*)wino_fused64_kernel<false, false, true>},
+         {(const void*)wino_fused64_kernel<false, true, false>, (const void*)wino_fused64_kernel<false, true, true>}},
+        {{(const void*)wino_fused64_kernel<true, false, false>, (const void*)wino_fused64_kernel<true, false, true>},
+         {(const void*)wino_fused64_kernel<true, true, false>, (const void*)wino_fused64_kernel<true, true, true>}}};
+    return wide ? k64[norm][one][walk] : k32[norm][walk];
+}
+
 int winograd_fused_prepare() {
-    QB_CHECK(hipFuncSetAttribute((const void*)wino_fused_kernel<true>, hipFuncAttributeMaxDynamicSharedMemorySize, SMEM_BYTES));
-    QB_CHECK(hipFuncSetAttribute((const void*)wino_fused_kernel<false>, hipFuncAttributeMaxDynamicSharedMemorySize, SMEM_BYTES));
-    QB_CHECK(hipFuncSetAttribute((const void*)wino_fused64_kernel<true>, hipFuncAttributeMaxDynamicSharedMemorySize, w64::SMEM_BYTES));
-    QB_CHECK(hipFuncSetAttribute((const void*)wino_fused64_kernel<false>, hipFuncAttributeMaxDynamicSharedMemorySize, w64::SMEM_BYTES));
-    QB_CHECK(hipFuncSetAttribute((const void*)wino_fused64_kernel<true, true>, hipFuncAttributeMaxDynamicSharedMemorySize, w64::SMEM_BYTES));
-    QB_CHECK(hipFuncSetAttribute((const void*)wino_fused64_kernel<false, true>, hipFuncAttributeMaxDynamicSharedMemorySize, w64::SMEM_BYTES));
+    for (int i = 0; i < 16; ++i) {
+        const bool wide = i & 1, one = i & 2;
+        if (!wide && one) continue;
+        QB_CHECK(hipFuncSetAttribute(fused_kernel(wide, one, i & 4, i & 8), hipFuncAttributeMaxDynamicSharedMemorySize, wide ? w64::SMEM_BYTES : SMEM_BYTES));
+    }
     return 0;
+}
+
+int winograd_fused_walk(int NB, int blocks, int block, int* items, int cap) {
+    if (NB < 0 || blocks <= 0 || block < 0 || block >= blocks) return 0;
+    const FusedWalk wk = fused_walk(NB, blocks, block);
+    int n = 0;
+    for (int vb = wk.first; vb < wk.end; vb += wk.step, ++n)
+        if (n < cap) items[n] = vb;
+    return n;
 }
 
 #ifdef WF_STAMPS
@@ -857,7 +950,7 @@
     const int ft = wide ? w64::FT : FT;
     a.NC = out.C / (wide ? w64::FC : FC);
     const long tblocks = (a.tiles + ft - 1) / ft;
-    if (tblocks * a.NC >= (1L << 31) || a.tiles + 64 >= (1L << 31)) return fail("winograd (fused): too many blocks");
+    if (tblocks * a.NC + 65536 >= (1L << 31) || a.tiles + 64 >= (1L << 31)) return fail("winograd (fused): too many blocks");
     a.NB = (int)(tblocks * a.NC);
     const bool gn_here = fused_gn_here(q, out.C, a.per_img, ft);
     if (dry) {
@@ -881,13 +974,18 @@
     {
         ProfScope prof(q.dtype == 3 ? "conv_gemm_f32pipe" : "wino_fused", 4.0 * G * ((double)Ball * H * W * (in.C + out.C) + (double)FP * in.C * out.C),
                        2.0 * G * FP * (double)a.tiles * in.C * out.C, st);
-        const void* fn32 = norm ? (const void*)wino_fused_kernel<true> : (const void*)wino_fused_kernel<false>;
-        const void* fn64 = in.C == 32 ? (norm ? (const void*)wino_fused64_kernel<true, true> : (const void*)wino_fused64_kernel<false, true>)
-                                      : (norm ? (const void*)wino_fused64_kernel<true> : (const void*)wino_fused64_kernel<false>);
-        const void* fn = wide ? fn64 : fn32;
+        int blocks = a.NB;
+        const bool gains = !norm && (!wide || in.C == 32);
+        const bool walk = tune().wino_fused_walk != 0 && (gains || tune().wino_fused_blocks > 0);
+        if (walk) {
+            const int cus = device_cus();
+            const int cap = tune().wino_fused_blocks > 0 ? std::max(8, (tune().wino_fused_blocks + 7) / 8 * 8) : cus > 0 ? cus : 256;
+            blocks = std::min((a.NB + 7) / 8 * 8, cap);
+        }
+        const void* fn = fused_kernel(wide, in.C == 32, norm, walk);
         const int smem_bytes = wide ? w64::SMEM_BYTES : SMEM_BYTES;
         void* args[] = {(void*)&a};
-        QB_CHECK(hipLaunchKernel(fn, dim3(a.NB, 1, G), dim3(256), args, smem_bytes, st));
+        QB_CHECK(hipLaunchKernel(fn, dim3(blocks, 1, G), dim3(256), args, smem_bytes, st));
     }
     QB_CHECK(hipGetLastError());
     if (q.gn_sum && !gn_here) return launch_gn_stats(out, Ball, G, q.gn_groups, q.gn_sum, st, false);
```

Result: no change. 10230 refined masks/s, median of 6 (+0.5%).
